# kyoungseoun-chung/pyapes

Measured on AMD Instinct MI355X. Metric: cell-updates*iters/sec, 3-D Poisson CG, higher is better.
Workload: dtype f64; 1 GPU; 3-D Poisson 512x512x512 double, periodic BCs, CG (BASELINE config 3); global_cells=134217728, parallelism=single

## Files before the change

pyapes_amd/csrc/pa_bc.hip:

```cpp
#include "pa_host.h"

#include <math.h>
#include <stdlib.h>
#include <stdio.h>
#include <string.h>

#include <algorithm>
#include <new>

template <typename T>
struct BCArgs {
  int axis, side, type;
  T sval;
  const T* vals;
  T c23, dxf, ndir;
  T c43, c13;
  const T* far0;
  const T* far1;
  const int* done;
};

template <typename T>
__global__ void __launch_bounds__(PA_BLOCK) k_bc_face(DevGeom G, T* __restrict__ x, BCArgs<T> B) {
  if (B.done && *B.done) return;
  const int a = B.axis;
  const int64_t nu = (a == 0) ? G.n1 : G.n0;
  const int64_t nv = (a == 2) ? G.n1 : G.n2;
  const int64_t N = (a == 0) ? G.g0 : (a == 1 ? G.n1 : G.n2);
  const int64_t off = (a == 0) ? G.off0 : 0;
  const int64_t st = (a == 0) ? G.s0 : (a == 1 ? G.s1 : 1);
  for (int64_t q = (int64_t)blockIdx.x * blockDim.x + threadIdx.x; q < nu * nv;
       q += (int64_t)gridDim.x * blockDim.x) {
    const int64_t u = q / nv, v = q - u * nv;
    int64_t base;
    if (a == 0) base = u * G.s1 + v;
    else if (a == 1) base = u * G.s0 + v;
    else base = u * G.s0 + v * G.s1;
    const int64_t f = (B.side == 0) ? 0 : N - 1;
    const int64_t p1 = (B.side == 0) ? pa_wrap(1, N) : pa_wrap(N - 2, N);
    const int64_t p2 = (B.side == 0) ? pa_wrap(2 % N, N) : pa_wrap(N - 3 < 0 ? N - 3 + N : N - 3, N);
    T* xf = x + base + (f - off) * st;
    if (B.type == 1) {
      *xf = B.vals ? B.vals[q] : B.sval;
    } else if (B.type == 2) {
      T vp = x[base + (p1 - off) * st];
      T vpp = x[base + (p2 - off) * st];
      T ct;
      if (B.vals) {
        ct = B.c23 * B.vals[q];
        ct = ct * B.dxf;
        ct = ct * B.ndir;
      } else {
        ct = B.sval;
      }
      T t1 = B.c43 * vp;
      T t2 = B.c13 * vpp;
      t1 = t1 - t2;
      *xf = t1 + ct;
    } else if (B.type == 3) {
      *xf = x[base + (p1 - off) * st];
    } else if (B.type == 4) {
      if (B.side == 0) {
        T vp = x[base + (p1 - off) * st];
        T vf, vff;
        if (B.far0) {
          vf = B.far0[q];
          vff = B.far1[q];
        } else {
          vf = x[base + (N - 1 - off) * st];
          vff = x[base + (pa_wrap(N - 2, N) - off) * st];
        }
        T t1 = vp - vf;
        *xf = t1 + vff;
      } else if (B.far0) {
        T t1 = B.far0[q] - x[base + (N - 1 - off) * st];
        *xf = t1 + x[base + (pa_wrap(N - 2, N) - off) * st];
      } else {
        *xf = x[base + (0 - off) * st];
      }
    }
  }
}

template <typename S>
__device__ __forceinline__ const S& pa_kernarg(size_t off) {
  return *(const S*)((const char*)__builtin_amdgcn_kernarg_segment_ptr() + off);
}
static_assert(sizeof(DevGeom) % 8 == 0, "second kernel parameter starts at sizeof(DevGeom)");

template <typename T>
__global__ void __launch_bounds__(PA_BLOCK) k_shell(DevGeom G, const SolverScalars* __restrict__ sc,
                                                     const T* __restrict__ x, T* __restrict__ shell_old,
                                                     double* __restrict__ partials, int mode) {
  if (mode == 1 && sc->done) return;
  const int64_t sz[3] = {G.n1 * G.n2, G.n0 * G.n2, G.n0 * G.n1};
  int64_t total = 0;
  int64_t start[6];
  for (int f = 0; f < 6; ++f) {
    start[f] = total;
    total += G.act[f >> 1] ? sz[f >> 1] : 0;
  }
  double s[1] = {0.0};
  for (int64_t q = (int64_t)blockIdx.x * blockDim.x + threadIdx.x; q < total;
       q += (int64_t)gridDim.x * blockDim.x) {
    int f = 0;
    for (int w = 1; w < 6; ++w)
      if (G.act[w >> 1] && q >= start[w]) f = w;
    const int a = f >> 1, side = f & 1;
    const int64_t local = q - start[f];
    int64_t i, j, k;
    if (a == 0) {
      int64_t gi = side == 0 ? 0 : G.g0 - 1;
      i = gi - G.off0;
      if (i < 0 || i >= G.n0) continue;
      j = local / G.n2; k = local - j * G.n2;
    } else if (a == 1) {
      i = local / G.n2; k = local - i * G.n2;
      j = side == 0 ? 0 : G.n1 - 1;
      int64_t gi = i + G.off0;
      if (G.act[0] && (gi == 0 || gi == G.g0 - 1)) continue;
    } else {
      i = local / G.n1; j = local - i * G.n1;
      k = side == 0 ? 0 : G.n2 - 1;
      int64_t gi = i + G.off0;
      if (G.act[0] && (gi == 0 || gi == G.g0 - 1)) continue;
      if (G.act[1] && (j == 0 || j == G.n1 - 1)) continue;
    }
    const int64_t o = i * G.s0 + j * G.s1 + k;
    T xn = x[o];
    if (mode == 1) {
      T df = xn - shell_old[q];
      T p = df * df;
      s[0] += (double)p;
    }
    shell_old[q] = xn;
  }
  if (mode == 1) pa_block_reduce_store<1>(s, partials);
}


template <typename T>
struct BCFaceDev {
  int type;
  T sval;
  const T* vals;
  T dxf, ndir;
};
template <typename T>
struct BCAll {
  BCFaceDev<T> f[6];
  T c43, c13, c23;
  const T* far_lo0;
  const T* far_lo1;
  const T* far_hi0;
  int slab_periodic0;
};

template <typename T>
__device__ __forceinline__ T pa_bc_const(const BCAll<T>& B, int f, int64_t q) {
  const BCFaceDev<T>& F = B.f[f];
  if (!F.vals) return F.sval;
  T ct = B.c23 * F.vals[q];
  ct = ct * F.dxf;
  return ct * F.ndir;
}

template <typename T, bool PER = true>
struct BCEval {
  const DevGeom& G;
  const BCAll<T>& B;
  const T* __restrict__ x;

  __device__ __forceinline__ T raw0(int f, int64_t g, int64_t base) const {
    const T* p = x + (g - G.off0) * G.s0;
    if (PER && B.slab_periodic0 && B.f[f].type == 4) {
      if (f == 0) {
        p = (g == G.g0 - 1) ? B.far_lo0 : ((g == G.g0 - 2) ? B.far_lo1 : p);
      } else {
        p = (g == 1) ? B.far_hi0 : p;
      }
    }
    return p[base];
  }

  __device__ __forceinline__ T stage0(int64_t i, int64_t j, int64_t k) const {
    const int64_t gi = i + G.off0;
    const int64_t base = j * G.s1 + k;
    int f = -1;
    if (G.act[0]) {
      if (gi == 0 && B.f[0].type) f = 0;
      else if (gi == G.g0 - 1 && B.f[1].type) f = 1;
    }
    if (f < 0) return x[i * G.s0 + base];
    const int type = B.f[f].type;
    const bool lower = f == 0;
    const int64_t N = G.g0;
    if (type == 1) return B.f[f].vals ? B.f[f].vals[base] : B.f[f].sval;
    if (type == 2) {
      T t1 = B.c43 * raw0(f, lower ? 1 : N - 2, base);
      T t2 = B.c13 * raw0(f, lower ? 2 : N - 3, base);
      t1 = t1 - t2;
      return t1 + pa_bc_const<T>(B, f, base);
    }
    if (type == 3 || !PER) return raw0(f, lower ? 1 : N - 2, base);
    T t1 = raw0(f, 1, base) - raw0(f, N - 1, base);
    return t1 + raw0(f, N - 2, base);
  }

  __device__ __forceinline__ T stage1(int64_t i, int64_t j, int64_t k) const {
    int f = -1;
    if (G.act[1]) {
      if (j == 0 && B.f[2].type) f = 2;
      else if (j == G.n1 - 1 && B.f[3].type) f = 3;
    }
    if (f < 0) return stage0(i, j, k);
    const int type = B.f[f].type;
    const bool lower = f == 2;
    const int64_t N = G.n1, q = i * G.n2 + k;
    if (type == 1) return B.f[f].vals ? B.f[f].vals[q] : B.f[f].sval;
    if (type == 2) {
      T t1 = B.c43 * stage0(i, lower ? 1 : N - 2, k);
      T t2 = B.c13 * stage0(i, lower ? 2 : N - 3, k);
      t1 = t1 - t2;
      return t1 + pa_bc_const<T>(B, f, q);
    }
    if (type == 3 || !PER) return stage0(i, lower ? 1 : N - 2, k);
    T t1 = stage0(i, 1, k) - stage0(i, N - 1, k);
    return t1 + stage0(i, N - 2, k);
  }

  __device__ __forceinline__ T stage2(int64_t i, int64_t j, int64_t k) const {
    int f = -1;
    if (G.act[2]) {
      if (k == 0 && B.f[4].type) f = 4;
      else if (k == G.n2 - 1 && B.f[5].type) f = 5;
    }
    if (f < 0) return stage1(i, j, k);
    const int type = B.f[f].type;
    const bool lower = f == 4;
    const int64_t N = G.n2, q = i * G.n1 + j;
    if (type == 1) return B.f[f].vals ? B.f[f].vals[q] : B.f[f].sval;
    if (type == 2) {
      T t1 = B.c43 * stage1(i, j, lower ? 1 : N - 2);
      T t2 = B.c13 * stage1(i, j, lower ? 2 : N - 3);
      t1 = t1 - t2;
      return t1 + pa_bc_const<T>(B, f, q);
    }
    if (type == 3 || !PER) return stage1(i, j, lower ? 1 : N - 2);
    T t1 = stage1(i, j, 1) - stage1(i, j, N - 1);
    return t1 + stage1(i, j, N - 2);
  }
};

template <typename T, bool PER>
__device__ __forceinline__ T pa_bc_v3(const DevGeom& G, const BCAll<T>& B, const T* __restrict__ x, int64_t i,
                                      int64_t j, int64_t k) {
  BCEval<T, PER> ev{G, B, x};
  return ev.stage2(i, j, k);
}

__device__ __forceinline__ bool pa_shell_node(const DevGeom& G, int64_t q, const int64_t* start, int64_t& i,
                                              int64_t& j, int64_t& k) {
  int f = 0;
  for (int w = 1; w < 6; ++w)
    if (G.act[w >> 1] && q >= start[w]) f = w;
  const int a = f >> 1, side = f & 1;
  const int64_t local = q - start[f];
  const int64_t dn = a == 2 ? G.n1 : G.n2;
  int64_t u, v;
  if (G.ncell <= 0x7fffffffLL) {
    const uint32_t lu = (uint32_t)local, du = (uint32_t)dn, uu = lu / du;
    u = uu; v = lu - uu * du;
  } else {
    u = local / dn; v = local - u * dn;
  }
  if (a == 0) {
    int64_t gi = side == 0 ? 0 : G.g0 - 1;
    i = gi - G.off0;
    if (i < 0 || i >= G.n0) return false;
    j = u; k = v;
  } else if (a == 1) {
    i = u; k = v;
    j = side == 0 ? 0 : G.n1 - 1;
    int64_t gi = i + G.off0;
    if (G.act[0] && (gi == 0 || gi == G.g0 - 1)) return false;
  } else {
    i = u; j = v;
    k = side == 0 ? 0 : G.n2 - 1;
    int64_t gi = i + G.off0;
    if (G.act[0] && (gi == 0 || gi == G.g0 - 1)) return false;
    if (G.act[1] && (j == 0 || j == G.n1 - 1)) return false;
  }
  return true;
}

template <typename T, bool PER>
__global__ void __launch_bounds__(PA_BLOCK) k_bc_compute(DevGeom G, BCAll<T> B_, const int* __restrict__ done,
                                                          const T* x, const T* __restrict__ shell_old,
                                                          T* __restrict__ shell_new, double* __restrict__ partials,
                                                          int with_delta, T* xw) {
  if (done && *done) return;
  const BCAll<T>& B = pa_kernarg<BCAll<T>>(sizeof(DevGeom));
  const int64_t sz[3] = {G.n1 * G.n2, G.n0 * G.n2, G.n0 * G.n1};
  int64_t total = 0, start[6];
  for (int f = 0; f < 6; ++f) { start[f] = total; total += G.act[f >> 1] ? sz[f >> 1] : 0; }
  double s[1] = {0.0};
  for (int64_t q = (int64_t)blockIdx.x * blockDim.x + threadIdx.x; q < total;
       q += (int64_t)gridDim.x * blockDim.x) {
    int64_t i, j, k;
    if (!pa_shell_node(G, q, start, i, j, k)) continue;
    T v = pa_bc_v3<T, PER>(G, B, x, i, j, k);
#ifdef PA_DEBUG_BC
    if (i == 0 && j == 1 && k == G.n2 - 1) {
      BCEval<T, PER> ev{G, B, x};
      printf("DBG node(0,1,%lld) v=%g stage1(0,1,n2-2)=%g stage0=%g types %d %d %d %d %d %d slabp %d far %p %p %p raw1 %g rawN1 %g rawN2 %g\n",
             (long long)k, (double)v, (double)ev.stage1(0, 1, G.n2 - 2), (double)ev.stage0(0, 1, G.n2 - 2),
             B.f[0].type, B.f[1].type, B.f[2].type, B.f[3].type, B.f[4].type, B.f[5].type, B.slab_periodic0,
             (void*)B.far_lo0, (void*)B.far_lo1, (void*)B.far_hi0, (double)ev.raw0(0, 1, 1 * G.s1 + G.n2 - 2),
             (double)ev.raw0(0, G.g0 - 1, 1 * G.s1 + G.n2 - 2), (double)ev.raw0(0, G.g0 - 2, 1 * G.s1 + G.n2 - 2));
    }
#endif
    shell_new[q] = v;
    if (xw) xw[i * G.s0 + j * G.s1 + k] = v;
    if (with_delta) {
      T df = v - shell_old[q];
      T p = df * df;
      s[0] += (double)p;
    }
  }
  if (with_delta) pa_block_reduce_store<1>(s, partials);
}

template <typename T>
__global__ void __launch_bounds__(PA_BLOCK) k_bc_scatter(DevGeom G, const int* __restrict__ done,
                                                          T* __restrict__ x, const T* __restrict__ shell_new) {
  if (done && *done) return;
  const int64_t sz[3] = {G.n1 * G.n2, G.n0 * G.n2, G.n0 * G.n1};
  int64_t total = 0, start[6];
  for (int f = 0; f < 6; ++f) { start[f] = total; total += G.act[f >> 1] ? sz[f >> 1] : 0; }
  for (int64_t q = (int64_t)blockIdx.x * blockDim.x + threadIdx.x; q < total;
       q += (int64_t)gridDim.x * blockDim.x) {
    int64_t i, j, k;
    if (!pa_shell_node(G, q, start, i, j, k)) continue;
    x[i * G.s0 + j * G.s1 + k] = shell_new[q];
  }
}


template <typename T>
struct BCPairArgs {
  BCArgs<T> lo, hi;
  int axis;
  int64_t pos_lo, pos_hi;
};

template <typename T>
__device__ __forceinline__ T pa_bc_face_value(const BCArgs<T>& B, const T* __restrict__ x, int64_t base, int64_t st,
                                              int64_t off, int64_t N, int64_t q, T x0_new) {
  const bool lower = B.side == 0;
  const int64_t p1 = lower ? 1 : N - 2, p2 = lower ? 2 : N - 3;
  if (B.type == 1) return B.vals ? B.vals[q] : B.sval;
  if (B.type == 2) {
    T ct;
    if (B.vals) {
      ct = B.c23 * B.vals[q];
      ct = ct * B.dxf;
      ct = ct * B.ndir;
    } else {
      ct = B.sval;
    }
    T t1 = B.c43 * x[base + (p1 - off) * st];
    T t2 = B.c13 * x[base + (p2 - off) * st];
    t1 = t1 - t2;
    return t1 + ct;
  }
  if (B.type == 3) return x[base + (p1 - off) * st];
  if (lower) {
    T vp = x[base + (1 - off) * st];
    T vf = B.far0 ? B.far0[q] : x[base + (N - 1 - off) * st];
    T vff = B.far0 ? B.far1[q] : x[base + (N - 2 - off) * st];
    T t1 = vp - vf;
    return t1 + vff;
  }
  if (B.far0) {
    T t1 = B.far0[q] - x[base + (N - 1 - off) * st];
    return t1 + x[base + (N - 2 - off) * st];
  }
  return x0_new;
}

template <typename T>
__global__ void __launch_bounds__(PA_BLOCK) k_bc_pair(DevGeom G, T* __restrict__ x, BCPairArgs<T> P,
                                                       const int* __restrict__ done, T* __restrict__ shell_old,
                                                       double* __restrict__ partials, int mode) {
  if (done && *done) return;
  const int a = P.axis;
  const int64_t nu = (a == 0) ? G.n1 : G.n0;
  const int64_t nv = (a == 2) ? G.n1 : G.n2;
  const int64_t N = (a == 0) ? G.g0 : (a == 1 ? G.n1 : G.n2);
  const int64_t off = (a == 0) ? G.off0 : 0;
  const int64_t st = (a == 0) ? G.s0 : (a == 1 ? G.s1 : 1);
  double s[1] = {0.0};
  for (int64_t q = (int64_t)blockIdx.x * blockDim.x + threadIdx.x; q < nu * nv;
       q += (int64_t)gridDim.x * blockDim.x) {
    const int64_t u = q / nv, v = q - u * nv;
    int64_t base;
    bool owned = true;
    if (a == 0) {
      base = u * G.s1 + v;
      if (G.act[1] && (u == 0 || u == G.n1 - 1)) owned = false;
      if (G.act[2] && (v == 0 || v == G.n2 - 1)) owned = false;
    } else if (a == 1) {
      base = u * G.s0 + v;
      if (G.act[2] && (v == 0 || v == G.n2 - 1)) owned = false;
    } else {
      base = u * G.s0 + v * G.s1;
    }
    T x0_new = (T)0;
    if (P.lo.type) {
      T* xf = x + base + (0 - off) * st;
      T val;
      if (mode == 3) {
        val = *xf;
      } else {
        val = pa_bc_face_value<T>(P.lo, x, base, st, off, N, q, (T)0);
        *xf = val;
      }
      x0_new = val;
      if (mode && owned) {
        if (mode == 1) {
          T df = val - shell_old[P.pos_lo + q];
          T p = df * df;
          s[0] += (double)p;
        }
        shell_old[P.pos_lo + q] = val;
      }
    } else if (P.hi.type == 4 && !P.hi.far0) {
      x0_new = x[base + (0 - off) * st];
    }
    if (P.hi.type) {
      T* xf = x + base + (N - 1 - off) * st;
      T val;
      if (mode == 3) {
        val = *xf;
      } else {
        val = pa_bc_face_value<T>(P.hi, x, base, st, off, N, q, x0_new);
        *xf = val;
      }
      if (mode && owned) {
        if (mode == 1) {
          T df = val - shell_old[P.pos_hi + q];
          T p = df * df;
          s[0] += (double)p;
        }
        shell_old[P.pos_hi + q] = val;
      }
    }
  }
  if (mode == 1) pa_block_reduce_store<1>(s, partials);
}

template <typename T>
static int pa_bc_shell_fused(pa_ctx* c, T* x, double* part2, int with_delta, bool guarded, int* nsh, bool standalone);
template <typename T>
static int pa_bc_pair_apply(pa_ctx* c, T* x, double* part2, int mode, bool guarded, int* nsh);
template <typename T>
static void pa_shell_launch(pa_ctx* c, const T* x, T* shell, double* part2, int with_delta);

template <typename T>
int pa_bc_apply_faces(pa_ctx* c, T* x, bool guarded) {
  const DevGeom& G = c->G;
  for (int w = 0; w < c->nbc; ++w) {
    int f = c->bc_order[w];
    const HostBC& b = c->bc[f];
    if (b.type == PA_BC_NONE) continue;
    int a = f >> 1, side = f & 1;
    if (!G.act[a]) continue;
    if (a == 0) {
      if (side == 0 && G.off0 != 0) continue;
      if (side == 1 && G.off0 + G.n0 != G.g0) continue;
    }
    BCArgs<T> B;
    memset(&B, 0, sizeof(B));
    B.axis = a; B.side = side; B.type = b.type;
    B.vals = (const T*)b.vals;
    B.c43 = (T)(4.0 / 3.0);
    B.c13 = (T)(1.0 / 3.0);
    B.c23 = (T)(2.0 / 3.0);
    B.dxf = (T)b.dxf;
    B.ndir = side == 0 ? (T)-1 : (T)1;
    B.done = guarded ? pa_done_flag(c) : nullptr;
    if (b.type == PA_BC_DIRICHLET) B.sval = (T)b.value;
    if (b.type == PA_BC_NEUMANN) {
      T pre = (T)((2.0 / 3.0) * b.value);
      pre = pre * B.dxf;
      pre = pre * B.ndir;
      B.sval = pre;
    }
    if (b.type == PA_BC_PERIODIC && a == 0 && G.n0 != G.g0) {
      B.far0 = (const T*)(side == 0 ? c->bc_far_lo0 : c->bc_far_hi0);
      B.far1 = (const T*)c->bc_far_lo1;
      if (!B.far0) { pa_set_err(c, "periodic axis-0 BC on a slab needs pa_bc_halo_ptrs planes"); return PA_E_STATE; }
    }
    int64_t nu = (a == 0) ? G.n1 : G.n0;
    int64_t nv = (a == 2) ? G.n1 : G.n2;
    hipLaunchKernelGGL(k_bc_face<T>, dim3(pa_grid_blocks(nu * nv)), dim3(PA_BLOCK), 0, c->stream, G, x, B);
  }
  PA_HIP(c, hipGetLastError());
  return PA_OK;
}

template <typename T>
int pa_bc_apply_auto(pa_ctx* c, T* x, bool guarded) {
  if (pa_bc_fusable(c)) return pa_bc_shell_fused<T>(c, x, nullptr, 0, guarded, nullptr, true);
  if (pa_bc_pairable(c)) return pa_bc_pair_apply<T>(c, x, nullptr, 0, guarded, nullptr);
  return pa_bc_apply_faces<T>(c, x, guarded);
}

int pa_bc_apply_any(pa_ctx* c, void* x) {
  return c->dtype == PA_F64 ? pa_bc_apply_auto<double>(c, (double*)x, false) : pa_bc_apply_auto<float>(c, (float*)x, false);
}

extern "C" {

int pa_apply_bc(pa_ctx* c, void* x) {
  if (!c || !c->grid_set) return PA_E_STATE;
  PA_HIP(c, hipSetDevice(c->device));
  return pa_bc_apply_any(c, x);
}

}

int pa_shell_blocks(const pa_ctx* c) {
  const DevGeom& G = c->G;
  int64_t tot = 0;
  if (G.act[0]) tot += 2 * G.n1 * G.n2;
  if (G.act[1]) tot += 2 * G.n0 * G.n2;
  if (G.act[2]) tot += 2 * G.n0 * G.n1;
  return pa_grid_blocks(tot);
}
int64_t pa_shell_elems(const pa_ctx* c) {
  const DevGeom& G = c->G;
  return 2 * (G.n1 * G.n2 + G.n0 * G.n2 + G.n0 * G.n1);
}

bool pa_bc_is_static(const pa_ctx* c) {
  for (int f = 0; f < 6; ++f) {
    int t = c->bc[f].type;
    if (t != PA_BC_NONE && t != PA_BC_DIRICHLET) return false;
  }
  return true;
}


bool pa_bc_fusable(const pa_ctx* c) {
  if (c->bc_path & 1) return false;
  bool one_pass = !c->slab;
  for (int f = 0; f < 6; ++f)
    if (c->bc[f].type == PA_BC_PERIODIC) one_pass = false;
  const int64_t limit = pa_bc_pairable(c) ? (one_pass ? 2000000 : 150000) : 400000;
  if (!(c->bc_path & 4) &&
      2 * (c->G.n1 * c->G.n2 + c->G.n0 * c->G.n2 + c->G.n0 * c->G.n1) > limit)
    return false;
  int last = -1;
  for (int w = 0; w < c->nbc; ++w) {
    if (c->bc[c->bc_order[w]].type == PA_BC_NONE) continue;
    if (c->bc_order[w] <= last) return false;
    last = c->bc_order[w];
  }
  const DevGeom& G = c->G;
  const int64_t N[3] = {G.g0, G.n1, G.n2};
  const int64_t nloc[3] = {G.n0, G.n1, G.n2};
  for (int a = 0; a < 3; ++a)
    if (G.act[a] && (N[a] < 5 || (a == 0 && nloc[0] < 3))) return false;
  for (int a = 0; a < 3; ++a)
    if ((c->bc[2 * a].type == PA_BC_PERIODIC) != (c->bc[2 * a + 1].type == PA_BC_PERIODIC)) return false;
  return true;
}

template <typename T>
static int bc_fill_all(pa_ctx* c, BCAll<T>& B) {
  memset(&B, 0, sizeof(B));
  const DevGeom& G = c->G;
  for (int f = 0; f < 6; ++f) {
    const HostBC& b = c->bc[f];
    BCFaceDev<T>& F = B.f[f];
    F.type = b.type;
    F.vals = (const T*)b.vals;
    F.dxf = (T)b.dxf;
    F.ndir = (f & 1) == 0 ? (T)-1 : (T)1;
    if (b.type == PA_BC_DIRICHLET) F.sval = (T)b.value;
    if (b.type == PA_BC_NEUMANN) {
      T pre = (T)((2.0 / 3.0) * b.value);
      pre = pre * F.dxf;
      pre = pre * F.ndir;
      F.sval = pre;
    }
    if ((f >> 1) == 0 && G.act[0]) {
      if (f == 0 && G.off0 != 0) F.type = PA_BC_NONE;
      if (f == 1 && G.off0 + G.n0 != G.g0) F.type = PA_BC_NONE;
    }
  }
  B.c43 = (T)(4.0 / 3.0);
  B.c13 = (T)(1.0 / 3.0);
  B.c23 = (T)(2.0 / 3.0);
  B.slab_periodic0 = (G.n0 != G.g0 && c->bc[0].type == PA_BC_PERIODIC) ? 1 : 0;
  if (B.slab_periodic0) {
    B.far_lo0 = (const T*)c->bc_far_lo0;
    B.far_lo1 = (const T*)c->bc_far_lo1;
    B.far_hi0 = (const T*)c->bc_far_hi0;
    if ((B.f[0].type == PA_BC_PERIODIC && (!B.far_lo0 || !B.far_lo1)) ||
        (B.f[1].type == PA_BC_PERIODIC && !B.far_hi0)) {
      pa_set_err(c, "periodic axis-0 BC on a slab needs the far planes (pa_slab_set)");
      return PA_E_STATE;
    }
  }
  return PA_OK;
}

template <typename T>
static int pa_bc_shell_fused(pa_ctx* c, T* x, double* part2, int with_delta, bool guarded, int* nsh,
                          bool standalone) {
  BCAll<T> B;
  int rc = bc_fill_all<T>(c, B);
  if (rc) return rc;
  const int nb = pa_shell_blocks(c);
  const size_t half = (size_t)pa_shell_elems(c);
  T *so, *sn;
  if (standalone) {
    if ((rc = pa_scratch(c, &c->scr[SCR_SHELL2], &c->cap[SCR_SHELL2], half * sizeof(T)))) return rc;
    so = sn = (T*)c->scr[SCR_SHELL2];
  } else {
    T* base = (T*)c->scr[SCR_SHELL];
    so = base + (c->shell_cur ? half : 0);
    sn = base + (c->shell_cur ? 0 : half);
  }
  const int* done = guarded ? pa_done_flag(c) : nullptr;
  bool direct = !c->slab;
  for (int f = 0; f < 6; ++f)
    if (c->bc[f].type == PA_BC_PERIODIC) direct = false;
  bool any_per = false;
  for (int f = 0; f < 6; ++f)
    if (c->bc[f].type == PA_BC_PERIODIC) any_per = true;
  if (any_per)
    hipLaunchKernelGGL((k_bc_compute<T, true>), dim3(nb), dim3(PA_BLOCK), 0, c->stream, c->G, B, done, (const T*)x,
                       (const T*)so, sn, part2, with_delta, direct ? x : (T*)nullptr);
  else
    hipLaunchKernelGGL((k_bc_compute<T, false>), dim3(nb), dim3(PA_BLOCK), 0, c->stream, c->G, B, done, (const T*)x,
                       (const T*)so, sn, part2, with_delta, direct ? x : (T*)nullptr);
  if (!direct)
    hipLaunchKernelGGL(k_bc_scatter<T>, dim3(nb), dim3(PA_BLOCK), 0, c->stream, c->G, done, x, (const T*)sn);
  if (!standalone) c->shell_cur ^= 1;
  if (nsh) *nsh = nb;
  PA_HIP(c, hipGetLastError());
  return PA_OK;
}

bool pa_bc_pairable(const pa_ctx* c) {
  if (c->bc_path & 2) return false;
  int last = -1, cnt = 0;
  for (int w = 0; w < c->nbc; ++w) {
    if (c->bc[c->bc_order[w]].type == PA_BC_NONE) continue;
    if (c->bc_order[w] <= last) return false;
    last = c->bc_order[w];
    ++cnt;
  }
  const DevGeom& G = c->G;
  const int64_t N[3] = {G.g0, G.n1, G.n2};
  int need = 0;
  for (int a = 0; a < 3; ++a) {
    if (!G.act[a]) continue;
    need += 2;
    if (N[a] < 5 || (a == 0 && G.n0 < 3)) return false;
    if (c->bc[2 * a].type == PA_BC_NONE || c->bc[2 * a + 1].type == PA_BC_NONE) return false;
    if ((c->bc[2 * a].type == PA_BC_PERIODIC) != (c->bc[2 * a + 1].type == PA_BC_PERIODIC)) return false;
  }
  return cnt == need;
}

template <typename T>
static void bc_face_args(pa_ctx* c, int f, BCArgs<T>& B, bool guarded) {
  const DevGeom& G = c->G;
  const HostBC& b = c->bc[f];
  memset(&B, 0, sizeof(B));
  const int a = f >> 1, side = f & 1;
  B.axis = a; B.side = side; B.type = b.type;
  if (a == 0) {
    if (side == 0 && G.off0 != 0) B.type = 0;
    if (side == 1 && G.off0 + G.n0 != G.g0) B.type = 0;
  }
  B.vals = (const T*)b.vals;
  B.c43 = (T)(4.0 / 3.0);
  B.c13 = (T)(1.0 / 3.0);
  B.c23 = (T)(2.0 / 3.0);
  B.dxf = (T)b.dxf;
  B.ndir = side == 0 ? (T)-1 : (T)1;
  B.done = guarded ? pa_done_flag(c) : nullptr;
  if (b.type == PA_BC_DIRICHLET) B.sval = (T)b.value;
  if (b.type == PA_BC_NEUMANN) {
    T pre = (T)((2.0 / 3.0) * b.value);
    pre = pre * B.dxf;
    pre = pre * B.ndir;
    B.sval = pre;
  }
  if (b.type == PA_BC_PERIODIC && a == 0 && G.n0 != G.g0) {
    B.far0 = (const T*)(side == 0 ? c->bc_far_lo0 : c->bc_far_hi0);
    B.far1 = (const T*)c->bc_far_lo1;
  }
}

template <typename T>
static int pa_bc_pair_apply(pa_ctx* c, T* x, double* part2, int mode, bool guarded, int* nsh) {
  const DevGeom& G = c->G;
  const int64_t sz[3] = {G.n1 * G.n2, G.n0 * G.n2, G.n0 * G.n1};
  int64_t start[6], total = 0;
  for (int f = 0; f < 6; ++f) { start[f] = total; total += G.act[f >> 1] ? sz[f >> 1] : 0; }
  T* shell = (T*)c->scr[SCR_SHELL];
  int rows = 0;
  for (int a = 0; a < 3; ++a) {
    if (!G.act[a]) continue;
    BCPairArgs<T> P;
    bc_face_args<T>(c, 2 * a, P.lo, guarded);
    bc_face_args<T>(c, 2 * a + 1, P.hi, guarded);
    if (mode != 3 && ((P.lo.type == PA_BC_PERIODIC && a == 0 && G.n0 != G.g0 && !P.lo.far0) ||
                      (P.hi.type == PA_BC_PERIODIC && a == 0 && G.n0 != G.g0 && !P.hi.far0))) {
      pa_set_err(c, "periodic axis-0 BC on a slab needs the far planes (pa_slab_set)");
      return PA_E_STATE;
    }
    if (!P.lo.type && !P.hi.type) continue;
    P.axis = a;
    P.pos_lo = start[2 * a];
    P.pos_hi = start[2 * a + 1];
    const int nb = pa_grid_blocks(sz[a]);
    hipLaunchKernelGGL(k_bc_pair<T>, dim3(nb), dim3(PA_BLOCK), 0, c->stream, G, x, P,
                       guarded ? pa_done_flag(c) : (const int*)nullptr, shell, part2 ? part2 + rows : nullptr,
                       mode);
    if (mode == 1) rows += nb;
  }
  if (nsh) *nsh = rows;
  PA_HIP(c, hipGetLastError());
  return PA_OK;
}


int pa_bc_shell_rows(const pa_ctx* c) {
  if (c->bc_fused || !c->bc_pair) return pa_shell_blocks(c);
  const DevGeom& G = c->G;
  const int64_t sz[3] = {G.n1 * G.n2, G.n0 * G.n2, G.n0 * G.n1};
  int rows = 0;
  for (int a = 0; a < 3; ++a) {
    if (!G.act[a]) continue;
    int lo = c->bc[2 * a].type, hi = c->bc[2 * a + 1].type;
    if (a == 0) {
      if (G.off0 != 0) lo = 0;
      if (G.off0 + G.n0 != G.g0) hi = 0;
    }
    if (lo || hi) rows += pa_grid_blocks(sz[a]);
  }
  return rows;
}

template <typename T>
static void pa_shell_launch(pa_ctx* c, const T* x, T* shell, double* part2, int with_delta) {
  hipLaunchKernelGGL(k_shell<T>, dim3(pa_shell_blocks(c)), dim3(PA_BLOCK), 0, c->stream, c->G, c->sc, x, shell, part2,
                     with_delta);
}

void pa_bc_plan(pa_ctx* c) {
  c->bc_static = pa_bc_is_static(c);
  c->bc_fused = pa_bc_fusable(c);
  c->bc_pair = (!c->bc_fused && pa_bc_pairable(c)) ? 1 : 0;
  c->shell_cur = 0;
}

template <typename T>
int pa_bc_fill_start(pa_ctx* c, T* x, bool filled_by_driver) {
  if (c->bc_fused && !filled_by_driver)
    return pa_bc_shell_fused<T>(c, x, nullptr, 0, false, nullptr, false);
  if (c->bc_pair) return pa_bc_pair_apply<T>(c, x, nullptr, filled_by_driver ? 3 : 2, false, nullptr);
  if (!filled_by_driver)
    if (int rc = pa_bc_apply_faces<T>(c, x)) return rc;
  pa_shell_launch<T>(c, (const T*)x, (T*)c->scr[SCR_SHELL], (double*)c->scr[SCR_PART2], 0);
  return PA_OK;
}

template <typename T>
int pa_bc_fill_step(pa_ctx* c, T* x, double* part2, int* nsh) {
  *nsh = 0;
  if (c->bc_static) return PA_OK;
  if (c->bc_fused) return pa_bc_shell_fused<T>(c, x, part2, 1, true, nsh, false);
  if (c->bc_pair) return pa_bc_pair_apply<T>(c, x, part2, 1, true, nsh);
  if (int rc = pa_bc_apply_faces<T>(c, x, true)) return rc;
  *nsh = pa_shell_blocks(c);
  pa_shell_launch<T>(c, (const T*)x, (T*)c->scr[SCR_SHELL], part2, 1);
  return PA_OK;
}

#define PA_BC_INST(T)                                                                            \
  template int pa_bc_apply_faces<T>(pa_ctx*, T*, bool);                                          \
  template int pa_bc_apply_auto<T>(pa_ctx*, T*, bool);                                           \
  template int pa_bc_fill_start<T>(pa_ctx*, T*, bool);                                           \
  template int pa_bc_fill_step<T>(pa_ctx*, T*, double*, int*);
PA_BC_INST(float)
PA_BC_INST(double)
#undef PA_BC_INST
```

pyapes_amd/csrc/pa_cg.hip:

```cpp
#include "pa_solver.h"

template <typename T>
__global__ void __launch_bounds__(PA_BLOCK) k_cg_a(DevGeom G, DevEq<T> E, const SolverScalars* __restrict__ sc,
                                                    Vec<T> rv, Vec<T> dv, T* __restrict__ dnew,
                                                    double* __restrict__ partials) {
  if (sc->done) return;
  DirAcc<T> acc{rv, dv, (T)sc->beta};
  double s[1] = {0.0};
  for (int64_t idx = (int64_t)blockIdx.x * blockDim.x + threadIdx.x; idx < G.ncell;
       idx += (int64_t)gridDim.x * blockDim.x) {
    int64_t i, j, k;
    pa_decode(G, idx, i, j, k);
    T e = (T)0;
    if (pa_in_S(G, i, j, k)) {
      e = acc.at(G, i, j, k);
      T Ad = pa_apply_terms<T>(G, E, acc, i, j, k, e);
      T p = e * Ad;
      s[0] += (double)p;
    }
    dnew[idx] = e;
  }
  pa_block_reduce_store<1>(s, partials);
}

template <typename T>
__global__ void __launch_bounds__(PA_BLOCK) k_cg_b(DevGeom G, DevEq<T> E, const SolverScalars* __restrict__ sc,
                                                    Vec<T> dv, T* __restrict__ x, const T* r, T* r_out,
                                                    T* __restrict__ send_lo, T* __restrict__ send_hi,
                                                    double* __restrict__ partials) {
  if (sc->done) return;
  FieldAcc<T> acc{dv};
  const T alpha = (T)sc->alpha;
  double s[2] = {0.0, 0.0};
  for (int64_t idx = (int64_t)blockIdx.x * blockDim.x + threadIdx.x; idx < G.ncell;
       idx += (int64_t)gridDim.x * blockDim.x) {
    int64_t i, j, k;
    pa_decode(G, idx, i, j, k);
    T rn = (T)0;
    if (pa_in_S(G, i, j, k)) {
      T dc = dv.p[idx];
      T Ad = pa_apply_terms<T>(G, E, acc, i, j, k, dc);
      T xo = x[idx];
      T ad = alpha * dc;
      T xn = xo + ad;
      x[idx] = xn;
      T aAd = alpha * Ad;
      rn = r[idx] - aAd;
      T p = rn * rn;
      s[0] += (double)p;
      if (!pa_on_shell(G, i, j, k)) {
        T df = xn - xo;
        T p2 = df * df;
        s[1] += (double)p2;
      }
    }
    r_out[idx] = rn;
    if (send_lo && i == 0) send_lo[j * G.s1 + k] = rn;
    if (send_hi && i == G.n0 - 1) send_hi[j * G.s1 + k] = rn;
  }
  pa_block_reduce_store<2>(s, partials);
}

template <typename T>
__global__ void __launch_bounds__(PA_BLOCK) k_cg_post_a(SolverScalars* sc, const double* partials, int nblk,
                                                         double* sums, int stage) {
  __shared__ double sm[PA_BLOCK / 64];
  if (sc->done) return;
  if (stage != 1) {
    double v = pa_reduce_partials(partials, nblk, 1, 0, sm);
    if (threadIdx.x == 0) sums[0] = v;
  }
  if (stage != 0 && threadIdx.x == 0) pa_logic_a<T>(sc, sums);
}

template <typename T>
__global__ void __launch_bounds__(PA_BLOCK) k_cg_post_b(SolverScalars* sc, const double* partials, int nblk,
                                                         const double* partials_shell, int nblk_shell,
                                                         double* sums, int stage) {
  __shared__ double sm[PA_BLOCK / 64];
  if (sc->done) return;
  if (stage != 1) {
    double rr = pa_reduce_partials(partials, nblk, 2, 0, sm);
    double dx2 = pa_reduce_partials(partials, nblk, 2, 1, sm);
    double sh = nblk_shell > 0 ? pa_reduce_partials(partials_shell, nblk_shell, 1, 0, sm) : 0.0;
    if (threadIdx.x == 0) {
      sums[1] = rr;
      sums[2] = dx2 + sh;
    }
  }
  if (stage != 0 && threadIdx.x == 0) pa_logic_b<T>(sc, sums);
}

template <typename T>
__global__ void __launch_bounds__(PA_BLOCK) k_ghost_dir(const SolverScalars* __restrict__ sc, int64_t n,
                                                         const T* __restrict__ r_lo, const T* __restrict__ r_hi,
                                                         const T* __restrict__ d_lo, const T* __restrict__ d_hi,
                                                         T* __restrict__ o_lo, T* __restrict__ o_hi) {
  if (sc->done) return;
  const T beta = (T)sc->beta;
  for (int64_t q = (int64_t)blockIdx.x * blockDim.x + threadIdx.x; q < n; q += (int64_t)gridDim.x * blockDim.x) {
    if (r_lo) { T b = beta * d_lo[q]; o_lo[q] = r_lo[q] + b; }
    if (r_hi) { T b = beta * d_hi[q]; o_hi[q] = r_hi[q] + b; }
  }
}

template <typename T>
struct MidArgs {
  const T* d;
  const T* r;
  const T* x;
  const T *r_lo, *r_hi;
  const T *d_lo, *d_hi;
  T *g_lo, *g_hi;
  T *send_lo, *send_hi;
  T *xp_lo1, *xp_hi0, *xp_hi1;
  LapCoef<T> lap;
  T coeff, sign;
  int has_coeff;
  const T* coeff_f;
};

template <typename T>
__device__ __forceinline__ T pa_lap_axis(const DevGeom& G, const LapCoef<T>& L, int a, int64_t g, int64_t N, T xp, T xc,
                                         T xm) {
  T cP = L.inv[a], cC = L.m2inv[a], cM = L.inv[a];
  const T cB = L.c23[a];
  const int rc = pa_row_case(G, a, g, N, G.treat);
  if (rc == 1) { cP = cB; cC = -cB; cM = (T)0; }
  if (rc == 2) { cP = (T)0; cC = -cB; cM = cB; }
  T s = cP * xp;
  T m = cC * xc;
  s = s + m;
  m = cM * xm;
  s = s + m;
  return s;
}

template <typename T>
__global__ void __launch_bounds__(PA_BLOCK) k_slab_mid(DevGeom G, SolverScalars* sc, const double* __restrict__ rows,
                                                        int nrows, double* __restrict__ sums, MidArgs<T> M) {
  __shared__ double sm[8];
  const int done_in = sc->done;
  const double rr_in = sc->rr;
  const T beta = (T)sc->beta;
  double v0 = 0.0;
  for (int b = threadIdx.x; b < nrows; b += PA_BLOCK) v0 += rows[b];
  if (done_in) return;
  for (int off = 32; off > 0; off >>= 1) v0 += __shfl_down(v0, off, 64);
  if ((threadIdx.x & 63) == 0) sm[threadIdx.x >> 6] = v0;
  __syncthreads();
  if (threadIdx.x == 0) {
    double v = 0.0;
    for (int w = 0; w < PA_BLOCK / 64; ++w) v += sm[w];
    const T dAd = (T)v;
    const T a = (T)rr_in / dAd;
    const double al = (isnan(a) || isinf(a)) ? 0.0 : (double)a;
    sm[4] = al;
    if (blockIdx.x == 0) {
      sc->dAd = (double)dAd;
      sc->alpha = al;
      sums[0] = v;
    }
  }
  __syncthreads();
  const T alpha = (T)sm[4];
  const int nb = (int)(gridDim.x / 5), sec = (int)(blockIdx.x / nb), bq = (int)(blockIdx.x - sec * nb);
  if (sec == 0 && !M.r_lo) return;
  if (sec == 1 && !M.r_hi) return;
  T* const xout = sec == 2 ? M.xp_lo1 : (sec == 3 ? M.xp_hi0 : M.xp_hi1);
  if (sec >= 2 && !xout) return;
  const int64_t ip = sec == 0 ? 0 : (sec == 1 ? G.n0 - 1 : (sec == 2 ? 1 : (sec == 3 ? G.n0 - 1 : G.n0 - 2)));
  const int64_t gi = ip + G.off0;
  const bool iS = gi >= G.slo[0] && gi <= G.shi[0];
  const T* const dpl = M.d + ip * G.s0;
  for (int64_t q = (int64_t)bq * blockDim.x + threadIdx.x; q < G.s0; q += (int64_t)nb * blockDim.x) {
    int64_t j, k;
    if (G.s0 <= 0x7fffffffLL) {
      const uint32_t qq = (uint32_t)q, s1 = (uint32_t)G.s1, jj = qq / s1;
      j = jj; k = qq - jj * s1;
    } else {
      j = q / G.s1; k = q - j * G.s1;
    }
    const bool inS = iS && j >= G.slo[1] && j <= G.shi[1] && k >= G.slo[2] && k <= G.shi[2];
    const T dc = dpl[q];
    if (sec >= 2) {
      const T xo = M.x[ip * G.s0 + q];
      T ad = alpha * dc;
      T xn = xo + ad;
      xout[q] = inS ? xn : xo;
      continue;
    }
    const T rg = sec == 0 ? M.r_lo[q] : M.r_hi[q];
    const T dg = sec == 0 ? M.d_lo[q] : M.d_hi[q];
    const T din = sec == 0 ? M.d[G.s0 + q] : M.d[(G.n0 - 2) * G.s0 + q];
    const T dj1 = dpl[pa_wrap(j + 1, G.n1) * G.s1 + k], dj0 = dpl[pa_wrap(j - 1, G.n1) * G.s1 + k];
    const T dk1 = dpl[j * G.s1 + pa_wrap(k + 1, G.n2)], dk0 = dpl[j * G.s1 + pa_wrap(k - 1, G.n2)];
    const T rc = M.r[ip * G.s0 + q];
    T cf = M.coeff;
    if (M.has_coeff && M.coeff_f) cf = M.coeff_f[ip * G.s0 + q];
    T bg = beta * dg;
    const T ghost = rg + bg;
    if (sec == 0) M.g_lo[q] = ghost; else M.g_hi[q] = ghost;
    T ax = (T)0;
    ax = ax + pa_lap_axis<T>(G, M.lap, 0, gi, G.g0, sec == 0 ? din : ghost, dc, sec == 0 ? ghost : din);
    ax = ax + pa_lap_axis<T>(G, M.lap, 1, j, G.n1, dj1, dc, dj0);
    ax = ax + pa_lap_axis<T>(G, M.lap, 2, k, G.n2, dk1, dc, dk0);
    if (M.has_coeff) ax = ax * cf;
    ax = ax * M.sign;
    T Ad = (T)0;
    Ad = Ad + ax;
    T aAd = alpha * Ad;
    T rn = rc - aAd;
    rn = inS ? rn : (T)0;
    if (sec == 0) M.send_lo[q] = rn; else M.send_hi[q] = rn;
  }
}

template <typename T>
static int cg_begin_t(pa_ctx* c, T* x, const T* rhs, double tol, int64_t max_it) {
  const DevGeom& G = c->G;
  const size_t fb = (size_t)G.ncell * sizeof(T);
  const int nblk = pa_grid_blocks(G.ncell);
  int rc;
  c->cg_ps1 = solver_pitch<T>(c, x);
  c->cg_pitch = c->cg_ps1 > 0 ? 1 : 0;
  const size_t fbp = c->cg_pitch ? (size_t)G.n0 * G.n1 * c->cg_ps1 * sizeof(T) : fb;
  if ((rc = pa_scratch(c, &c->scr[SCR_R], &c->cap[SCR_R], fbp))) return rc;
  if ((rc = pa_scratch(c, &c->scr[SCR_D0], &c->cap[SCR_D0], fbp))) return rc;
  if ((rc = pa_scratch(c, &c->scr[SCR_D1], &c->cap[SCR_D1], fbp))) return rc;
  if ((rc = pa_scratch(c, &c->scr[SCR_PART], &c->cap[SCR_PART], (size_t)PA_MAX_PARTIALS * 4 * sizeof(double)))) return rc;
  if ((rc = pa_scratch(c, &c->scr[SCR_PART2], &c->cap[SCR_PART2], (size_t)3 * PA_MAX_GRID * sizeof(double)))) return rc;
  if ((rc = pa_scratch(c, &c->scr[SCR_SHELL], &c->cap[SCR_SHELL], 2 * (size_t)pa_shell_elems(c) * sizeof(T)))) return rc;
  if ((rc = init_scalars(c, tol, max_it))) return rc;
  if ((rc = pa_place_begin(c, x, fb))) return rc;
  if (!c->cg_pitch) PA_HIP(c, hipMemsetAsync(c->scr[SCR_D1], 0, fb, c->stream));
  c->cg_x = x;
  c->cur = 0;
  c->fold_a_n = c->fold_b_n = c->fold_b_nsh = 0;
  c->fold_b_shell = nullptr;
  c->slab_fold = c->slab_fold_live = 0;
  pa_bc_plan(c);
  c->solve = PA_SOLVE_CG;
  DevEq<T> E;
  pa_build_eq<T>(c, c->nterms, c->terms, E);
  if ((rc = pa_bc_fill_start<T>(c, x, c->slab != 0))) return rc;
  T* r = (T*)c->scr[SCR_R];
  T* d = (T*)c->scr[SCR_D0];
  double* part = (double*)c->scr[SCR_PART];
  Vec<T> xv = pa_vec_self<T>(c, x);
  if (c->slab) { xv.glo = (const T*)c->x_glo; xv.ghi = (const T*)c->x_ghi; }
  if (c->cg_pitch) {
    if ((rc = cg_residual_init_pitch<T>(c, E, xv, rhs, (T*)c->scr[SCR_D1], r, d, part))) return rc;
    PA_HIP(c, hipMemsetAsync(c->scr[SCR_D1], 0, fbp, c->stream));
  }
  if (!c->cg_pitch && (rc = cg_residual_init<T>(c, E, xv, rhs, r, d, (T*)c->r_send_lo, (T*)c->r_send_hi, part))) return rc;
  launch_post_init<T>(c, part, nblk, c->slab ? 0 : 2);
  c->pending_init_logic = c->slab ? 1 : 0;
  if (c->slab) {
    const size_t pb = (size_t)G.s0 * sizeof(T);
    if ((rc = pa_scratch(c, &c->scr[SCR_GHOST], &c->cap[SCR_GHOST], 4 * pb))) return rc;
    PA_HIP(c, hipMemsetAsync(c->scr[SCR_GHOST], 0, 4 * pb, c->stream));
    char* g = (char*)c->scr[SCR_GHOST];
    c->d_glo[0] = g; c->d_ghi[0] = g + pb; c->d_glo[1] = g + 2 * pb; c->d_ghi[1] = g + 3 * pb;
  }
  PA_HIP(c, hipGetLastError());
  return PA_OK;
}

template <typename T>
static Vec<T> cg_vec(pa_ctx* c, const T* p, int which ) {
  Vec<T> v = pa_vec_self<T>(c, p);
  if (c->cg_pitch) v.glo = p + (c->G.n0 - 1) * c->G.n1 * c->cg_ps1;
  if (c->slab) {
    if (which == 0) {
      if (c->r_recv_lo) v.glo = (const T*)c->r_recv_lo;
      if (c->r_recv_hi) v.ghi = (const T*)c->r_recv_hi;
    } else {
      if (c->r_recv_lo) v.glo = (const T*)c->d_glo[c->cur];
      if (c->r_recv_hi) v.ghi = (const T*)c->d_ghi[c->cur];
    }
  }
  return v;
}

template <typename T>
static void cg_flush_fold(pa_ctx* c) {
  if (c->fold_a_n > 0) {
    hipLaunchKernelGGL(k_cg_post_a<T>, dim3(1), dim3(PA_BLOCK), 0, c->stream, c->sc,
                       (const double*)c->scr[SCR_PART] + 2 * (size_t)PA_MAX_PARTIALS, c->fold_a_n, pa_sums(c), 2);
    c->fold_a_n = 0;
  }
  if (c->fold_b_n > 0) {
    hipLaunchKernelGGL(k_cg_post_b<T>, dim3(1), dim3(PA_BLOCK), 0, c->stream, c->sc, c->fold_b_part,
                       c->fold_b_n, c->fold_b_shell ? c->fold_b_shell : (const double*)c->scr[SCR_PART2],
                       c->fold_b_nsh, pa_sums(c), 2);
    c->fold_b_n = c->fold_b_nsh = 0;
    c->fold_b_shell = nullptr;
  }
}

template <typename T>
int pa_cg_phase_a_t(pa_ctx* c, int stage_post) {
  PaRange range_("pyapes CG phase A: d' = r + beta d, sum d'.(A d')");
  const DevGeom& G = c->G;
  const int nblk = pa_grid_blocks(G.ncell);
  DevEq<T> E;
  pa_build_eq<T>(c, c->nterms, c->terms, E);
  T* r = (T*)c->scr[SCR_R];
  T* dold = (T*)c->scr[c->cur ? SCR_D1 : SCR_D0];
  T* dnew = (T*)c->scr[c->cur ? SCR_D0 : SCR_D1];
  double* part = (double*)c->scr[SCR_PART];
  const bool foldable = c->fold && c->in_iterate && stage_post == 2 && !c->slab && !c->profile;
  if (foldable) part += 2 * (size_t)PA_MAX_PARTIALS;
  const bool live = c->slab_fold_live != 0;
  if (live) part = c->rows_send;
  if (c->pending_init_logic) {
    launch_post_init<T>(c, nullptr, 0, 1);
    c->pending_init_logic = 0;
  }
  Vec<T> rv = cg_vec<T>(c, r, 0), dv = cg_vec<T>(c, dold, 1);
  if (c->slab && !live && (c->r_recv_lo || c->r_recv_hi)) {
    hipLaunchKernelGGL(k_ghost_dir<T>, dim3(pa_grid_blocks(G.s0)), dim3(PA_BLOCK), 0, c->stream, c->sc, G.s0,
                       (const T*)c->r_recv_lo, (const T*)c->r_recv_hi, (const T*)c->d_glo[c->cur],
                       (const T*)c->d_ghi[c->cur], (T*)c->d_glo[c->cur ^ 1], (T*)c->d_ghi[c->cur ^ 1]);
  }
  if (c->profile) (void)hipEventRecord(c->pev[0], c->stream);
  int rc = pa_cg3d_phase_a<T>(c, E, rv, dv, dnew, part);
  if (rc < 0) return rc;
  int used_blocks = rc;
  if (rc == 0 && live) { pa_set_err(c, "folded slab iteration: the tiled phase A declined after the plan"); return PA_E_STATE; }
  if (rc == 0 && c->cg_pitch) { pa_set_err(c, "pitched CG: the tiled phase A declined"); return PA_E_STATE; }
  if (rc == 0) {
    cg_flush_fold<T>(c);
    hipLaunchKernelGGL(k_cg_a<T>, dim3(nblk), dim3(PA_BLOCK), 0, c->stream, G, E, c->sc, rv, dv, dnew, part);
    used_blocks = nblk;
  }
  if (c->profile) pa_profile_stop(c, 0);
  c->cur ^= 1;
  if (live) {
  } else if (foldable && used_blocks <= PA_MAX_GRID)
    c->fold_a_n = used_blocks;
  else
    hipLaunchKernelGGL(k_cg_post_a<T>, dim3(1), dim3(PA_BLOCK), 0, c->stream, c->sc, part, used_blocks, pa_sums(c),
                       stage_post);
  PA_HIP(c, hipGetLastError());
  return PA_OK;
}

template <typename T>
int pa_cg_phase_b_t(pa_ctx* c, int stage_post) {
  PaRange range_("pyapes CG phase B: x += alpha d', r -= alpha A d', BC fill, sums");
  const DevGeom& G = c->G;
  const int nblk = pa_grid_blocks(G.ncell);
  DevEq<T> E;
  pa_build_eq<T>(c, c->nterms, c->terms, E);
  T* r = (T*)c->scr[SCR_R];
  T* d = (T*)c->scr[c->cur ? SCR_D1 : SCR_D0];
  T* x = (T*)c->cg_x;
  double* part = (double*)c->scr[SCR_PART];
  double* part2 = (double*)c->scr[SCR_PART2];
  Vec<T> dv = cg_vec<T>(c, d, 1);
  const bool live = c->slab_fold_live != 0;
  if (live) part = c->rows_send + c->fold_rows[0] + c->fold_rows[2];
  if (c->profile) (void)hipEventRecord(c->pev[2], c->stream);
  int rc = pa_cg3d_phase_b<T>(c, E, dv, x, r, part);
  if (rc < 0) return rc;
  int used_blocks = rc;
  if (rc == 0 && live) { pa_set_err(c, "folded slab iteration: the tiled phase B declined after the plan"); return PA_E_STATE; }
  if (rc == 0 && c->cg_pitch) { pa_set_err(c, "pitched CG: the tiled phase B declined"); return PA_E_STATE; }
  if (rc == 0) {
    cg_flush_fold<T>(c);
    hipLaunchKernelGGL(k_cg_b<T>, dim3(nblk), dim3(PA_BLOCK), 0, c->stream, G, E, c->sc, dv, x, (const T*)r,
                       c->cg_r_out ? (T*)c->cg_r_out : r, (T*)c->r_send_lo, (T*)c->r_send_hi, part);
    used_blocks = nblk;
  }
  if (c->cg_r_out) pa_place_r_written(c);
  if (c->profile) pa_profile_stop(c, 1);
  c->b_blocks = used_blocks;
  if (c->slab) {
    if (!live) pack_x_planes<T>(c, x);
    PA_HIP(c, hipGetLastError());
    return PA_OK;
  }
  int nsh;
  if ((rc = pa_bc_fill_step<T>(c, x, part2, &nsh))) return rc;
  const bool foldable = c->fold && c->in_iterate && stage_post == 2 && !c->slab && !c->profile &&
                        used_blocks <= PA_MAX_GRID && nsh <= 3 * PA_MAX_GRID;
  if (foldable) {
    c->fold_b_n = used_blocks;
    c->fold_b_nsh = nsh;
    c->fold_b_part = part;
  } else {
    hipLaunchKernelGGL(k_cg_post_b<T>, dim3(1), dim3(PA_BLOCK), 0, c->stream, c->sc, part, used_blocks, part2, nsh,
                       pa_sums(c), stage_post);
  }
  PA_HIP(c, hipGetLastError());
  return PA_OK;
}

template <typename T>
int pa_cg_bc_t(pa_ctx* c) {
  const DevGeom& G = c->G;
  T* x = (T*)c->cg_x;
  double* part = (double*)c->scr[SCR_PART];
  double* part2 = (double*)c->scr[SCR_PART2];
  const bool live = c->slab_fold_live != 0;
  if (live) part2 = c->rows_send + c->fold_rows[0];
  int nsh, rc;
  if ((rc = pa_bc_fill_step<T>(c, x, part2, &nsh))) return rc;
  if (live) {
    if (nsh > c->fold_rows[2]) { pa_set_err(c, "folded slab iteration: %d shell rows, %d planned", nsh, c->fold_rows[2]); return PA_E_STATE; }
    c->fold_b_part = c->rows_recv + c->fold_rows[0] + c->fold_rows[2];
    c->fold_b_n = c->fold_rows[1];
    c->fold_b_shell = c->rows_recv + c->fold_rows[0];
    c->fold_b_nsh = c->fold_rows[2];
  } else {
    hipLaunchKernelGGL(k_cg_post_b<T>, dim3(1), dim3(PA_BLOCK), 0, c->stream, c->sc, part, c->b_blocks, part2, nsh,
                       pa_sums(c), 0);
  }
  PA_HIP(c, hipGetLastError());
  return PA_OK;
}

template <typename T>
static int cg_slab_mid_t(pa_ctx* c) {
  const DevGeom& G = c->G;
  DevEq<T> E;
  pa_build_eq<T>(c, c->nterms, c->terms, E);
  if (E.nterms != 1 || E.t[0].kind != PA_OP_LAPLACIAN || c->coord != PA_COORD_XYZ || !G.act[0]) {
    pa_set_err(c, "folded slab iteration: one Laplacian term on a 3-D xyz mesh expected (the tiled kernels' equation)");
    return PA_E_STATE;
  }
  MidArgs<T> M;
  memset(&M, 0, sizeof(M));
  M.lap = E.lap;
  M.coeff = E.t[0].coeff; M.sign = E.t[0].sign; M.has_coeff = E.t[0].has_coeff; M.coeff_f = E.t[0].coeff_f;
  M.d = (const T*)c->scr[c->cur ? SCR_D1 : SCR_D0];
  M.r = (const T*)c->scr[SCR_R];
  M.x = (const T*)c->cg_x;
  M.r_lo = (const T*)c->r_recv_lo; M.r_hi = (const T*)c->r_recv_hi;
  M.d_lo = (const T*)c->d_glo[c->cur ^ 1]; M.d_hi = (const T*)c->d_ghi[c->cur ^ 1];
  M.g_lo = (T*)c->d_glo[c->cur]; M.g_hi = (T*)c->d_ghi[c->cur];
  M.send_lo = (T*)c->r_send_lo; M.send_hi = (T*)c->r_send_hi;
  if ((M.r_lo && !M.send_lo) || (M.r_hi && !M.send_hi)) { pa_set_err(c, "slab: a neighbour without a send plane"); return PA_E_STATE; }
  M.xp_lo1 = (T*)c->x_pack_lo1; M.xp_hi0 = (T*)c->x_pack_hi0; M.xp_hi1 = (T*)c->x_pack_hi1;
  const bool planes = M.r_lo || M.r_hi || M.xp_lo1 || M.xp_hi0 || M.xp_hi1;
  const int nbm = planes ? std::min(256, pa_grid_blocks(G.s0)) : 1;
  hipLaunchKernelGGL(k_slab_mid<T>, dim3(5 * nbm), dim3(PA_BLOCK), 0, c->stream, G, c->sc,
                     (const double*)c->rows_recv, c->fold_rows[0], pa_sums(c), M);
  PA_HIP(c, hipGetLastError());
  return PA_OK;
}

int pa_cg_slab_mid(pa_ctx* c) {
  return c->dtype == PA_F64 ? cg_slab_mid_t<double>(c) : cg_slab_mid_t<float>(c);
}

int pa_cg_slab_flush(pa_ctx* c) {
  if (c->dtype == PA_F64) cg_flush_fold<double>(c); else cg_flush_fold<float>(c);
  PA_HIP(c, hipGetLastError());
  return PA_OK;
}

template <typename T>
static int cg_run_t(pa_ctx* c, T* x, const T* rhs, double tol, int64_t max_it, pa_report* out) {
  int rc;
  if (try_resident<T>(c, 0, x, rhs, tol, max_it, 1.0, out, &rc)) return rc;
  if ((rc = cg_begin_t<T>(c, x, rhs, tol, max_it))) return rc;
  const int poll = poll_interval(c);
  PA_HIP(c, hipEventRecord(c->ev0, c->stream));
  int64_t enq = 0;
  c->in_iterate = 1;
  PollPipe P;
  bool done = false;
  int64_t batch = 1;
  while (!done && !rc) {
    int64_t nb = std::min<int64_t>(batch, max_it + 1 - enq);
    if (nb <= 0) {
      if ((rc = poll_drain(c, P, &done)) || done) break;
      nb = 1;
    }
    for (int64_t q = 0; q < nb && !rc; ++q) {
      if ((rc = pa_place_tick(c))) break;
      if ((rc = pa_cg_phase_a_t<T>(c, 2))) break;
      copy_x_old<T>(c, x);
      rc = pa_cg_phase_b_t<T>(c, 2);
      ++enq;
    }
    if (rc) break;
    if ((rc = pa_place_batch_end(c))) break;
    cg_flush_fold<T>(c);
    rc = poll_submit(c, P, &done);
    batch = std::min<int64_t>(poll, std::max<int64_t>(1, enq));
  }
  if (!rc) rc = read_scalars(c);
  c->in_iterate = 0;
  if (rc) { c->fold_a_n = c->fold_b_n = c->fold_b_nsh = 0; pa_place_end(c, 0); return rc; }
  rc = timed_report(c, out);
  pa_place_end(c, 1);
  return rc;
}

extern "C" int pa_cg(pa_ctx* c, void* x, const void* rhs, double tol, int64_t max_it, pa_report* out) {
  if (!c || !c->grid_set || !c->eq_set) { if (c) pa_set_err(c, "pa_cg: grid/equation not set"); return PA_E_STATE; }
  if (int rc0 = pa_check_eq_applicable(c)) return rc0;
  if (!out) return PA_E_ARG;
  if (c->slab) { pa_set_err(c, "pa_cg is the single-GPU loop; use the stepwise API on a slab"); return PA_E_STATE; }
  PA_HIP(c, hipSetDevice(c->device));
  const int rc = c->dtype == PA_F64 ? cg_run_t<double>(c, (double*)x, (const double*)rhs, tol, max_it, out)
                                    : cg_run_t<float>(c, (float*)x, (const float*)rhs, tol, max_it, out);
  c->solve = PA_SOLVE_NONE;
  pa_place_end(c, 0);
  return rc;
}

template <typename T>
static int cg_fold_plan_t(pa_ctx* c, int64_t* rows) {
  rows[0] = rows[1] = rows[2] = 0;
  DevEq<T> E;
  pa_build_eq<T>(c, c->nterms, c->terms, E);
  T* r = (T*)c->scr[SCR_R];
  T* d0 = (T*)c->scr[SCR_D0];
  T* d1 = (T*)c->scr[SCR_D1];
  double* part = (double*)c->scr[SCR_PART];
  c->plan_only = 1;
  const int na = pa_cg3d_phase_a<T>(c, E, cg_vec<T>(c, r, 0), cg_vec<T>(c, d0, 1), d1, part);
  const int nb = pa_cg3d_phase_b<T>(c, E, cg_vec<T>(c, d1, 1), (T*)c->cg_x, r, part);
  c->plan_only = 0;
  (void)hipGetLastError();
  const int ns = c->bc_static ? 0 : pa_bc_shell_rows(c);
  if (na <= 0 || nb <= 0 || na > PA_MAX_GRID || nb > PA_MAX_GRID || ns > 3 * PA_MAX_GRID) return PA_OK;
  rows[0] = na; rows[1] = nb; rows[2] = ns;
  return PA_OK;
}

extern "C" {

int pa_cg_begin(pa_ctx* c, void* x, const void* rhs, double tol, int64_t max_it) {
  if (!c || !c->grid_set || !c->eq_set) { if (c) pa_set_err(c, "pa_cg_begin: grid/equation not set"); return PA_E_STATE; }
  if (int rc0 = pa_check_eq_applicable(c)) return rc0;
  PA_HIP(c, hipSetDevice(c->device));
  return c->dtype == PA_F64 ? cg_begin_t<double>(c, (double*)x, (const double*)rhs, tol, max_it)
                            : cg_begin_t<float>(c, (float*)x, (const float*)rhs, tol, max_it);
}

int pa_cg_phase_a(pa_ctx* c) {
  if (int rc = pa_require_solve(c, PA_SOLVE_CG, "pa_cg_phase_a")) return rc;
  const int st = c->slab ? 0 : 2;
  return c->dtype == PA_F64 ? pa_cg_phase_a_t<double>(c, st) : pa_cg_phase_a_t<float>(c, st);
}

int pa_cg_phase_b(pa_ctx* c) {
  if (int rc = pa_require_solve(c, PA_SOLVE_CG, "pa_cg_phase_b")) return rc;
  if (c->slab && !c->slab_fold_live) {
    if (c->dtype == PA_F64)
      hipLaunchKernelGGL(k_cg_post_a<double>, dim3(1), dim3(PA_BLOCK), 0, c->stream, c->sc, (const double*)nullptr, 0, pa_sums(c), 1);
    else
      hipLaunchKernelGGL(k_cg_post_a<float>, dim3(1), dim3(PA_BLOCK), 0, c->stream, c->sc, (const double*)nullptr, 0, pa_sums(c), 1);
  }
  const int st = c->slab ? 0 : 2;
  return c->dtype == PA_F64 ? pa_cg_phase_b_t<double>(c, st) : pa_cg_phase_b_t<float>(c, st);
}

int pa_cg_bc(pa_ctx* c) {
  if (int rc = pa_require_solve(c, PA_SOLVE_CG, "pa_cg_bc")) return rc;
  if (!c->slab) return PA_OK;
  return c->dtype == PA_F64 ? pa_cg_bc_t<double>(c) : pa_cg_bc_t<float>(c);
}

int pa_cg_finish_iter(pa_ctx* c) {
  if (int rc = pa_require_solve(c, PA_SOLVE_CG, "pa_cg_finish_iter")) return rc;
  if (!c->slab || c->slab_fold_live) return PA_OK;
  if (c->dtype == PA_F64)
    hipLaunchKernelGGL(k_cg_post_b<double>, dim3(1), dim3(PA_BLOCK), 0, c->stream, c->sc, (const double*)nullptr, 0,
                       (const double*)nullptr, 0, pa_sums(c), 1);
  else
    hipLaunchKernelGGL(k_cg_post_b<float>, dim3(1), dim3(PA_BLOCK), 0, c->stream, c->sc, (const double*)nullptr, 0,
                       (const double*)nullptr, 0, pa_sums(c), 1);
  PA_HIP(c, hipGetLastError());
  return PA_OK;
}

int pa_cg_fold_plan(pa_ctx* c, int64_t* rows) {
  if (!c || !rows) return PA_E_ARG;
  if (int rc = pa_require_solve(c, PA_SOLVE_CG, "pa_cg_fold_plan")) return rc;
  if (!c->slab) { pa_set_err(c, "pa_cg_fold_plan needs a live slab solve (pa_slab_set, pa_cg_begin)"); return PA_E_STATE; }
  return c->dtype == PA_F64 ? cg_fold_plan_t<double>(c, rows) : cg_fold_plan_t<float>(c, rows);
}

int pa_cg_fold_set(pa_ctx* c, const int64_t* rows) {
  if (!c) return PA_E_ARG;
  if (int rc = pa_require_solve(c, PA_SOLVE_CG, "pa_cg_fold_set")) return rc;
  if (!c->slab) { pa_set_err(c, "pa_cg_fold_set needs a live slab solve"); return PA_E_STATE; }
  c->slab_fold = 0;
  if (!rows || rows[0] <= 0 || rows[1] <= 0 || rows[2] < 0) return PA_OK;
  if (rows[0] > PA_MAX_GRID || rows[1] > PA_MAX_GRID || rows[2] > 3 * PA_MAX_GRID) {
    pa_set_err(c, "pa_cg_fold_set: row counts beyond one resident wave of workgroups");
    return PA_E_ARG;
  }
  int64_t mine[3];
  if (int rc = pa_cg_fold_plan(c, mine)) return rc;
  if (mine[0] <= 0 || mine[0] > rows[0] || mine[1] > rows[1] || mine[2] > rows[2]) {
    pa_set_err(c, "pa_cg_fold_set: agreed rows (%lld %lld %lld) below this rank's (%lld %lld %lld)", (long long)rows[0],
               (long long)rows[1], (long long)rows[2], (long long)mine[0], (long long)mine[1], (long long)mine[2]);
    return PA_E_ARG;
  }
  const size_t tot = (size_t)rows[0] + 2 * (size_t)rows[1] + (size_t)rows[2];
  PA_HIP(c, hipSetDevice(c->device));
  if (tot > c->rows_cap) {
    if (c->rows_buf[0]) (void)hipFree(c->rows_buf[0]);
    if (c->rows_buf[1]) (void)hipFree(c->rows_buf[1]);
    c->rows_buf[0] = c->rows_buf[1] = nullptr;
    c->rows_cap = 0;
    PA_HIP(c, hipMalloc((void**)&c->rows_buf[0], tot * sizeof(double)));
    PA_HIP(c, hipMalloc((void**)&c->rows_buf[1], tot * sizeof(double)));
    c->rows_cap = tot;
  }
  c->rows_send = c->rows_buf[0];
  c->rows_recv = (mine[0] == rows[0] && mine[1] == rows[1] && mine[2] == rows[2]) ? c->rows_buf[0] : c->rows_buf[1];
  PA_HIP(c, hipMemsetAsync(c->rows_buf[0], 0, tot * sizeof(double), c->stream));
  PA_HIP(c, hipMemsetAsync(c->rows_buf[1], 0, tot * sizeof(double), c->stream));
  for (int q = 0; q < 3; ++q) c->fold_rows[q] = (int)rows[q];
  c->slab_fold = 1;
  return PA_OK;
}

int pa_cg_iterate(pa_ctx* c, int64_t n) {
  if (int rc = pa_require_solve(c, PA_SOLVE_CG, "pa_cg_iterate")) return rc;
  if (c->slab) { pa_set_err(c, "pa_cg_iterate is single-rank; drive the phases on a slab"); return PA_E_STATE; }
  c->in_iterate = 1;
  int rc = PA_OK;
  for (int64_t q = 0; q < n && !rc; ++q) {
    if ((rc = pa_place_tick(c))) break;
    rc = c->dtype == PA_F64 ? pa_cg_phase_a_t<double>(c, 2) : pa_cg_phase_a_t<float>(c, 2);
    if (!rc) rc = c->dtype == PA_F64 ? pa_cg_phase_b_t<double>(c, 2) : pa_cg_phase_b_t<float>(c, 2);
  }
  c->in_iterate = 0;
  if (!rc) rc = pa_place_batch_end(c);
  if (c->dtype == PA_F64) cg_flush_fold<double>(c); else cg_flush_fold<float>(c);
  return rc;
}

int pa_cg_end(pa_ctx* c, pa_report* out) {
  if (int rc = pa_require_solve(c, PA_SOLVE_CG, "pa_cg_end")) return rc;
  int rc = out ? pa_report_read(c, out) : PA_OK;
  c->solve = PA_SOLVE_NONE;
  pa_place_end(c, out ? 1 : 0);
  if (rc) return rc;
  return (out && out->status) ? PA_E_NONFINITE : PA_OK;
}

}
```

pyapes_amd/csrc/pa_cg3d.hip:

```cpp
#include "pa_cg3d_kernel.h"
#include "pa_cg2d_kernel.h"

template <typename T>
int pa_cg3d_phase_a(pa_ctx* c, const DevEq<T>& E, Vec<T> r, Vec<T> d, T* dnew, double* partials) {
  const int mode = c->cg_pitch ? 3 : cg3d_mode<T>(c, E, {r.p, d.p, dnew, r.glo, r.ghi, d.glo, d.ghi}, false, false, true);
  if (!mode) return 0;
  const bool rz = c->coord == PA_COORD_RZ;
  Cg3dArgs<T> A;
  memset(&A, 0, sizeof(A));
  fill_common<T>(c, E, A);
  A.ps1 = c->cg_ps1; A.ps0 = c->cg_ps1 * c->G.n1;
  A.r = r; A.d = d; A.dnew = dnew; A.partials = partials;
  A.reverse = 0;
  if (c->fold_b_n > 0) {
    A.pre_part = c->fold_b_part;
    A.pre_n = c->fold_b_n;
    A.pre_shell = c->fold_b_shell ? c->fold_b_shell : (const double*)c->scr[SCR_PART2];
    A.pre_nsh = c->fold_b_nsh;
    A.sc_w = c->sc_alt;
    A.pre_sums = pa_sums(c);
  }
  int n = (mode == 1 || mode == 3 || mode == 4) ? launch_cg2d<T, 0>(c, A, mode == 3) : 0;
  if (n == 0 && rz) return 0;
  if (n == 0) n = launch_any<T, 0>(c, A, mode);
  if (n > 0 && hipGetLastError() != hipSuccess) { pa_set_err(c, "k_cg3d phase A launch failed"); return PA_E_HIP; }
  if (n > 0 && c->fold_b_n > 0) {
    SolverScalars* t = c->sc; c->sc = c->sc_alt; c->sc_alt = t;
    c->fold_b_n = c->fold_b_nsh = 0;
    c->fold_b_shell = nullptr;
  }
  return n;
}

template <typename T>
int pa_cg3d_phase_b(pa_ctx* c, const DevEq<T>& E, Vec<T> d, T* x, T* r, double* partials) {
  T* const r_out = c->cg_r_out ? (T*)c->cg_r_out : r;
  const int mode = c->cg_pitch ? 3 : cg3d_mode<T>(c, E, {d.p, x, r, r_out, d.glo, d.ghi, c->r_send_lo, c->r_send_hi}, false, false, true);
  if (!mode) return 0;
  const bool rz = c->coord == PA_COORD_RZ;
  Cg3dArgs<T> A;
  memset(&A, 0, sizeof(A));
  fill_common<T>(c, E, A);
  A.ps1 = c->cg_ps1; A.ps0 = c->cg_ps1 * c->G.n1;
  A.d = d; A.x = x; A.rw = r; A.rw_out = r_out; A.partials = partials;
  if (!c->slab_fold_live) {
    A.send_lo = (T*)c->r_send_lo; A.send_hi = (T*)c->r_send_hi;
  }
  A.reverse = 1;
  if (c->fold_a_n > 0) {
    A.pre_part = (const double*)c->scr[SCR_PART] + 2 * (size_t)PA_MAX_PARTIALS;
    A.pre_n = c->fold_a_n;
    A.sc_w = c->sc;
    A.pre_sums = pa_sums(c);
  }
  int n = (mode == 1 || mode == 3 || mode == 4) ? launch_cg2d<T, 1>(c, A, mode == 3) : 0;
  if (n == 0 && rz) return 0;
  if (n == 0) n = launch_any<T, 1>(c, A, mode);
  if (n > 0 && hipGetLastError() != hipSuccess) { pa_set_err(c, "k_cg3d phase B launch failed"); return PA_E_HIP; }
  if (n > 0) c->fold_a_n = 0;
  return n;
}

template <typename T>
int pa_tile3d_jacobi(pa_ctx* c, const DevEq<T>& E, Vec<T> x, const T* rhs, T* xnew, double omega, double* partials) {
  const int mode = cg3d_mode<T>(c, E, {x.p, rhs, xnew, x.glo, x.ghi}, false, false, true);
  if (!mode) return 0;
  const bool rz = c->coord == PA_COORD_RZ;
  Cg3dArgs<T> A;
  memset(&A, 0, sizeof(A));
  fill_common<T>(c, E, A);
  A.d = x; A.out = xnew; A.aux = rhs; A.p0 = (T)omega; A.partials = partials;
  if (c->fold_b_n > 0) {
    A.pre_part = c->fold_b_part;
    A.pre_n = c->fold_b_n;
    A.pre_shell = c->fold_b_shell ? c->fold_b_shell : (const double*)c->scr[SCR_PART2];
    A.pre_nsh = c->fold_b_nsh;
    A.sc_w = c->sc_alt;
    A.pre_sums = pa_sums(c);
  }
  int n = 0;
  if (mode == 1 || mode == 4) {
    const bool back2 = c->jac_alt && c->jac_dir && !c->plan_only;
    n = back2 ? launch_cg2d<T, 9>(c, A, false) : launch_cg2d<T, 4>(c, A, false);
    if (n > 0 && !c->plan_only) c->jac_dir ^= 1;
  }
  if (n == 0 && rz) return 0;
  if (n == 0) {
    const bool back = c->jac_alt && c->jac_dir && !c->plan_only;
    n = back ? launch_any<T, 9>(c, A, mode) : launch_any<T, 4>(c, A, mode);
    if (n > 0 && !c->plan_only) c->jac_dir ^= 1;
  }
  if (n > 0 && hipGetLastError() != hipSuccess) { pa_set_err(c, "k_cg3d Jacobi launch failed"); return PA_E_HIP; }
  if (n > 0 && c->fold_b_n > 0) {
    SolverScalars* t = c->sc; c->sc = c->sc_alt; c->sc_alt = t;
    c->fold_b_n = c->fold_b_nsh = 0;
    c->fold_b_shell = nullptr;
  }
  return n;
}

template int pa_tile3d_jacobi<float>(pa_ctx*, const DevEq<float>&, Vec<float>, const float*, float*, double, double*);
template int pa_tile3d_jacobi<double>(pa_ctx*, const DevEq<double>&, Vec<double>, const double*, double*, double, double*);
template int pa_cg3d_phase_a<float>(pa_ctx*, const DevEq<float>&, Vec<float>, Vec<float>, float*, double*);
template int pa_cg3d_phase_a<double>(pa_ctx*, const DevEq<double>&, Vec<double>, Vec<double>, double*, double*);
template int pa_cg3d_phase_b<float>(pa_ctx*, const DevEq<float>&, Vec<float>, float*, float*, double*);
template int pa_cg3d_phase_b<double>(pa_ctx*, const DevEq<double>&, Vec<double>, double*, double*, double*);
```

pyapes_amd/csrc/pa_cg3d_kernel.h:

```cpp
#pragma once
#include "pa_host.h"

#include <stdio.h>
#include <stdlib.h>
#include <string.h>

template <typename T> struct VecOf;
template <> struct VecOf<double> { static constexpr int N = 2; typedef double type __attribute__((ext_vector_type(2))); };
template <> struct VecOf<float>  { static constexpr int N = 4; typedef float type __attribute__((ext_vector_type(4))); };

template <typename T>
struct Cg3dArgs {
  DevGeom G;
  LapCoef<T> lap;
  T coeff, sign;
  int has_coeff;
  const T* coeff_f;
  const SolverScalars* sc;
  Vec<T> r, d;
  T* dnew;
  T* x;
  T* rw;
  T* rw_out;
  T* send_lo;
  T* send_hi;
  double* partials;
  int tiles_j, tiles_k, chunks, reverse;
  const T* aux;
  T* out;
  Vec<T> v;
  T* out2;
  T p0, p1, u;
  T hh[3], h2[3], ih[3];
  int kind;
  int lap_off;
  GradCoef<T> grd;
  int gnd;
  int64_t ps0, ps1;
  const T* rz;
  int64_t rz_n;
  int interior_only;
  int out_all;
  int bcl_type[6];
  T bcl_val[6];
  T bcl_c43, bcl_c13;
  const double* pre_part;
  const double* pre_shell;
  int pre_n, pre_nsh;
  SolverScalars* sc_w;
  double* pre_sums;
  const T* stg_phi0;
  T stg_c0, stg_c1;
  const T* src;
  T src_val;
};

__device__ __forceinline__ int pa_xcd_remap(int b, int nb) {
  const int q = nb >> 3, r = nb & 7, xcd = b & 7, w = b >> 3;
  return (xcd < r ? xcd * (q + 1) : r * (q + 1) + (xcd - r) * q) + w;
}

__device__ __forceinline__ int64_t pa_wrapmod(int64_t v, int64_t n) {
  v %= n;
  return v < 0 ? v + n : v;
}

template <typename T, int RJ, int PHASE, bool CF = false, int KIND = 0, int LAY = 0, bool STG = false>
__global__ void __launch_bounds__(256) k_cg3d(Cg3dArgs<T> A) {
  static_assert(!STG || PHASE == 3, "STG: the explicit Euler step");
  constexpr int PH = PHASE == 9 ? 4 : PHASE;
  constexpr bool NARROW = LAY == 1, PITCH = LAY == 2;
  static_assert(!PITCH || ((PH == 0 || PH == 1 || PH == 5 || PH == 6 || PH == 8) && !CF && KIND == 0),
                "PITCH: the CG / BiCGSTAB phases of a plain Laplacian");
  constexpr int VEC = NARROW ? 1 : VecOf<T>::N;
  typedef T V __attribute__((ext_vector_type(VEC)));
  constexpr int TJ = 4 * RJ, TK = 64 * VEC, TKP = TK + 2 * VEC;
  __shared__ __attribute__((aligned(16))) T tile[2][TJ + 2][TKP];

  (void)sizeof(int[PH >= 0 && PH <= 8 ? 1 : -1]);
  T beta = (T)0, alpha = (T)0;
  T omega = (T)0;
  const DevGeom& G = A.G;
  const int lane = threadIdx.x & 63, wv = threadIdx.x >> 6;
  const int vb = pa_xcd_remap(blockIdx.x, gridDim.x);
  const int tiles = A.tiles_j * A.tiles_k;
  const int chunk = vb / tiles, tl = vb - chunk * tiles;
  const int tjb = tl / A.tiles_k, tkb = tl - tjb * A.tiles_k;
  const int64_t i0 = (int64_t)chunk * G.n0 / A.chunks, i1 = (int64_t)(chunk + 1) * G.n0 / A.chunks;
  const int CI = (int)(i1 - i0);
  const int64_t j0 = (int64_t)tjb * TJ, k0 = (int64_t)tkb * TK;
  constexpr int rev = (PHASE == 1 || PHASE == 9) ? 1 : 0;

  const int64_t kg = k0 + (int64_t)lane * VEC;
  const int64_t kc = pa_wrapmod(kg, G.n2);
  const bool kvalid = kg < G.n2;
  const int64_t fs0 = PITCH ? A.ps0 : G.s0, fs1 = PITCH ? A.ps1 : G.s1;
  const int64_t kcf = PITCH ? (kg < fs1 ? kg : 0) : kc;
  int64_t jrow[RJ];
  unsigned rowS = 0, rowShell = 0, rowValid = 0, rowLo = 0, rowHi = 0;
#pragma unroll
  for (int jj = 0; jj < RJ; ++jj) {
    const int64_t jg = j0 + wv * RJ + jj;
    jrow[jj] = pa_wrapmod(jg, G.n1);
    const bool valid = jg < G.n1;
    if (valid) rowValid |= 1u << jj;
    if (valid && jg >= G.slo[1] && jg <= G.shi[1]) rowS |= 1u << jj;
    if (jg == 0 || jg == G.n1 - 1) rowShell |= 1u << jj;
    const int rc = pa_row_case(G, 1, jg, G.n1, G.treat);
    if (rc == 1) rowLo |= 1u << jj;
    if (rc == 2) rowHi |= 1u << jj;
  }
  unsigned rowPLo = 0, rowPHi = 0, colPLo = 0, colPHi = 0;
  if (PH == 3 || PH == 7 || KIND != 0) {
#pragma unroll
    for (int jj = 0; jj < RJ; ++jj) {
      const int64_t jg = j0 + wv * RJ + jj;
      if (G.bct[2] == 4 && jg == 1) rowPLo |= 1u << jj;
      if (G.bct[3] == 4 && jg == G.n1 - 2) rowPHi |= 1u << jj;
    }
#pragma unroll
    for (int v = 0; v < VEC; ++v) {
      if (G.bct[4] == 4 && kg + v == 1) colPLo |= 1u << v;
      if (G.bct[5] == 4 && kg + v == G.n2 - 2) colPHi |= 1u << v;
    }
  }
  unsigned colS = 0, colShell = 0, colLo = 0, colHi = 0;
#pragma unroll
  for (int v = 0; v < VEC; ++v) {
    const int64_t kk = kg + v;
    if (kvalid && kk >= G.slo[2] && kk <= G.shi[2]) colS |= 1u << v;
    if (kk == 0 || kk == G.n2 - 1) colShell |= 1u << v;
    const int rc = pa_row_case(G, 2, kk, G.n2, G.treat);
    if (rc == 1) colLo |= 1u << v;
    if (rc == 2) colHi |= 1u << v;
  }
#ifdef PA_PLAIN_EXPERIMENT
  rowLo = rowHi = colLo = colHi = 0;
  rowS = rowValid = (1u << RJ) - 1;
  colS = (1u << VEC) - 1;
#endif
  const int64_t hrow = (wv == 0) ? pa_wrapmod(j0 - 1, G.n1) : pa_wrapmod(j0 + TJ, G.n1);
  const bool hvec = (wv == 0 || wv == 3);
  const bool hsc = (wv == 1 && lane < 2 * TJ);
  const int hs_row = lane >> 1, hs_side = lane & 1;
  const int64_t hs_off = pa_wrapmod(j0 + hs_row, G.n1) * fs1 +
                         (hs_side ? pa_wrapmod(k0 + TK, G.n2) : pa_wrapmod(k0 - 1, G.n2));

  auto plane_of = [&](int q) -> int64_t { return rev ? (i1 - 1 - q) : (i0 + q); };
  auto pptr = [&](const Vec<T>& v, int64_t ii) -> const T* {
    return ii < 0 ? v.glo : (ii >= G.n0 ? v.ghi : v.p + ii * fs0);
  };

  struct Raw {
    V d[RJ];
    V r[RJ];
    V q[RJ];
    V hd, hr, hq;
    T sd, sr, sq;
  };
  constexpr bool HAS_R = (PH == 0 || PH == 5 || PH == 6);
  constexpr bool HAS_Q = (PH == 5);
  auto issue_at = [&](const T* dp, const T* rp, const T* qp, Raw& w, bool with_halo) {
#pragma unroll
    for (int jj = 0; jj < RJ; ++jj) {
      const int64_t o = jrow[jj] * fs1 + kcf;
      w.d[jj] = *reinterpret_cast<const V*>(dp + o);
      if (HAS_R) w.r[jj] = *reinterpret_cast<const V*>(rp + o);
      if (HAS_Q) w.q[jj] = *reinterpret_cast<const V*>(qp + o);
    }
    if (with_halo) {
      if (hvec) {
        const int64_t o = hrow * fs1 + kcf;
        w.hd = *reinterpret_cast<const V*>(dp + o);
        if (HAS_R) w.hr = *reinterpret_cast<const V*>(rp + o);
        if (HAS_Q) w.hq = *reinterpret_cast<const V*>(qp + o);
      }
      if (hsc) {
        w.sd = dp[hs_off];
        if (HAS_R) w.sr = rp[hs_off];
        if (HAS_Q) w.sq = qp[hs_off];
      }
    }
  };
  auto issue = [&](int64_t ii, Raw& w, bool with_halo) {
    const T* dp = pptr(A.d, ii);
    issue_at(dp, HAS_R ? pptr(A.r, ii) : dp, HAS_Q ? pptr(A.v, ii) : dp, w, with_halo);
  };
  auto combine = [&](T rr_, T dd_, T qq_) -> T {
    if (PH == 0) {
      T bd = beta * dd_;
      return rr_ + bd;
    } else if (PH == 5) {
      T t = omega * qq_;
      t = dd_ - t;
      t = beta * t;
      return rr_ + t;
    } else if (PH == 6) {
      T av = alpha * dd_;
      return rr_ - av;
    }
    return dd_;
  };
  auto finish_own = [&](const Raw& w, V (&e)[RJ]) {
#pragma unroll
    for (int jj = 0; jj < RJ; ++jj) {
#pragma unroll
      for (int v = 0; v < VEC; ++v)
        e[jj][v] = combine(HAS_R ? w.r[jj][v] : (T)0, w.d[jj][v], HAS_Q ? w.q[jj][v] : (T)0);
    }
  };
  auto finish_halo = [&](const Raw& w, V& hv, T& hs) {
#pragma unroll
    for (int v = 0; v < VEC; ++v) hv[v] = combine(HAS_R ? w.hr[v] : (T)0, w.hd[v], HAS_Q ? w.hq[v] : (T)0);
    hs = combine(HAS_R ? w.sr : (T)0, w.sd, HAS_Q ? w.sq : (T)0);
  };
  auto stage = [&](int buf, const V (&e)[RJ], const V& hv, const T& hs) {
#pragma unroll
    for (int jj = 0; jj < RJ; ++jj)
      *reinterpret_cast<V*>(&tile[buf][wv * RJ + jj + 1][VEC + lane * VEC]) = e[jj];
    if (hvec) *reinterpret_cast<V*>(&tile[buf][wv == 0 ? 0 : TJ + 1][VEC + lane * VEC]) = hv;
    if (hsc) tile[buf][hs_row + 1][hs_side ? VEC + TK : VEC - 1] = hs;
  };

  V ea[RJ], ec[RJ], eb[RJ];
  V hv;
  T hs = (T)0;
  Raw w;
#pragma unroll
  for (int v = 0; v < VEC; ++v) { hv[v] = (T)0; w.hd[v] = (T)0; w.hr[v] = (T)0; w.hq[v] = (T)0; }
  w.sd = (T)0; w.sr = (T)0; w.sq = (T)0;

  const bool act0 = G.act[0] != 0;
  Raw wa = w, wc = w;
  if (act0) issue(plane_of(-1), wa, false);
  issue(plane_of(0), wc, true);
  if (act0) issue(plane_of(1), w, CI > 1);

  if ((PH == 0 || PH == 4) && A.pre_n > 0) {
    __shared__ double pre_sm[16];
    const SolverScalars* si = A.sc;
    const int done_in = si->done;
    const double rr_in = si->rr, beta_in = si->beta, tol_lim = si->tolerance;
    const long long itr_in = si->itr, max_it = si->max_it;
    double v0 = 0.0, v1 = 0.0, v2 = 0.0;
    for (int b = threadIdx.x; b < A.pre_n; b += 256) {
      if (PH == 0) v0 += A.pre_part[2 * (int64_t)b];
      v1 += A.pre_part[2 * (int64_t)b + 1];
    }
    for (int b = threadIdx.x; b < A.pre_nsh; b += 256) v2 += A.pre_shell[b];
    if (done_in) {
      if (blockIdx.x == 0 && threadIdx.x == 0) *A.sc_w = *si;
      return;
    }
    for (int off = 32; off > 0; off >>= 1) {
      v0 += __shfl_down(v0, off, 64);
      v1 += __shfl_down(v1, off, 64);
      v2 += __shfl_down(v2, off, 64);
    }
    if ((threadIdx.x & 63) == 0) {
      const int w = threadIdx.x >> 6;
      pre_sm[3 * w] = v0;
      pre_sm[3 * w + 1] = v1;
      pre_sm[3 * w + 2] = v2;
    }
    __syncthreads();
    if (threadIdx.x == 0) {
      double rr = 0.0, dx2 = 0.0, sh = 0.0;
      for (int w = 0; w < 4; ++w) { rr += pre_sm[3 * w]; dx2 += pre_sm[3 * w + 1]; sh += pre_sm[3 * w + 2]; }
      const T rr_new = (T)rr;
      const T tolv = (T)sqrt(dx2 + sh);
      const bool bad = isnan(tolv) || isinf(tolv);
      const T rr_old = (T)rr_in;
      const double bq = bad ? beta_in : (double)(rr_new / rr_old);
      const long long itr = itr_in + (bad ? 0 : 1);
      const int done = (bad || itr > max_it || !((double)tolv > tol_lim)) ? 1 : 0;
      pre_sm[12] = bq;
      pre_sm[13] = done ? 1.0 : 0.0;
      if (blockIdx.x == 0) {
        SolverScalars* so = A.sc_w;
        *so = *si;
        so->tol = (double)tolv;
        so->done = done;
        if (bad) {
          so->err = 1;
        } else {
          if (PH == 0) {
            so->rr_old = (double)rr_old;
            so->beta = bq;
            so->rr = (double)rr_new;
          }
          so->itr = itr;
        }
        if (PH == 0) A.pre_sums[1] = rr;
        A.pre_sums[2] = dx2 + sh;
      }
    }
    __syncthreads();
    if (pre_sm[13] != 0.0) return;
    beta = (T)pre_sm[12];
  } else if (PH == 1 && A.pre_n > 0) {
    __shared__ double pre_sm[8];
    const int done_in = A.sc->done;
    const double rr_in = A.sc->rr;
    double v0 = 0.0;
    for (int b = threadIdx.x; b < A.pre_n; b += 256) v0 += A.pre_part[b];
    if (done_in) return;
    for (int off = 32; off > 0; off >>= 1) v0 += __shfl_down(v0, off, 64);
    if ((threadIdx.x & 63) == 0) pre_sm[threadIdx.x >> 6] = v0;
    __syncthreads();
    if (threadIdx.x == 0) {
      double v = 0.0;
      for (int w = 0; w < 4; ++w) v += pre_sm[w];
      const T dAd = (T)v;
      const T a = (T)rr_in / dAd;
      const double al = (isnan(a) || isinf(a)) ? 0.0 : (double)a;
      pre_sm[4] = al;
      if (blockIdx.x == 0) {
        A.sc_w->dAd = (double)dAd;
        A.sc_w->alpha = al;
        A.pre_sums[0] = v;
      }
    }
    __syncthreads();
    alpha = (T)pre_sm[4];
  } else if ((PH == 5 || PH == 8) && A.pre_n > 0) {
    __shared__ double pre_sm[8];
    const SolverScalars* si = A.sc;
    const int done_in = si->done, fe = si->finished_early;
    const double tol_lim = si->tolerance, rho_next = si->rho_next, rho_in = si->rho, alpha_in = si->alpha,
                 omega_in = si->omega;
    const long long itr_in = si->itr, max_it = si->max_it;
    double v0 = 0.0;
    for (int b = threadIdx.x; b < A.pre_n; b += 256) v0 += A.pre_part[b];
    if (done_in) {
      if (blockIdx.x == 0 && threadIdx.x == 0) *A.sc_w = *si;
      return;
    }
    for (int off = 32; off > 0; off >>= 1) v0 += __shfl_down(v0, off, 64);
    if ((threadIdx.x & 63) == 0) pre_sm[threadIdx.x >> 6] = v0;
    __syncthreads();
    if (threadIdx.x == 0) {
      double v = 0.0;
      for (int w = 0; w < 4; ++w) v += pre_sm[w];
      const T tolv = (T)sqrt(v);
      const bool bad = !fe && (isnan(tolv) || isinf(tolv));
      int done = (fe || bad) ? 1 : 0;
      T bq = (T)0;
      if (!fe && !bad) {
        if ((double)tolv <= tol_lim) done = 1;
        if (itr_in >= max_it) done = 1;
        bq = (T)rho_next / (T)rho_in;
        bq = bq * (T)alpha_in;
        bq = bq / (T)omega_in;
      }
      pre_sm[4] = (double)bq;
      pre_sm[5] = done ? 1.0 : 0.0;
      if (blockIdx.x == 0) {
        SolverScalars* so = A.sc_w;
        *so = *si;
        so->done = done;
        if (!fe) {
          so->tol = (double)tolv;
          if (bad) {
            so->err = 1;
          } else {
            so->beta = (double)bq;
            so->rho = rho_next;
          }
        }
      }
    }
    __syncthreads();
    if (pre_sm[5] != 0.0) return;
    beta = (T)pre_sm[4];
    omega = (T)omega_in;
  } else if (PH == 6 && A.pre_n > 0) {
    __shared__ double pre_sm[8];
    const int done_in = A.sc->done;
    const double rho_in = A.sc->rho;
    double v0 = 0.0;
    for (int b = threadIdx.x; b < A.pre_n; b += 256) v0 += A.pre_part[b];
    if (done_in) return;
    for (int off = 32; off > 0; off >>= 1) v0 += __shfl_down(v0, off, 64);
    if ((threadIdx.x & 63) == 0) pre_sm[threadIdx.x >> 6] = v0;
    __syncthreads();
    if (threadIdx.x == 0) {
      double v = 0.0;
      for (int w = 0; w < 4; ++w) v += pre_sm[w];
      const T q = (T)rho_in / (T)v;
      const double al = (isnan(q) || isinf(q)) ? 0.0 : (double)q;
      pre_sm[4] = al;
      if (blockIdx.x == 0) {
        A.sc_w->itr += 1;
        A.sc_w->alpha = al;
      }
    }
    __syncthreads();
    alpha = (T)pre_sm[4];
  } else {
    if (PH != 2 && PH != 3 && PH != 7 && A.sc->done) return;
    if (PH == 0) beta = (T)A.sc->beta;
    if (PH == 1) alpha = (T)A.sc->alpha;
    if (PH == 5) { beta = (T)A.sc->beta; omega = (T)A.sc->omega; }
    if (PH == 6) alpha = (T)A.sc->alpha;
  }

  if (act0) {
    finish_own(wa, ea);
  } else {
#pragma unroll
    for (int jj = 0; jj < RJ; ++jj)
#pragma unroll
      for (int v = 0; v < VEC; ++v) ea[jj][v] = (T)0;
  }
  finish_own(wc, ec);
  finish_halo(wc, hv, hs);
  stage(0, ec, hv, hs);
  if (act0) {
    finish_own(w, eb);
    finish_halo(w, hv, hs);
  } else {
#pragma unroll
    for (int jj = 0; jj < RJ; ++jj)
#pragma unroll
      for (int v = 0; v < VEC; ++v) eb[jj][v] = (T)0;
  }
  __syncthreads();

  double s0 = 0.0, s1 = 0.0, s2 = 0.0, s3 = 0.0;
  const T sgn = A.sign, cf = A.coeff;
  const int hasc = A.has_coeff;
  const T cfe = hasc ? cf : (T)1;
  constexpr bool VROW = (PH == 2 || PH == 3 || PH == 4 || PH == 7 || KIND != 0);
  V cPkV, cCkV, cMkV;
  if (VROW) {
#pragma unroll
    for (int v = 0; v < VEC; ++v) {
      T p = A.lap.inv[2], c0 = A.lap.m2inv[2], mq = A.lap.inv[2];
      if (colLo >> v & 1) { p = A.lap.c23[2]; c0 = -A.lap.c23[2]; mq = (T)0; }
      if (colHi >> v & 1) { p = (T)0; c0 = -A.lap.c23[2]; mq = A.lap.c23[2]; }
      cPkV[v] = p; cCkV[v] = c0; cMkV[v] = mq;
    }
  }
  V gPkV, gCkV, gMkV;
  if (PH == 7) {
#pragma unroll
    for (int v = 0; v < VEC; ++v) {
      T p = A.grd.g[2], c0 = (T)0, mq = A.grd.mg[2];
      if (colLo >> v & 1) { p = A.grd.lo_p[2]; c0 = A.grd.lo_c[2]; mq = (T)0; }
      if (colHi >> v & 1) { p = (T)0; c0 = A.grd.hi_c[2]; mq = A.grd.hi_m[2]; }
      if (colPLo >> v & 1) mq = (T)0;
      if (colPHi >> v & 1) p = (T)0;
      gPkV[v] = p; gCkV[v] = c0; gMkV[v] = mq;
    }
  }

  const int64_t pstep = rev ? -fs0 : fs0;
  const T* d_run = A.d.p + plane_of(1) * fs0;
  const T* r_run = HAS_R ? A.r.p + plane_of(1) * fs0 : d_run;
  const T* q_run = HAS_Q ? A.v.p + plane_of(1) * fs0 : d_run;
  const T* const d_end = pptr(A.d, plane_of(CI));
  const T* const r_end = HAS_R ? pptr(A.r, plane_of(CI)) : d_end;
  const T* const q_end = HAS_Q ? pptr(A.v, plane_of(CI)) : d_end;

  for (int m = 0; m < CI; ++m) {
    const int buf = m & 1;
    const int64_t ii = plane_of(m);
    const bool more = m + 1 < CI;
    if (more) stage(buf ^ 1, eb, hv, hs);
    V xv[RJ], rv[RJ];
    if (PH == 1) {
#pragma unroll
      for (int jj = 0; jj < RJ; ++jj) {
        const int64_t o = ii * G.s0 + jrow[jj] * G.s1 + kc;
        if (PITCH) {
          rv[jj] = __builtin_nontemporal_load(reinterpret_cast<const V*>(A.rw + ii * fs0 + jrow[jj] * fs1 + kcf));
          const T* xp = A.x + ii * G.s0 + jrow[jj] * G.s1;
#pragma unroll
          for (int v = 0; v < VEC; ++v) xv[jj][v] = xp[kg + v < G.n2 ? kg + v : G.n2 - 1];
        } else if (NARROW) {
          xv[jj] = *reinterpret_cast<const V*>(A.x + o);
          rv[jj] = *reinterpret_cast<const V*>(A.rw + o);
        } else {
          xv[jj] = __builtin_nontemporal_load(reinterpret_cast<const V*>(A.x + o));
          rv[jj] = __builtin_nontemporal_load(reinterpret_cast<const V*>(A.rw + o));
        }
      }
    }
    V cv[RJ];
    if (CF) {
#pragma unroll
      for (int jj = 0; jj < RJ; ++jj)
        cv[jj] = *reinterpret_cast<const V*>(A.coeff_f + ii * G.s0 + jrow[jj] * G.s1 + kc);
    }
    if (PH == 4 || PH == 5 || PH == 6 || PH == 8 || ((PH == 3 || (PH == 2 && KIND != 0)) && A.aux)) {
#pragma unroll
      for (int jj = 0; jj < RJ; ++jj) {
        if ((PH == 5 || PH == 6 || PH == 8) && !NARROW) {
          xv[jj] = PITCH ? __builtin_nontemporal_load(reinterpret_cast<const V*>(A.aux + ii * fs0 + jrow[jj] * fs1 + kcf))
                         : __builtin_nontemporal_load(reinterpret_cast<const V*>(A.aux + ii * G.s0 + jrow[jj] * G.s1 + kc));
          continue;
        }
        xv[jj] = PITCH ? *reinterpret_cast<const V*>(A.aux + ii * fs0 + jrow[jj] * fs1 + kcf)
                 : (PH == 4 && !NARROW) ? __builtin_nontemporal_load(reinterpret_cast<const V*>(A.aux + ii * G.s0 + jrow[jj] * G.s1 + kc))
                       : *reinterpret_cast<const V*>(A.aux + ii * G.s0 + jrow[jj] * G.s1 + kc);
      }
    }
    if constexpr (STG) {
#pragma unroll
      for (int jj = 0; jj < RJ; ++jj)
        rv[jj] = *reinterpret_cast<const V*>(A.stg_phi0 + ii * G.s0 + jrow[jj] * G.s1 + kc);
    }
    d_run += pstep;
    if (HAS_R) r_run += pstep;
    if (HAS_Q) q_run += pstep;
    if (more) {
      const bool inside = m + 2 < CI;
      issue_at(inside ? d_run : d_end, HAS_R ? (inside ? r_run : r_end) : d_run, HAS_Q ? (inside ? q_run : q_end) : d_run, w, inside);
    }

    const int64_t gi = ii + G.off0;
    const bool iS = gi >= G.slo[0] && gi <= G.shi[0];
    const bool iShell = act0 && (gi == 0 || gi == G.g0 - 1);
    T cPi = A.lap.inv[0], cCi = A.lap.m2inv[0], cMi = A.lap.inv[0];
    {
      const int rc = pa_row_case(G, 0, gi, G.g0, G.treat);
      if (rc == 1) { cPi = A.lap.c23[0]; cCi = -A.lap.c23[0]; cMi = (T)0; }
      if (rc == 2) { cPi = (T)0; cCi = -A.lap.c23[0]; cMi = A.lap.c23[0]; }
      if (!act0) { cPi = (T)0; cCi = (T)0; cMi = (T)0; }
    }
    const bool iPLo = (PH == 3 || PH == 7 || KIND != 0) && G.bct[0] == 4 && gi == 1;
    const bool iPHi = (PH == 3 || PH == 7 || KIND != 0) && G.bct[1] == 4 && gi == G.g0 - 2;
    T gP0 = A.grd.g[0], gC0 = (T)0, gM0 = A.grd.mg[0];
    if (PH == 7) {
      const int rc = pa_row_case(G, 0, gi, G.g0, G.treat);
      if (rc == 1) { gP0 = A.grd.lo_p[0]; gC0 = A.grd.lo_c[0]; gM0 = (T)0; }
      if (rc == 2) { gP0 = (T)0; gC0 = A.grd.hi_c[0]; gM0 = A.grd.hi_m[0]; }
      if (iPLo) gM0 = (T)0;
      if (iPHi) gP0 = (T)0;
    }
    V res[RJ];
    V g0r[RJ], g1r[RJ], g2r[RJ];
#pragma unroll
    for (int jj = 0; jj < RJ; ++jj) {
      const int R = wv * RJ + jj + 1;
      T cPj = A.lap.inv[1], cCj = A.lap.m2inv[1], cMj = A.lap.inv[1];
      if (rowLo >> jj & 1) { cPj = A.lap.c23[1]; cCj = -A.lap.c23[1]; cMj = (T)0; }
      if (rowHi >> jj & 1) { cPj = (T)0; cCj = -A.lap.c23[1]; cMj = A.lap.c23[1]; }
      V up, dn;
      if (jj > 0) up = ec[jj - 1]; else up = *reinterpret_cast<const V*>(&tile[buf][R - 1][VEC + lane * VEC]);
      if (jj < RJ - 1) dn = ec[jj + 1]; else dn = *reinterpret_cast<const V*>(&tile[buf][R + 1][VEC + lane * VEC]);
      const T left = tile[buf][R][VEC + lane * VEC - 1];
      const T right = tile[buf][R][VEC + lane * VEC + VEC];
      if constexpr (VROW) {
        const V xc = ec[jj];
        const V xpi = rev ? ea[jj] : eb[jj];
        const V xmi = rev ? eb[jj] : ea[jj];
        V xpk, xmk;
  #pragma unroll
        for (int v = 0; v < VEC; ++v) {
          xpk[v] = (v < VEC - 1) ? xc[v + 1 < VEC ? v + 1 : v] : right;
          xmk[v] = (v > 0) ? xc[v > 0 ? v - 1 : 0] : left;
        }
        if constexpr (PH == 7) {
          T pj = A.grd.g[1], cj = (T)0, mj = A.grd.mg[1];
          if (rowLo >> jj & 1) { pj = A.grd.lo_p[1]; cj = A.grd.lo_c[1]; mj = (T)0; }
          if (rowHi >> jj & 1) { pj = (T)0; cj = A.grd.hi_c[1]; mj = A.grd.hi_m[1]; }
          if (rowPLo >> jj & 1) mj = (T)0;
          if (rowPHi >> jj & 1) pj = (T)0;
          V s = gP0 * xpi;
          V mm = gC0 * xc;
          s = s + mm;
          mm = gM0 * xmi;
          g0r[jj] = s + mm;
          s = pj * dn;
          mm = cj * xc;
          s = s + mm;
          mm = mj * up;
          g1r[jj] = s + mm;
          s = gPkV * xpk;
          mm = gCkV * xc;
          s = s + mm;
          mm = gMkV * xmk;
          g2r[jj] = s + mm;
          continue;
        }
        V axv;
        {
          V s = cPi * xpi;
          V mm = cCi * xc;
          s = s + mm;
          mm = cMi * xmi;
          s = s + mm;
          if (act0) axv = s; else axv = (V)(T)0;
          s = cPj * dn;
          mm = cCj * xc;
          s = s + mm;
          mm = cMj * up;
          s = s + mm;
          axv = axv + s;
          s = cPkV * xpk;
          mm = cCkV * xc;
          s = s + mm;
          mm = cMkV * xmk;
          s = s + mm;
          axv = axv + s;
          if (hasc) {
            if (CF) axv = axv * cv[jj]; else axv = axv * cf;
          }
          axv = axv * sgn;
        }
        auto div_row = [&](const V& uc) -> V {
          const V xp3[3] = {xpi, dn, xpk}, xm3[3] = {xmi, up, xmk};
          V adv = (V)(T)0;
          if (KIND == 4) {
            V upl, umi;
  #pragma unroll
            for (int v = 0; v < VEC; ++v) {
              upl[v] = uc[v] > (T)0 ? uc[v] : (T)0;
              umi[v] = uc[v] < (T)0 ? uc[v] : (T)0;
            }
  #pragma unroll
            for (int a = 0; a < 3; ++a) {
              if (a == 0 && !act0) continue;
              V bwd = xc - xm3[a];
              V fwd = xp3[a] - xc;
              V t = upl * bwd;
              V m2 = umi * fwd;
              t = t + m2;
              t = t * A.ih[a];
              adv = adv + t;
            }
          } else if (KIND == 3) {
            V cP, cC, cM;
  #pragma unroll
            for (int v = 0; v < VEC; ++v) {
              cP[v] = (T)2 * (uc[v] < (T)0 ? uc[v] : (T)0);
              cC[v] = (T)0 * ((T)2 * uc[v]);
              cM[v] = (T)2 * (uc[v] > (T)0 ? uc[v] : (T)0);
            }
  #pragma unroll
            for (int a = 0; a < 3; ++a) {
              if (a == 0 && !act0) continue;
              V t = cP * xp3[a];
              V m2 = cC * xc;
              t = t + m2;
              m2 = cM * xm3[a];
              t = t + m2;
              adv = adv + t;
            }
          } else {
  #pragma unroll
            for (int a = 0; a < 3; ++a) {
              if (a == 0 && !act0) continue;
              V cP = uc, cC = (T)0 * uc, cM = -uc;
  #pragma unroll
              for (int v = 0; v < VEC; ++v) {
                const bool lo = a == 0 ? iPLo : (a == 1 ? (bool)(rowPLo >> jj & 1) : (bool)(colPLo >> v & 1));
                const bool hi = a == 0 ? iPHi : (a == 1 ? (bool)(rowPHi >> jj & 1) : (bool)(colPHi >> v & 1));
                if (lo) cM[v] = (T)0;
                if (hi) cP[v] = (T)0;
              }
              cP = cP / A.h2[a];
              cC = cC / A.h2[a];
              cM = cM / A.h2[a];
              V t = cP * xp3[a];
              V m2 = cC * xc;
              t = t + m2;
              m2 = cM * xm3[a];
              t = t + m2;
              adv = adv + t;
            }
          }
          return adv;
        };
        if constexpr (PH == 3) {
          const V ax = axv;
          V uc;
          if (A.aux) uc = xv[jj]; else uc = (V)A.u;
          const V adv = div_row(uc);
          V q = A.p0 * ax;
          q = q - adv;
          q = A.p1 * q;
          res[jj] = xc + q;
          continue;
        }
        if constexpr (KIND != 0 && PH != 3) {
          V dv = div_row((PH == 2 && A.aux) ? xv[jj] : (V)A.u);
          dv = dv * A.p0;
          if (A.lap_off) axv = (V)(T)0;
          if (A.p1 != (T)0) axv = dv + axv; else axv = axv + dv;
        }
  #pragma unroll
        for (int v = 0; v < VEC; ++v) {
          T ax = axv[v];
          T cCk = cCkV[v];
          if (PH == 4) {
            T dg = act0 ? cCi : (T)0;
            dg = dg + cCj;
            dg = dg + cCk;
            if (hasc) dg = dg * (CF ? cv[jj][v] : cf);
            dg = dg * sgn;
            T q = xv[jj][v] - ax;
            q = q / dg;
            q = A.p0 * q;
            ax = xc[v] + q;
          }
          res[jj][v] = ax;
        }
      } else {
  #pragma unroll
        for (int v = 0; v < VEC; ++v) {
          const T xc = ec[jj][v];
          const T xpi = rev ? ea[jj][v] : eb[jj][v];
          const T xmi = rev ? eb[jj][v] : ea[jj][v];
          T s = cPi * xpi;
          T mm = cCi * xc;
          s = s + mm;
          mm = cMi * xmi;
          s = s + mm;
          T ax = s;
          s = cPj * dn[v];
          mm = cCj * xc;
          s = s + mm;
          mm = cMj * up[v];
          s = s + mm;
          ax = ax + s;
          T cPk = A.lap.inv[2], cCk = A.lap.m2inv[2], cMk = A.lap.inv[2];
          if (colLo >> v & 1) { cPk = A.lap.c23[2]; cCk = -A.lap.c23[2]; cMk = (T)0; }
          if (colHi >> v & 1) { cPk = (T)0; cCk = -A.lap.c23[2]; cMk = A.lap.c23[2]; }
          const T xpk = (v < VEC - 1) ? ec[jj][v + 1 < VEC ? v + 1 : v] : right;
          const T xmk = (v > 0) ? ec[jj][v > 0 ? v - 1 : 0] : left;
          s = cPk * xpk;
          mm = cCk * xc;
          s = s + mm;
          mm = cMk * xmk;
          s = s + mm;
          ax = ax + s;
          if (CF) ax = ax * cv[jj][v]; else ax = ax * cfe;
          ax = ax * sgn;
          if (PH == 4) {
            T dg = act0 ? cCi : (T)0;
            dg = dg + cCj;
            dg = dg + cCk;
            if (hasc) dg = dg * (CF ? cv[jj][v] : cf);
            dg = dg * sgn;
            T q = xv[jj][v] - ax;
            q = q / dg;
            q = A.p0 * q;
            ax = xc + q;
          }
          res[jj][v] = ax;
        }
      }
    }

#pragma unroll
    for (int jj = 0; jj < RJ; ++jj) {
      if constexpr (PH == 7) {
        if (kvalid && (rowValid >> jj & 1)) {
          const int64_t o = ii * G.s0 + jrow[jj] * G.s1 + kc;
          const int c0 = A.gnd - 3;
          if (act0) *reinterpret_cast<V*>(A.out + (int64_t)c0 * G.ncell + o) = g0r[jj];
          *reinterpret_cast<V*>(A.out + (int64_t)(c0 + 1) * G.ncell + o) = g1r[jj];
          *reinterpret_cast<V*>(A.out + (int64_t)(c0 + 2) * G.ncell + o) = g2r[jj];
        }
        continue;
      }
      V outd;
      V outx;
#pragma unroll
      for (int v = 0; v < VEC; ++v) {
        const bool inS = iS && (rowS >> jj & 1) && (colS >> v & 1);
        const T xc = ec[jj][v];
        if (PH == 5 || PH == 6 || PH == 8) {
          const bool mine = kvalid && (rowValid >> jj & 1);
          const T an = inS ? res[jj][v] : (T)0;
          outd[v] = xc;
          outx[v] = an;
          const T r0c = xv[jj][v];
          if (PH == 5 || PH == 8) {
            T p = r0c * an;
            s0 += inS ? (double)p : 0.0;
          } else {
            T p = xc * xc;
            s0 += mine ? (double)p : 0.0;
            T a = an * xc, b = an * an, cc = r0c * an;
            s1 += inS ? (double)a : 0.0;
            s2 += inS ? (double)b : 0.0;
            s3 += inS ? (double)cc : 0.0;
          }
        } else if (PH == 2) {
          outd[v] = (inS || !A.interior_only) ? res[jj][v] : (T)0;
        } else if (PH == 3) {
          outd[v] = inS ? res[jj][v] : xc;
          if constexpr (STG) {
            T t0 = A.stg_c0 * rv[jj][v];
            T t1 = A.stg_c1 * outd[v];
            outd[v] = t0 + t1;
          }
        } else if (PH == 4) {
          const T xn = inS ? res[jj][v] : xc;
          const bool offshell = inS && !(iShell || (rowShell >> jj & 1) || (colShell >> v & 1));
          T df = xn - xc;
          T p2 = df * df;
          s1 += offshell ? (double)p2 : 0.0;
          outd[v] = xn;
        } else if (PH == 0) {
          const T e = inS ? xc : (T)0;
          outd[v] = e;
          T p = e * res[jj][v];
          s0 += (double)p;
        } else {
          const T xo = xv[jj][v];
          T ad = alpha * xc;
          T xn = xo + ad;
          T aAd = alpha * res[jj][v];
          T rn = rv[jj][v] - aAd;
          xn = inS ? xn : xo;
          rn = inS ? rn : (T)0;
          T p = rn * rn;
          s0 += (double)p;
          const bool offshell = inS && !(iShell || (rowShell >> jj & 1) || (colShell >> v & 1));
          T df = xn - xo;
          T p2 = df * df;
          s1 += offshell ? (double)p2 : 0.0;
          outd[v] = rn;
          outx[v] = xn;
        }
      }
      if (kvalid && (rowValid >> jj & 1)) {
        const int64_t o = ii * G.s0 + jrow[jj] * G.s1 + kc;
        const int64_t ob = PITCH ? ii * fs0 + jrow[jj] * fs1 + kcf : o;
        if (PH == 8) {
          *reinterpret_cast<V*>(A.out2 + ob) = outx;
        } else if (PH == 5 || PH == 6) {
          if (PH == 5 || A.out) *reinterpret_cast<V*>(A.out + ob) = outd;
          *reinterpret_cast<V*>(A.out2 + ob) = outx;
        } else if (PH >= 2) {
          *reinterpret_cast<V*>(A.out + o) = outd;
        } else if (PH == 0) {
          if (PITCH) __builtin_nontemporal_store(outd, reinterpret_cast<V*>(A.dnew + ii * fs0 + jrow[jj] * fs1 + kcf));
          else if (NARROW) *reinterpret_cast<V*>(A.dnew + o) = outd;
          else __builtin_nontemporal_store(outd, reinterpret_cast<V*>(A.dnew + o));
        } else {
          if (PITCH) {
            __builtin_nontemporal_store(outd, reinterpret_cast<V*>(A.rw_out + ii * fs0 + jrow[jj] * fs1 + kcf));
            T* xp = A.x + ii * G.s0 + jrow[jj] * G.s1;
#pragma unroll
            for (int v = 0; v < VEC; ++v)
              if (kg + v < G.n2) xp[kg + v] = outx[v];
          } else if (NARROW) {
            *reinterpret_cast<V*>(A.x + o) = outx;
            *reinterpret_cast<V*>(A.rw_out + o) = outd;
          } else {
            __builtin_nontemporal_store(outx, reinterpret_cast<V*>(A.x + o));
            __builtin_nontemporal_store(outd, reinterpret_cast<V*>(A.rw_out + o));
          }
          if (A.send_lo && ii == 0) *reinterpret_cast<V*>(A.send_lo + jrow[jj] * G.s1 + kc) = outd;
          if (A.send_hi && ii == G.n0 - 1) *reinterpret_cast<V*>(A.send_hi + jrow[jj] * G.s1 + kc) = outd;
        }
      }
    }

#pragma unroll
    for (int jj = 0; jj < RJ; ++jj) {
      ea[jj] = ec[jj];
      ec[jj] = eb[jj];
    }
    if (more) {
      finish_own(w, eb);
      finish_halo(w, hv, hs);
    }
    __syncthreads();
  }

  if (PH == 0) {
    double s[1] = {s0};
    pa_block_reduce_store<1>(s, A.partials);
  } else if (PH == 1 || PH == 4) {
    double s[2] = {s0, s1};
    pa_block_reduce_store<2>(s, A.partials);
  } else if (PH == 5 || PH == 8) {
    double s[1] = {s0};
    pa_block_reduce_store<1>(s, A.partials);
  } else if (PH == 6) {
    double s[4] = {s0, s1, s2, s3};
    pa_block_reduce_store<4>(s, A.partials);
  }
}

template <typename T>
static bool eq_lap_div(const DevEq<T>& E, int& il, int& id, bool field_speed = false) {
  il = id = -1;
  if (E.nterms == 1 && E.t[0].kind == PA_OP_LAPLACIAN) { il = 0; return true; }
  if (E.nterms == 1) {
    const int k = E.t[0].kind;
    const bool speed_ok = !E.t[0].u_f || (field_speed && k != PA_OP_DIV_CENTRAL);
    if ((k == PA_OP_DIV_CENTRAL || k == PA_OP_DIV_UPWIND_COMPAT || k == PA_OP_DIV_UPWIND) && speed_ok &&
        !E.t[0].coeff_f) { id = 0; return true; }
    return false;
  }
  if (E.nterms != 2) return false;
  for (int q = 0; q < 2; ++q) {
    const int k = E.t[q].kind;
    if (k == PA_OP_LAPLACIAN) il = q;
    else if ((k == PA_OP_DIV_CENTRAL || k == PA_OP_DIV_UPWIND_COMPAT || k == PA_OP_DIV_UPWIND) && !E.t[q].u_f) id = q;
  }
  return il >= 0 && id >= 0 && !E.t[il].coeff_f;
}

template <typename T>
static int cg3d_mode(const pa_ctx* c, const DevEq<T>& E, std::initializer_list<const void*> ptrs,
                     bool allow_div = false, bool field_speed = false, bool rz_ok = false) {
  if (!c->fastpath) return 0;
  if (c->coord != PA_COORD_XYZ) {
    if (!rz_ok || c->coord != PA_COORD_RZ || c->ndim != 2 || E.nterms != 1 || E.t[0].kind != PA_OP_LAPLACIAN || E.t[0].coeff_f)
      return 0;
    uintptr_t bits = 0;
    for (const void* q : ptrs) bits |= (uintptr_t)q;
    if ((bits & 15) || c->G.n2 % VecOf<T>::N != 0) return 0;
    return 4;
  }
  if (c->ndim != 3 && c->ndim != 2) return 0;
  int il, id;
  if (!eq_lap_div<T>(E, il, id, field_speed) || (id >= 0 && !allow_div)) return 0;
  if ((c->ndim == 3 && c->G.n0 < 3) || c->G.n1 < 3 || c->G.n2 < 3) return 0;
  uintptr_t bits = il >= 0 ? (uintptr_t)E.t[il].coeff_f : 0;
  if (id >= 0) bits |= (uintptr_t)E.t[id].u_f;
  for (const void* q : ptrs) bits |= (uintptr_t)q;
  if (bits & (sizeof(T) - 1)) return 0;
  constexpr int VEC = VecOf<T>::N;
  if ((bits & 15) || c->G.n2 % VEC != 0 || c->G.n2 < 2 * VEC) return 2;
  return 1;
}

static int cus_of(pa_ctx* c) {
  static int cus = 0;
  if (!cus) {
    hipDeviceProp_t prop;
    if (hipGetDeviceProperties(&prop, c->device) == hipSuccess) cus = prop.multiProcessorCount;
    if (cus <= 0) cus = 256;
  }
  return cus;
}

template <typename T, int RJ, int PHASE, bool CF, int KIND = 0, int LAY = 0, bool STG = false>
static int blocks_per_cu() {
  static int cached = 0;
  if (!cached) {
    int n = 0;
    if (hipOccupancyMaxActiveBlocksPerMultiprocessor(&n, k_cg3d<T, RJ, PHASE, CF, KIND, LAY, STG>, 256, 0) != hipSuccess || n <= 0) n = 2;
    cached = n;
  }
  return cached;
}

template <typename T, int RJ, int PHASE, bool CF = false, int KIND = 0, int LAY = 0, bool STG = false>
static int launch_cg3d(pa_ctx* c, Cg3dArgs<T>& A) {
  constexpr bool NARROW = LAY == 1;
  constexpr int VEC = NARROW ? 1 : VecOf<T>::N;
  constexpr int TJ = 4 * RJ, TK = 64 * VEC;
  const DevGeom& G = c->G;
  int64_t n1e = G.n1, n2e = G.n2;
  if (PHASE == 0 || PHASE == 1 || PHASE == 5 || PHASE == 6 || PHASE == 8) {
    if (G.bct[3] != PA_BC_PERIODIC && n1e > 2) n1e -= 1;
    if (G.bct[5] != PA_BC_PERIODIC && n2e > 2) n2e -= 1;
  }
  A.tiles_j = (int)((n1e + TJ - 1) / TJ);
  A.tiles_k = (int)((n2e + TK - 1) / TK);
  const int tiles = A.tiles_j * A.tiles_k;
  const int capacity = cus_of(c) * blocks_per_cu<T, RJ, PHASE, CF, KIND, LAY, STG>();
  int chunks = capacity / tiles;
  if (chunks < 1) chunks = 1;
  if (chunks > G.n0) chunks = (int)G.n0;
  if (c->chunks > 0 && chunks > c->chunks) chunks = c->chunks;
  A.chunks = chunks;
  const int nblk = tiles * chunks;
  if (nblk > PA_MAX_PARTIALS) return 0;
  static int dbg = -1;
  if (dbg < 0) dbg = getenv("PYAPES_HIP_DEBUG") ? 8 : 0;
  if (dbg > 0) {
    --dbg;
    fprintf(stderr, "[pyapes_hip] k_cg3d phase %c%s%s: tiles %dx%d chunks %d (CI ~%lld) blocks %d, %d blocks/CU x %d CUs\n",
            (char)('A' + PHASE), LAY == 1 ? " (narrow)" : (LAY == 2 ? " (pitched)" : ""), STG ? " (RK stage)" : "", A.tiles_j, A.tiles_k, chunks, (long long)(G.n0 / chunks), nblk,
            blocks_per_cu<T, RJ, PHASE, CF, KIND, LAY, STG>(), cus_of(c));
  }
  if (c->plan_only) return nblk;
  hipLaunchKernelGGL((k_cg3d<T, RJ, PHASE, CF, KIND, LAY, STG>), dim3(nblk), dim3(256), 0, c->stream, A);
  return nblk;
}

template <typename T, int PHASE = 0>
static int pick_rj(pa_ctx* c, bool narrow = false, bool cg_phase = false) {
  const int VEC = narrow ? 1 : VecOf<T>::N;
  const DevGeom& G = c->G;
  if (!G.act[0]) return 4;
  const int64_t n1e = G.n1 - ((cg_phase && G.bct[3] != PA_BC_PERIODIC && G.n1 > 2) ? 1 : 0);
  const int64_t n2e = G.n2 - ((cg_phase && G.bct[5] != PA_BC_PERIODIC && G.n2 > 2) ? 1 : 0);
  const int64_t tk = (n2e + 64 * VEC - 1) / (64 * VEC);
  const int cap = cus_of(c) * 2;
  auto chunk_len = [&](int rj) {
    const int64_t tiles = ((n1e + 4 * rj - 1) / (4 * rj)) * tk;
    const int64_t chunks = cap / tiles > 0 ? cap / tiles : 1;
    return G.n0 / chunks;
  };
  if (PHASE == 3) {
    return chunk_len(4) >= 12 ? 4 : 2;
  }
  if (G.n1 <= 4) return 1;
  if (G.n1 <= 8) return 2;
  return (chunk_len(4) < 24 && chunk_len(2) >= 24) ? 2 : 4;
}

template <typename T, int PHASE, int NARROW, bool STG = false>
static int launch_any_w(pa_ctx* c, Cg3dArgs<T>& A) {
  constexpr bool CF_OK = (PHASE == 0 || PHASE == 1 || PHASE == 2 || PHASE == 4 || PHASE == 9);
  if (A.coeff_f) {
    if (!CF_OK) return 0;
    if constexpr (CF_OK) {
      switch (pick_rj<T>(c, NARROW == 1)) {
        case 1: return launch_cg3d<T, 1, PHASE, true, 0, NARROW>(c, A);
        case 2: return launch_cg3d<T, 2, PHASE, true, 0, NARROW>(c, A);
        default: return launch_cg3d<T, 4, PHASE, true, 0, NARROW>(c, A);
      }
    }
  }
  if constexpr (PHASE == 3) {
    const int rj = pick_rj<T, 3>(c, NARROW == 1);
#define PA_EULER_CASE(K)                                                   \
    case K:                                                                \
      switch (rj) {                                                        \
        case 1: return launch_cg3d<T, 1, 3, false, K, NARROW, STG>(c, A);  \
        case 2: return launch_cg3d<T, 2, 3, false, K, NARROW, STG>(c, A);  \
        default: return launch_cg3d<T, 4, 3, false, K, NARROW, STG>(c, A); \
      }
    switch (A.kind) {
      PA_EULER_CASE(PA_OP_DIV_CENTRAL)
      PA_EULER_CASE(PA_OP_DIV_UPWIND_COMPAT)
      PA_EULER_CASE(PA_OP_DIV_UPWIND)
      default: return 0;
    }
#undef PA_EULER_CASE
  }
  if constexpr (PHASE == 2 || PHASE == 5 || PHASE == 6 || PHASE == 8) {
    if (A.kind != 0) {
      const bool four = pick_rj<T>(c, NARROW == 1) == 4;
#define PA_DIV_CASE(K)                                                                   \
      case K:                                                                            \
        return four ? launch_cg3d<T, 4, PHASE, false, K, NARROW>(c, A)                   \
                    : launch_cg3d<T, 2, PHASE, false, K, NARROW>(c, A);
      switch (A.kind) {
        PA_DIV_CASE(PA_OP_DIV_CENTRAL)
        PA_DIV_CASE(PA_OP_DIV_UPWIND_COMPAT)
        PA_DIV_CASE(PA_OP_DIV_UPWIND)
        default: return 0;
      }
#undef PA_DIV_CASE
    }
  }
  const int rj = pick_rj<T>(c, NARROW == 1, PHASE == 0 || PHASE == 1 || PHASE == 5 || PHASE == 6 || PHASE == 8);
  switch (rj) {
    case 1: return launch_cg3d<T, 1, PHASE, false, 0, NARROW>(c, A);
    case 2: return launch_cg3d<T, 2, PHASE, false, 0, NARROW>(c, A);
    default: return launch_cg3d<T, 4, PHASE, false, 0, NARROW>(c, A);
  }
}

template <typename T, int PHASE>
static int launch_pitched(pa_ctx* c, Cg3dArgs<T>& A) {
  static_assert(PHASE == 0 || PHASE == 1 || PHASE == 5 || PHASE == 6 || PHASE == 8, "PITCH: CG / BiCGSTAB phases");
  if (A.coeff_f || A.kind != 0) return 0;
  switch (pick_rj<T>(c, false, true)) {
    case 1: return launch_cg3d<T, 1, PHASE, false, 0, 2>(c, A);
    case 2: return launch_cg3d<T, 2, PHASE, false, 0, 2>(c, A);
    default: return launch_cg3d<T, 4, PHASE, false, 0, 2>(c, A);
  }
}

template <typename T, int PHASE, bool STG = false>
static int launch_any(pa_ctx* c, Cg3dArgs<T>& A, int mode) {
  if constexpr (PHASE == 0 || PHASE == 1 || PHASE == 5 || PHASE == 6 || PHASE == 8) {
    if (mode == 3) return launch_pitched<T, PHASE>(c, A);
  }
  return mode == 2 ? launch_any_w<T, PHASE, 1, STG>(c, A) : launch_any_w<T, PHASE, 0, STG>(c, A);
}

template <typename T>
static void fill_common(pa_ctx* c, const DevEq<T>& E, Cg3dArgs<T>& A) {
  int il = 0, id = -1;
  (void)eq_lap_div<T>(E, il, id, true);
  A.lap_off = (il < 0 && id >= 0) ? 1 : 0;
  if (il < 0) il = 0;
  A.G = c->G;
  A.lap = E.lap;
  A.coeff = E.t[il].coeff;
  A.coeff_f = E.t[il].coeff_f;
  A.sign = E.t[il].sign;
  A.has_coeff = E.t[il].has_coeff;
  A.sc = c->sc;
  if (id >= 0) {
    for (int a = 0; a < 3; ++a) {
      T h = (T)c->dx[a];
      A.hh[a] = h;
      A.h2[a] = (T)2 * h;
      A.ih[a] = (T)1 / h;
    }
    A.kind = E.t[id].kind;
    A.u = E.t[id].u;
    A.p0 = E.t[id].sign;
    A.p1 = id < il ? (T)1 : (T)0;
  }
}

template <typename T>
static void fill_h(const pa_ctx* c, Cg3dArgs<T>& A) {
  for (int a = 0; a < 3; ++a) {
    T h = (T)c->dx[a];
    A.hh[a] = h;
    A.h2[a] = (T)2 * h;
    A.ih[a] = (T)1 / h;
  }
}
```

pyapes_amd/csrc/pa_core.hip:

```cpp
#include "pa_host.h"

#include <dlfcn.h>
#include <math.h>
#include <stdlib.h>
#include <stdio.h>
#include <string.h>

#include <algorithm>
#include <chrono>
#include <new>

template <typename T>
__global__ void __launch_bounds__(PA_BLOCK) k_rz_tables(int64_t nr, const T* __restrict__ r_nodes, T dr,
                                                         T* __restrict__ tab) {
  auto nn = [](T v) -> T { return (isnan(v) || isinf(v)) ? (T)0 : v; };
  const T h2 = dr * dr;
  const T c23 = (T)(2.0 / 3.0), c13 = (T)(1.0 / 3.0);
  for (int64_t i = (int64_t)blockIdx.x * blockDim.x + threadIdx.x; i < nr; i += (int64_t)gridDim.x * blockDim.x) {
    const T r = r_nodes[i];
    T t = (T)2 * r;
    const T s = nn(dr / t);
    T ap = (T)1 + s;
    T am = (T)1 - s;
    tab[i] = ap / h2;
    tab[nr + i] = am / h2;
    t = c23 * dr;
    T a = nn(t / r);
    a = c23 + a;
    tab[2 * nr + i] = a / h2;
    t = c13 * dr;
    a = nn(t / r);
    tab[3 * nr + i] = c23 - a;
    t = (T)2 * dr;
    tab[4 * nr + i] = nn(t / r);
    tab[5 * nr + i] = r;
  }
}


static thread_local char g_create_err[512] = "";



void pa_set_err(pa_ctx* c, const char* fmt, ...) {
  va_list ap;
  va_start(ap, fmt);
  if (c) vsnprintf(c->err, sizeof(c->err), fmt, ap);
  else vsnprintf(g_create_err, sizeof(g_create_err), fmt, ap);
  va_end(ap);
}

namespace {
struct Roctx {
  int want = -1;
  int state = 0;
  int (*push)(const char*) = nullptr;
  int (*pop)() = nullptr;
};
Roctx g_roctx;
bool roctx_on() {
  Roctx& R = g_roctx;
  if (R.state == 0) {
    R.state = -1;
    const char* e = getenv("PYAPES_HIP_ROCTX");
    if (R.want >= 0 ? R.want != 0 : (e && atoi(e) != 0)) {
      void* h = dlopen("libroctx64.so.4", RTLD_NOW | RTLD_GLOBAL);
      if (!h) h = dlopen("libroctx64.so", RTLD_NOW | RTLD_GLOBAL);
      if (h) {
        R.push = reinterpret_cast<int (*)(const char*)>(dlsym(h, "roctxRangePushA"));
        R.pop = reinterpret_cast<int (*)()>(dlsym(h, "roctxRangePop"));
        if (R.push && R.pop) R.state = 1;
      }
    }
  }
  return R.state == 1;
}
}

void pa_range_push(const char* name) { if (roctx_on()) (void)g_roctx.push(name); }
void pa_range_pop() { if (roctx_on()) (void)g_roctx.pop(); }

int pa_hip_fail(pa_ctx* c, hipError_t e, const char* what) {
  pa_set_err(c, "HIP error in %s: %s", what, hipGetErrorString(e));
  return PA_E_HIP;
}

int pa_grid_blocks(int64_t work) {
  int64_t b = (work + PA_BLOCK - 1) / PA_BLOCK;
  if (b < 1) b = 1;
  if (b > PA_MAX_GRID) b = PA_MAX_GRID;
  return (int)b;
}

int pa_scratch(pa_ctx* c, void** slot, size_t* cap, size_t bytes) {
  if (*cap >= bytes && *slot) return PA_OK;
  const int q = (int)(slot - c->scr);
  if (*slot && (q == SCR_R || q == SCR_D0 || q == SCR_D1)) pa_place_reset(c);
  if (*slot) { (void)hipFree(c->scr_base[q]); c->scr_base[q] = nullptr; *slot = nullptr; *cap = 0; }
  if (bytes == 0) return PA_OK;
  const long stagger = 69888, sbase = 1;
  const size_t off = (size_t)(q + sbase) * (size_t)stagger;
  void* base = nullptr;
  {
    static const bool dbg = getenv("PYAPES_HIP_DEBUG") != nullptr;
    const auto t0 = std::chrono::steady_clock::now();
    PA_HIP(c, hipMalloc(&base, bytes + off + PA_PLACE_ROOM));
    if (dbg && bytes >= ((size_t)32 << 20))
      fprintf(stderr, "[pyapes_hip] scratch slot %d: hipMalloc of %.0f MiB: %.0f us\n", q, bytes / 1048576.0,
              std::chrono::duration<double, std::micro>(std::chrono::steady_clock::now() - t0).count());
  }
  c->scr_base[q] = base;
  *slot = (char*)base + off;
  *cap = bytes;
  return PA_OK;
}

template <typename T>
static void fill_coefs(const pa_ctx* c, DevEq<T>& E) {
  for (int a = 0; a < 3; ++a) {
    T h = (T)c->dx[a];
    T h2 = h * h;
    E.lap.inv[a] = (T)1 / h2;
    E.lap.m2inv[a] = (T)-2 / h2;
    E.lap.c23[a] = (T)(2.0 / 3.0) / h2;
    T th = (T)2 * h;
    T third = (T)(1.0 / 3.0);
    E.grd.h[a] = h;
    E.grd.ih[a] = (T)1 / h;
    E.grd.h2[a] = th;
    E.grd.g[a] = (T)1 / th;
    E.grd.mg[a] = (T)-1 / th;
    T v = (T)1 + third;
    E.grd.lo_p[a] = v / th;
    v = (T)0 - third;
    E.grd.lo_c[a] = v / th;
    v = (T)0 + third;
    E.grd.hi_c[a] = v / th;
    v = (T)-1 - third;
    E.grd.hi_m[a] = v / th;
  }
}

template <typename T>
void pa_build_eq(const pa_ctx* c, int nterms, const pa_term* terms, DevEq<T>& E) {
  memset(&E, 0, sizeof(E));
  E.nterms = nterms;
  for (int q = 0; q < nterms; ++q) {
    E.t[q].kind = terms[q].kind;
    E.t[q].has_coeff = terms[q].has_coeff;
    E.t[q].sign = (T)terms[q].sign;
    E.t[q].coeff = (T)terms[q].coeff;
    E.t[q].coeff_f = (const T*)terms[q].coeff_field;
    E.t[q].u = (T)terms[q].u;
    E.t[q].u_f = (const T*)terms[q].u_field;
  }
  fill_coefs<T>(c, E);
  E.rz = c->coord == PA_COORD_RZ ? (const T*)c->rz_tab : nullptr;
  E.rz_n = c->G.n1;
}
template void pa_build_eq<float>(const pa_ctx*, int, const pa_term*, DevEq<float>&);
template void pa_build_eq<double>(const pa_ctx*, int, const pa_term*, DevEq<double>&);

void pa_refresh_geom(pa_ctx* c) {
  DevGeom& G = c->G;
  for (int a = 0; a < 3; ++a) {
    int64_t N = a == 0 ? G.g0 : (a == 1 ? G.n1 : G.n2);
    if (!G.act[a]) { G.slo[a] = 0; G.shi[a] = 0; continue; }
    G.slo[a] = 1;
    G.shi[a] = N - 2;
    int lo_pos = -1, hi_pos = -1;
    for (int w = 0; w < c->nbc; ++w) {
      if (c->bc_order[w] == 2 * a) lo_pos = w;
      if (c->bc_order[w] == 2 * a + 1) hi_pos = w;
    }
    G.hi_last[a] = hi_pos > lo_pos;
  }
  for (int f = 0; f < 6; ++f) {
    int t = c->bc[f].type;
    G.bct[f] = t;
    G.treat[f] = (t == PA_BC_NEUMANN || t == PA_BC_SYMMETRY);
    if (t == PA_BC_PERIODIC) {
      int a = f >> 1;
      int64_t N = a == 0 ? G.g0 : (a == 1 ? G.n1 : G.n2);
      if ((f & 1) == 0) G.slo[a] = 0; else G.shi[a] = N - 1;
    }
  }
}

template <typename T>
Vec<T> pa_vec_self(const pa_ctx* c, const T* p) {
  Vec<T> v;
  v.p = p;
  v.glo = p + (c->G.n0 - 1) * c->G.s0;
  v.ghi = p;
  return v;
}
template Vec<float> pa_vec_self<float>(const pa_ctx*, const float*);
template Vec<double> pa_vec_self<double>(const pa_ctx*, const double*);

extern "C" {

const char* pa_version(void) { return "pyapes_hip 0.2 (gfx950)"; }

const char* pa_last_error(const pa_ctx* c) { return c ? c->err : g_create_err; }

int pa_ctx_create(int device, void* hip_stream, pa_ctx** out) {
  if (!out) { pa_set_err(nullptr, "pa_ctx_create: out is NULL"); return PA_E_ARG; }
  *out = nullptr;
  int ndev = 0;
  hipError_t e = hipGetDeviceCount(&ndev);
  if (e != hipSuccess || ndev == 0) {
    pa_set_err(nullptr, "pa_ctx_create: no HIP device visible (%s)", hipGetErrorString(e));
    return PA_E_HIP;
  }
  if (device < 0 || device >= ndev) { pa_set_err(nullptr, "pa_ctx_create: bad device %d", device); return PA_E_ARG; }
  e = hipSetDevice(device);
  if (e != hipSuccess) { pa_set_err(nullptr, "hipSetDevice: %s", hipGetErrorString(e)); return PA_E_HIP; }
  pa_ctx* c = new (std::nothrow) pa_ctx();
  if (!c) { pa_set_err(nullptr, "out of host memory"); return PA_E_ARG; }
  c->device = device;
  c->stream = (hipStream_t)hip_stream;
  c->err[0] = 0;
  static const struct { const char* env; const char* opt; } named[] = {
      {"PYAPES_HIP_FASTPATH", "fastpath"}, {"PYAPES_HIP_SF", "sf"}, {"PYAPES_HIP_FOLD", "fold"}, {"PYAPES_HIP_RESIDENT", "resident"},
      {"PYAPES_HIP_PITCH", "pitch"}, {"PYAPES_HIP_BCL", "bcl"}, {"PYAPES_HIP_COMM", "comm"}, {"PYAPES_HIP_SLAB_FOLD", "slab_fold"},
      {"PYAPES_HIP_COMM_OVERLAP", "comm_overlap"}, {"PYAPES_HIP_COMM_TIMEOUT", "comm_timeout"}};
  int orc = PA_OK;
  for (const auto& nv : named)
    if (const char* v = getenv(nv.env)) orc = orc ? orc : pa_ctx_set_option(c, nv.opt, atoi(v));
  if (const char* pl = getenv("PYAPES_HIP_PLACE")) {
    c->place = atoi(pl) != 0;
    if (atoi(pl) == 2) { c->ps.minbytes = 0; c->ps.budget = 1e9; }
  }
  if (const char* all = getenv("PYAPES_HIP_OPTIONS")) {
    char buf[1024];
    strncpy(buf, all, sizeof(buf) - 1);
    buf[sizeof(buf) - 1] = 0;
    for (char* tok = strtok(buf, ","); tok && !orc; tok = strtok(nullptr, ",")) {
      char* eq = strchr(tok, '=');
      if (!eq) { pa_set_err(c, "PYAPES_HIP_OPTIONS: '%s' is not name=value", tok); orc = PA_E_ARG; break; }
      *eq = 0;
      orc = pa_ctx_set_option(c, tok, atoi(eq + 1));
    }
  }
  if (orc) {
    pa_set_err(nullptr, "pa_ctx_create: %s", c->err);
    delete c;
    return orc;
  }
  if (hipMalloc((void**)&c->sc_base, 2 * sizeof(SolverScalars)) != hipSuccess ||
      hipMalloc((void**)&c->sums, PA_NSUM * sizeof(double)) != hipSuccess ||
      hipHostMalloc((void**)&c->h_sc, sizeof(SolverScalars)) != hipSuccess ||
      hipHostMalloc((void**)&c->h_poll[0], sizeof(SolverScalars)) != hipSuccess ||
      hipHostMalloc((void**)&c->h_poll[1], sizeof(SolverScalars)) != hipSuccess ||
      hipEventCreateWithFlags(&c->ev_poll[0], hipEventDisableTiming) != hipSuccess ||
      hipEventCreateWithFlags(&c->ev_poll[1], hipEventDisableTiming) != hipSuccess ||
      hipEventCreate(&c->ev0) != hipSuccess || hipEventCreate(&c->ev1) != hipSuccess) {
    pa_set_err(nullptr, "pa_ctx_create: allocation failed");
    delete c;
    return PA_E_HIP;
  }
  c->sc = c->sc_base;
  c->sc_alt = c->sc_base + 1;
  (void)hipMemsetAsync(c->sc_base, 0, 2 * sizeof(SolverScalars), c->stream);
  (void)hipMemsetAsync(c->sums, 0, PA_NSUM * sizeof(double), c->stream);
  *out = c;
  return PA_OK;
}

int pa_ctx_set_stream(pa_ctx* c, void* hip_stream) {
  if (!c) return PA_E_ARG;
  if (c->solve != PA_SOLVE_NONE && (hipStream_t)hip_stream != c->stream) {
    pa_set_err(c, "pa_ctx_set_stream during a stepwise solve");
    return PA_E_STATE;
  }
  hipStream_t next = (hipStream_t)hip_stream;
  if (next != c->stream) {
    PA_HIP(c, hipSetDevice(c->device));
    if (!c->ev_switch) PA_HIP(c, hipEventCreateWithFlags(&c->ev_switch, hipEventDisableTiming));
    auto order_after = [&](hipStream_t from) {
      if (hipEventRecord(c->ev_switch, from) == hipSuccess && hipStreamWaitEvent(next, c->ev_switch, 0) == hipSuccess) return;
      (void)hipGetLastError();
      (void)hipDeviceSynchronize();
      (void)hipGetLastError();
    };
    order_after(c->stream);
    if (c->xstream) order_after(c->xstream);
  }
  c->stream = next;
  return PA_OK;
}

int pa_ctx_set_option(pa_ctx* c, const char* name, int value) {
  if (!c || !name) return PA_E_ARG;
  if (c->solve != PA_SOLVE_NONE) { pa_set_err(c, "pa_ctx_set_option during a solve"); return PA_E_STATE; }
  if (!strcmp(name, "fastpath")) c->fastpath = value != 0;
  else if (!strcmp(name, "sf")) c->sf = (value == 2 || value == 4) ? value : (value != 0);
  else if (!strcmp(name, "chunks")) c->chunks = value < 0 ? 0 : value;
  else if (!strcmp(name, "sfq")) c->sfq = value < 0 ? 0 : value;
  else if (!strcmp(name, "fold")) c->fold = value != 0;
  else if (!strcmp(name, "resident")) c->resident = value != 0;
  else if (!strcmp(name, "cg2d_mincells")) c->cg2d_mincells = value;
  else if (!strcmp(name, "bcl")) c->bcl = value != 0;
  else if (!strcmp(name, "pitch")) c->pitch = value != 0;
  else if (!strcmp(name, "place")) c->place = value != 0;
  else if (!strcmp(name, "place_minbytes")) c->ps.minbytes = value < 0 ? 0 : (size_t)value;
  else if (!strcmp(name, "place_blocks")) c->ps.blocks = value < 0 ? 0 : (value > PA_PLACE_MAXSPARE ? PA_PLACE_MAXSPARE : value);
  else if (!strcmp(name, "place_budget")) c->ps.budget = 0.01 * (value < 0 ? 0 : value);
  else if (!strcmp(name, "resident_coop")) c->resident_coop = value != 0;
  else if (!strcmp(name, "bc_path")) c->bc_path = value & 7;
  else if (!strcmp(name, "bicg_pfold")) c->bicg_pfold = value != 0;
  else if (!strcmp(name, "bicg_srv")) c->bicg_srv = value != 0;
  else if (!strcmp(name, "jac_alt")) c->jac_alt = value != 0;
  else if (!strcmp(name, "rhs_full")) c->rhs_full = value != 0;
  else if (!strcmp(name, "res_cells")) c->res_cells = value;
  else if (!strcmp(name, "res_nt")) c->res_nt = value;
  else if (!strcmp(name, "res_nt_cells")) c->res_nt_cells = value;
  else if (!strcmp(name, "res_spin")) c->res_spin = value;
  else if (!strcmp(name, "res_rzlean")) c->res_rzlean = value != 0;
  else if (!strcmp(name, "comm")) c->opt_comm = value != 0;
  else if (!strcmp(name, "slab_fold")) c->opt_slab_fold = value != 0;
  else if (!strcmp(name, "comm_overlap")) c->comm_overlap = value < 0 ? -1 : (value != 0);
  else if (!strcmp(name, "comm_timeout")) c->comm_timeout = value > 0 ? value : 60;
  else if (!strcmp(name, "roctx")) { g_roctx.want = value != 0; g_roctx.state = 0; }
  else { pa_set_err(c, "pa_ctx_set_option: unknown option '%s'", name); return PA_E_ARG; }
  return PA_OK;
}

int pa_ctx_get_option(const pa_ctx* c, const char* name, int* value) {
  if (!c || !name || !value) return PA_E_ARG;
  const struct { const char* n; int v; } tab[] = {
      {"fastpath", c->fastpath}, {"sf", c->sf}, {"sfq", c->sfq}, {"chunks", c->chunks}, {"fold", c->fold}, {"resident", c->resident}, {"bcl", c->bcl}, {"pitch", c->pitch},
      {"place", c->place}, {"resident_coop", c->resident_coop}, {"bc_path", c->bc_path}, {"bicg_pfold", c->bicg_pfold}, {"bicg_srv", c->bicg_srv}, {"jac_alt", c->jac_alt},
      {"rhs_full", c->rhs_full}, {"comm", c->opt_comm}, {"slab_fold", c->opt_slab_fold}, {"comm_overlap", c->comm_overlap},
      {"comm_timeout", c->comm_timeout}, {"place_blocks", c->ps.blocks}};
  for (const auto& t : tab)
    if (!strcmp(name, t.n)) { *value = t.v; return PA_OK; }
  return PA_E_ARG;
}

int pa_ctx_destroy(pa_ctx* c) {
  if (!c) return PA_OK;
  (void)hipSetDevice(c->device);
  (void)hipStreamSynchronize(c->stream);
  if (c->comm) (void)pa_comm_destroy(c);
  pa_place_destroy(c);
  for (int q = 0; q < PA_NSCRATCH; ++q)
    if (c->scr_base[q]) (void)hipFree(c->scr_base[q]);
  if (c->sc_base) (void)hipFree(c->sc_base);
  if (c->sums) (void)hipFree(c->sums);
  if (c->rows_buf[0]) (void)hipFree(c->rows_buf[0]);
  if (c->rows_buf[1]) (void)hipFree(c->rows_buf[1]);
  if (c->h_sc) (void)hipHostFree(c->h_sc);
  for (int q = 0; q < 2; ++q) {
    if (c->h_poll[q]) (void)hipHostFree(c->h_poll[q]);
    if (c->ev_poll[q]) (void)hipEventDestroy(c->ev_poll[q]);
  }
  if (c->ev0) (void)hipEventDestroy(c->ev0);
  if (c->ev1) (void)hipEventDestroy(c->ev1);
  if (c->ev_switch) (void)hipEventDestroy(c->ev_switch);
  for (int q = 0; q < 4; ++q)
    if (c->pev[q]) (void)hipEventDestroy(c->pev[q]);
  delete c;
  return PA_OK;
}

int pa_grid_set(pa_ctx* c, int ndim, const int64_t* n, const double* dx, int dtype, int64_t i_off,
                int64_t n0_global) {
  if (!c) return PA_E_ARG;
  if (ndim < 1 || ndim > 3) { pa_set_err(c, "pa_grid_set: ndim must be 1..3"); return PA_E_ARG; }
  if (dtype != PA_F32 && dtype != PA_F64) { pa_set_err(c, "pa_grid_set: bad dtype"); return PA_E_ARG; }
  for (int a = 0; a < ndim; ++a)
    if (n[a] < 3 && !(a == 0 && n0_global >= 3 && n[a] >= 1)) {
      pa_set_err(c, "pa_grid_set: every axis needs >= 3 nodes (linalg.py:43-45)");
      return PA_E_ARG;
    }
  if (ndim < 3 && (i_off != 0 || n0_global != n[0])) {
    pa_set_err(c, "pa_grid_set: slab decomposition is for 3-D meshes only (1-D/2-D: replicas)");
    return PA_E_ARG;
  }
  if (i_off < 0 || i_off + n[0] > n0_global) { pa_set_err(c, "pa_grid_set: slab outside the global grid"); return PA_E_ARG; }
  DevGeom& G = c->G;
  memset(&G, 0, sizeof(G));
  int64_t ext[3] = {1, 1, 1};
  double h[3] = {1.0, 1.0, 1.0};
  const int sh = 3 - ndim;
  for (int a = 0; a < ndim; ++a) { ext[a + sh] = n[a]; h[a + sh] = dx[a]; G.act[a + sh] = 1; }
  G.n0 = ext[0]; G.n1 = ext[1]; G.n2 = ext[2];
  G.s1 = G.n2; G.s0 = G.n1 * G.n2;
  G.ncell = G.n0 * G.n1 * G.n2;
  G.off0 = ndim == 3 ? i_off : 0;
  G.g0 = ndim == 3 ? n0_global : 1;
  for (int a = 0; a < 3; ++a) c->dx[a] = h[a];
  c->ndim = ndim;
  c->dtype = dtype;
  c->esize = dtype == PA_F64 ? 8 : 4;
  c->grid_set = 1;
  c->eq_set = 0;
  c->solve = PA_SOLVE_NONE;
  for (int f = 0; f < 6; ++f) c->bc[f] = HostBC();
  c->nbc = 0;
  c->coord = PA_COORD_XYZ;
  c->rz_tab = nullptr;
  pa_refresh_geom(c);
  pa_place_reset(c);
  return PA_OK;
}

int pa_coord_set(pa_ctx* c, int coord_sys, const void* r_nodes) {
  if (!c || !c->grid_set) { if (c) pa_set_err(c, "pa_coord_set before pa_grid_set"); return PA_E_STATE; }
  if (coord_sys == PA_COORD_XYZ) { c->coord = PA_COORD_XYZ; c->rz_tab = nullptr; return PA_OK; }
  if (coord_sys != PA_COORD_RZ) { pa_set_err(c, "pa_coord_set: unknown coordinate system %d", coord_sys); return PA_E_ARG; }
  if (c->ndim != 2) { pa_set_err(c, "pa_coord_set: rz coordinate system only accepts 2-D grids (_mesh.py:48-49)"); return PA_E_ARG; }
  if (!r_nodes) { pa_set_err(c, "pa_coord_set: rz needs the r coordinates of the nodes"); return PA_E_ARG; }
  PA_HIP(c, hipSetDevice(c->device));
  const int64_t nr = c->G.n1;
  int rc = pa_scratch(c, &c->scr[SCR_RZ], &c->cap[SCR_RZ], (size_t)6 * nr * c->esize);
  if (rc) return rc;
  if (c->dtype == PA_F64)
    hipLaunchKernelGGL(k_rz_tables<double>, dim3(pa_grid_blocks(nr)), dim3(PA_BLOCK), 0, c->stream, nr,
                       (const double*)r_nodes, (double)c->dx[1], (double*)c->scr[SCR_RZ]);
  else
    hipLaunchKernelGGL(k_rz_tables<float>, dim3(pa_grid_blocks(nr)), dim3(PA_BLOCK), 0, c->stream, nr,
                       (const float*)r_nodes, (float)c->dx[1], (float*)c->scr[SCR_RZ]);
  PA_HIP(c, hipGetLastError());
  c->coord = PA_COORD_RZ;
  c->rz_tab = c->scr[SCR_RZ];
  c->solve = PA_SOLVE_NONE;
  return PA_OK;
}

static int pa_refuse_live(pa_ctx* c, const char* what) {
  if (c->solve == PA_SOLVE_NONE) return PA_OK;
  pa_set_err(c, "%s during a stepwise solve (pa_cg_begin ... pa_cg_end); end or abort it first", what);
  return PA_E_STATE;
}

int pa_bc_clear(pa_ctx* c) {
  if (!c || !c->grid_set) return PA_E_STATE;
  if (int rl = pa_refuse_live(c, "pa_bc_clear")) return rl;
  for (int f = 0; f < 6; ++f) c->bc[f] = HostBC();
  c->nbc = 0;
  pa_refresh_geom(c);
  return PA_OK;
}

int pa_bc_set(pa_ctx* c, int face, int order_pos, int type, double value, const void* face_vals, double dxf) {
  if (!c || !c->grid_set) { if (c) pa_set_err(c, "pa_bc_set before pa_grid_set"); return PA_E_STATE; }
  if (int rl = pa_refuse_live(c, "pa_bc_set")) return rl;
  if (face < 0 || face >= 2 * c->ndim) { pa_set_err(c, "pa_bc_set: face %d outside a %d-D mesh", face, c->ndim); return PA_E_ARG; }
  if (order_pos < 0 || order_pos >= 6) { pa_set_err(c, "pa_bc_set: bad order_pos"); return PA_E_ARG; }
  if (type < PA_BC_NONE || type > PA_BC_PERIODIC) { pa_set_err(c, "pa_bc_set: bad type"); return PA_E_ARG; }
  int fi = face + 2 * (3 - c->ndim);
  HostBC& b = c->bc[fi];
  b.type = type; b.value = value; b.vals = face_vals; b.dxf = dxf;
  c->bc_order[order_pos] = fi;
  if (order_pos + 1 > c->nbc) c->nbc = order_pos + 1;
  pa_refresh_geom(c);
  return PA_OK;
}

int pa_eq_set(pa_ctx* c, int nterms, const pa_term* terms) {
  if (!c || !c->grid_set) { if (c) pa_set_err(c, "pa_eq_set before pa_grid_set"); return PA_E_STATE; }
  if (int rl = pa_refuse_live(c, "pa_eq_set")) return rl;
  if (nterms < 1 || nterms > PA_MAX_TERMS) { pa_set_err(c, "pa_eq_set: 1..%d terms", PA_MAX_TERMS); return PA_E_ARG; }
  for (int q = 0; q < nterms; ++q) {
    int k = terms[q].kind;
    if (k == PA_OP_DIV_QUICK) { pa_set_err(c, "pa_eq_set: Div quick is explicit-only (no solver equations)"); return PA_E_ARG; }
    if (k < PA_OP_LAPLACIAN || k > PA_OP_DIV_UPWIND) { pa_set_err(c, "pa_eq_set: bad kind"); return PA_E_ARG; }
    if (k == PA_OP_DIV_CENTRAL)
      for (int f = 0; f < 6; ++f)
        if (c->G.treat[f]) {
          pa_set_err(c, "central Div with neumann/symmetry faces: the reference raises IndexError (fdc.py:583)");
          return PA_E_ARG;
        }
    if (k == PA_OP_DIV_CENTRAL && terms[q].u_field && c->G.n0 != c->G.g0 && c->ndim == 3) {
      pa_set_err(c, "tensor-u central Div is single-GPU only");
      return PA_E_ARG;
    }
  }
  c->nterms = nterms;
  for (int q = 0; q < nterms; ++q) c->terms[q] = terms[q];
  c->eq_set = 1;
  return PA_OK;
}

}

extern "C" {

int pa_slab_set(pa_ctx* c, const pa_slab* s) {
  if (!c || !c->grid_set) { if (c) pa_set_err(c, "pa_slab_set before pa_grid_set"); return PA_E_STATE; }
  if (c->solve != PA_SOLVE_NONE) { pa_set_err(c, "pa_slab_set during a solve"); return PA_E_STATE; }
  if (!s) {
    c->slab = 0;
    c->ext_sums = nullptr;
    c->x_glo = c->x_ghi = nullptr;
    c->r_send_lo = c->r_send_hi = nullptr;
    c->r_recv_lo = c->r_recv_hi = nullptr;
    c->bc_far_lo0 = c->bc_far_lo1 = c->bc_far_hi0 = nullptr;
    c->x_pack_lo1 = c->x_pack_hi0 = c->x_pack_hi1 = nullptr;
    return PA_OK;
  }
  if (c->ndim != 3) { pa_set_err(c, "pa_slab_set: slabs are for 3-D meshes"); return PA_E_ARG; }
  if (!s->sums) { pa_set_err(c, "pa_slab_set: sums buffer is required"); return PA_E_ARG; }
  c->slab = 1;
  c->ext_sums = (double*)s->sums;
  c->r_send_lo = s->r_send_lo; c->r_send_hi = s->r_send_hi;
  c->r_recv_lo = s->r_recv_lo; c->r_recv_hi = s->r_recv_hi;
  c->x_glo = s->x_ghost_lo; c->x_ghi = s->x_ghost_hi;
  c->bc_far_lo0 = s->bc_far_lo0; c->bc_far_lo1 = s->bc_far_lo1; c->bc_far_hi0 = s->bc_far_hi0;
  c->x_pack_lo1 = s->x_pack_lo1; c->x_pack_hi0 = s->x_pack_hi0; c->x_pack_hi1 = s->x_pack_hi1;
  return PA_OK;
}

}
```

pyapes_amd/csrc/pa_host.h:

```cpp
#pragma once
#include <hip/hip_runtime.h>
#include <stdarg.h>
#include <stdint.h>

#include "../../include/pyapes_hip.h"
#include "pa_device.h"

#define PA_MAX_GRID 2048
#define PA_MAX_PARTIALS 131072

struct SolverScalars {
  double rr, rr_old, dAd, alpha, beta, tol, tolerance;
  double rho, omega, rho_next, r0v, ts, tt, r0t;
  long long itr, max_it;
  int done, err, finished_early;
};

struct HostBC {
  int type = PA_BC_NONE;
  double value = 0.0;
  const void* vals = nullptr;
  double dxf = 0.0;
};

enum {
  SCR_R = 0, SCR_D0, SCR_D1, SCR_PART, SCR_PART2, SCR_SHELL, SCR_R0, SCR_V0, SCR_V1, SCR_S, SCR_TT,
  SCR_GHOST, SCR_SHELL2, SCR_RZ, SCR_RES, PA_NSCRATCH
};

#define PA_PLACE_ROOM ((size_t)2 << 20)

#define PA_PLACE_MAXSPARE 8
#define PA_PLACE_NEV 8
#define PA_PLACE_NDUR 32
#define PA_PLACE_NX 4
struct PlaceSearch {
  size_t minbytes = (size_t)128 << 20;
  int blocks = 3;
  double budget = 0.03;
  char* spare[PA_PLACE_MAXSPARE] = {nullptr};
  int spare_epoch[PA_PLACE_MAXSPARE] = {0};
  int nspare = 0;
  size_t bytes = 0, blk = 0;
  int phase = 0;
  int role = 0, cand = 0;
  const void* decided[PA_PLACE_NX] = {nullptr};
  int n_decided = 0;
  int active = 0, st = 0, pause = 0;
  int r_move = 0;
  int epoch = 0;
  const void* x = nullptr;
  int64_t it = 0, known = -1, s = 0, clean_from = 1;
  double base = 0.0;
  double dur[PA_PLACE_NDUR] = {0.0};
  double base_par[2] = {0.0, 0.0};
  unsigned char par[PA_PLACE_NDUR] = {0};
  hipEvent_t ev0[PA_PLACE_NEV] = {nullptr}, ev1[PA_PLACE_NEV] = {nullptr};
  hipEvent_t evs[2] = {nullptr, nullptr};
  int closed = 1, sw_timed = 0;
  int trials = 0, accepted = 0, mallocs = 0;
  double spent_us = 0.0, elapsed_us = 0.0, first_pair = 0.0;
};

enum PaSolve { PA_SOLVE_NONE, PA_SOLVE_CG, PA_SOLVE_BICG, PA_SOLVE_JACOBI };

struct pa_ctx {
  int device = 0;
  hipStream_t stream = nullptr;
  char err[512];
  int grid_set = 0, ndim = 0, dtype = PA_F64, esize = 8;
  double dx[3] = {1, 1, 1};
  DevGeom G;
  HostBC bc[6];
  int bc_order[6] = {0, 0, 0, 0, 0, 0};
  int nbc = 0;
  int eq_set = 0, nterms = 0;
  pa_term terms[PA_MAX_TERMS];
  void* scr[PA_NSCRATCH] = {nullptr};
  void* scr_base[PA_NSCRATCH] = {nullptr};
  size_t cap[PA_NSCRATCH] = {0};
  SolverScalars* sc = nullptr;
  SolverScalars* sc_alt = nullptr;
  SolverScalars* sc_base = nullptr;
  int fold = 1, in_iterate = 0;
  int fold_a_n = 0;
  int fold_b_n = 0, fold_b_nsh = 0;
  const double* fold_b_part = nullptr;
  const double* fold_b_shell = nullptr;
  int slab_fold = 0;
  int slab_fold_live = 0;
  int fold_rows[3] = {0, 0, 0};
  double* rows_send = nullptr;
  double* rows_recv = nullptr;
  double* rows_buf[2] = {nullptr, nullptr};
  size_t rows_cap = 0;
  int plan_only = 0;
  SolverScalars* h_sc = nullptr;
  SolverScalars* h_poll[2] = {nullptr, nullptr};
  hipEvent_t ev_poll[2] = {nullptr, nullptr};
  double* sums = nullptr;
  double* ext_sums = nullptr;
  hipEvent_t ev0 = nullptr, ev1 = nullptr;
  hipEvent_t ev_switch = nullptr;
  PaSolve solve = PA_SOLVE_NONE;
  int cur = 0, pending_init_logic = 0, b_blocks = 0;
  int bc_static = 0, bc_fused = 0, bc_pair = 0;
  int shell_cur = 0;
  void* cg_x = nullptr;
  const void* jac_rhs = nullptr;
  double jac_omega = 1.0;
  void* cg_r_out = nullptr;
  int64_t cg2d_mincells = 1500000;
  int bcl = 1;
  int place = 1;
  PlaceSearch ps;
  int pitch = 1;
  int bc_path = 0;
  int bicg_pfold = 1;
  int bicg_srv = 1;
  int bicg_s_stored = 1;
  int jac_alt = 1;
  int jac_dir = 0;
  int rhs_full = 0;
  int res_cells = 0, res_nt = 0, res_nt_cells = 0, res_spin = -1, res_rzlean = 1;
  int opt_comm = 1;
  int opt_slab_fold = 1;
  int comm_overlap = -1;
  int comm_timeout = 60;
  int cg_pitch = 0;
  int64_t cg_ps1 = 0;
  void* x_old_out = nullptr;
  int slab = 0;
  const void* x_glo = nullptr;
  const void* x_ghi = nullptr;
  void* r_send_lo = nullptr;
  void* r_send_hi = nullptr;
  const void* r_recv_lo = nullptr;
  const void* r_recv_hi = nullptr;
  void* d_glo[2] = {nullptr, nullptr};
  void* d_ghi[2] = {nullptr, nullptr};
  const void* bc_far_lo0 = nullptr;
  const void* bc_far_lo1 = nullptr;
  const void* bc_far_hi0 = nullptr;
  void* v_send_lo = nullptr;
  void* v_send_hi = nullptr;
  const void* v_recv_lo = nullptr;
  const void* v_recv_hi = nullptr;
  void* x_pack_lo1 = nullptr;
  void* x_pack_hi0 = nullptr;
  void* x_pack_hi1 = nullptr;
  int profile = 0;
  hipEvent_t pev[4] = {nullptr, nullptr, nullptr, nullptr};
  double prof_ms[2] = {0.0, 0.0};
  int64_t prof_n[2] = {0, 0};
  int fastpath = 1;
  int sfq = 1;
  int sf = 1;
  int chunks = 0;
  int resident = 1;
  int resident_coop = 1;
  int resident_used = 0;
  void* comm = nullptr;
  void* comm2 = nullptr;
  hipStream_t xstream = nullptr;
  hipEvent_t ev_b = nullptr, ev_x = nullptr;
  int comm_rank = 0, comm_n = 0;
  pa_exchange plan;
  int plan_set = 0;
  int coord = 0;
  const void* rz_tab = nullptr;
};

static inline double* pa_sums(const pa_ctx* c) { return (c->slab && c->ext_sums) ? c->ext_sums : c->sums; }

static inline const int* pa_done_flag(const pa_ctx* c) { return &c->sc->done; }

void pa_set_err(pa_ctx* c, const char* fmt, ...);
void pa_range_push(const char* name);
void pa_range_pop();
struct PaRange {
  explicit PaRange(const char* name) { pa_range_push(name); }
  ~PaRange() { pa_range_pop(); }
};
int pa_hip_fail(pa_ctx* c, hipError_t e, const char* what);
int pa_grid_blocks(int64_t work);
int pa_scratch(pa_ctx* c, void** slot, size_t* cap, size_t bytes);
void pa_refresh_geom(pa_ctx* c);
int pa_bc_apply_any(pa_ctx* c, void* x);
int pa_check_eq_applicable(pa_ctx* c);
int pa_require_solve(pa_ctx* c, PaSolve kind, const char* what);
int pa_cg_slab_mid(pa_ctx* c);
int pa_cg_slab_flush(pa_ctx* c);
int pa_bc_shell_rows(const pa_ctx* c);
void pa_profile_stop(pa_ctx* c, int which);
int pa_place_begin(pa_ctx* c, const void* x, size_t array_bytes);
int pa_place_tick(pa_ctx* c);
int pa_place_batch_end(pa_ctx* c);
void pa_place_r_written(pa_ctx* c);
int pa_place_prepare_block(pa_ctx* c, void* block);
void pa_place_end(pa_ctx* c, int may_free);
void pa_place_reset(pa_ctx* c);
void pa_place_destroy(pa_ctx* c);

int pa_shell_blocks(const pa_ctx* c);
int64_t pa_shell_elems(const pa_ctx* c);
bool pa_bc_is_static(const pa_ctx* c);
bool pa_bc_fusable(const pa_ctx* c);
bool pa_bc_pairable(const pa_ctx* c);
template <typename T>
int pa_bc_apply_faces(pa_ctx* c, T* x, bool guarded = false);
template <typename T>
int pa_bc_apply_auto(pa_ctx* c, T* x, bool guarded);
void pa_bc_plan(pa_ctx* c);
template <typename T>
int pa_bc_fill_start(pa_ctx* c, T* x, bool filled_by_driver);
template <typename T>
int pa_bc_fill_step(pa_ctx* c, T* x, double* part2, int* nsh);

#define PA_HIP(c, call)                                              \
  do {                                                               \
    hipError_t e__ = (call);                                         \
    if (e__ != hipSuccess) return pa_hip_fail((c), e__, #call);      \
  } while (0)

template <typename T>
void pa_build_eq(const pa_ctx* c, int nterms, const pa_term* terms, DevEq<T>& E);
template <typename T>
Vec<T> pa_vec_self(const pa_ctx* c, const T* p);

template <typename T>
int pa_cg3d_phase_a(pa_ctx* c, const DevEq<T>& E, Vec<T> r, Vec<T> d, T* dnew, double* partials);
template <typename T>
int pa_cg3d_phase_b(pa_ctx* c, const DevEq<T>& E, Vec<T> d, T* x, T* r, double* partials);

template <typename T>
int pa_resident_launch(pa_ctx* c, int solver, T* x, const T* rhs, double tol, int64_t max_it, double omega);

template <typename T>
int pa_tile3d_aop(pa_ctx* c, const DevEq<T>& E, Vec<T> x, T* y, int interior_only);
template <typename T>
int pa_tile3d_grad(pa_ctx* c, Vec<T> x, T* y, int nd);
template <typename T>
int pa_sfq_euler(pa_ctx* c, Vec<T> phi, T* out, double u, const void* u_field, double nu, double dt, const T* phi0 = nullptr,
                 double c0 = 0.0, double c1 = 0.0, const pa_source* src = nullptr);
template <typename T>
int pa_tile3d_euler(pa_ctx* c, Vec<T> phi, T* out, int kind, double u, const void* u_field, double nu, double dt,
                    int bcl = 0,
                    const T* phi0 = nullptr, double c0 = 0.0, double c1 = 0.0,
                    const pa_source* src = nullptr);
template <typename T>
int pa_tile3d_jacobi(pa_ctx* c, const DevEq<T>& E, Vec<T> x, const T* rhs, T* xnew, double omega, double* partials);
template <typename T>
int pa_tile3d_bicg_pv(pa_ctx* c, const DevEq<T>& E, Vec<T> r, Vec<T> p, Vec<T> v, const T* r0, T* pnew, T* vnew,
                      double* partials);
template <typename T>
int pa_tile3d_bicg_v(pa_ctx* c, const DevEq<T>& E, Vec<T> p, const T* r0, T* vnew, double* partials);
template <typename T>
int pa_tile3d_bicg_st(pa_ctx* c, const DevEq<T>& E, Vec<T> r, Vec<T> v, const T* r0, T* s_out, T* t_out,
                      double* partials);
```

Before: 88.07 billion cell-updates*iters/s.

## Fold periodic z-face boundary fill into CG phase B kernel

Adds a ZF variant of the tiled CG phase B kernel. It applies the periodic z-face boundary update (the two end k-columns) inline, and its own tail lanes handle the last z vectors and write the wrapped ghost value. The separate BC pair kernel then covers only the remaining rows near the x/y faces, which shrinks the z-axis BC pass and its extra global reads and writes of the x field. The cost is a more complex kernel with extra lane broadcasts and masked stores, a waves_per_eu hint of 2, and an extra partial reduction buffer.

```diff
diff --git a/pyapes_amd/csrc/pa_bc.hip b/pyapes_amd/csrc/pa_bc.hip
--- a/pyapes_amd/csrc/pa_bc.hip
+++ b/pyapes_amd/csrc/pa_bc.hip
@@ -352,6 +352,7 @@
   BCArgs<T> lo, hi;
   int axis;
   int64_t pos_lo, pos_hi;
+  int zlo[2], zhi[2];
 };
 
 template <typename T>
@@ -389,7 +390,7 @@
   return x0_new;
 }
 
-template <typename T>
+template <typename T, bool ZROWS = false>
 __global__ void __launch_bounds__(PA_BLOCK) k_bc_pair(DevGeom G, T* __restrict__ x, BCPairArgs<T> P,
                                                        const int* __restrict__ done, T* __restrict__ shell_old,
                                                        double* __restrict__ partials, int mode) {
@@ -401,9 +402,26 @@
   const int64_t off = (a == 0) ? G.off0 : 0;
   const int64_t st = (a == 0) ? G.s0 : (a == 1 ? G.s1 : 1);
   double s[1] = {0.0};
-  for (int64_t q = (int64_t)blockIdx.x * blockDim.x + threadIdx.x; q < nu * nv;
-       q += (int64_t)gridDim.x * blockDim.x) {
-    const int64_t u = q / nv, v = q - u * nv;
+  const int64_t nI = ZROWS ? P.zlo[0] + P.zhi[0] : 0, nJ = ZROWS ? P.zlo[1] + P.zhi[1] : 0;
+  const int64_t work = ZROWS ? nI * nv + (nu - nI) * nJ : nu * nv;
+  for (int64_t w = (int64_t)blockIdx.x * blockDim.x + threadIdx.x; w < work;
+       w += (int64_t)gridDim.x * blockDim.x) {
+    int64_t u, v;
+    if (ZROWS) {
+      if (w < nI * nv) {
+        const int64_t ui = w / nv;
+        v = w - ui * nv;
+        u = ui < P.zlo[0] ? ui : nu - nI + ui;
+      } else {
+        const int64_t w2 = w - nI * nv, ui = w2 / nJ, vj = w2 - ui * nJ;
+        u = P.zlo[0] + ui;
+        v = vj < P.zlo[1] ? vj : nv - nJ + vj;
+      }
+    } else {
+      u = w / nv;
+      v = w - u * nv;
+    }
+    const int64_t q = u * nv + v;
     int64_t base;
     bool owned = true;
     if (a == 0) {
@@ -463,7 +481,7 @@
 template <typename T>
 static int pa_bc_shell_fused(pa_ctx* c, T* x, double* part2, int with_delta, bool guarded, int* nsh, bool standalone);
 template <typename T>
-static int pa_bc_pair_apply(pa_ctx* c, T* x, double* part2, int mode, bool guarded, int* nsh);
+static int pa_bc_pair_apply(pa_ctx* c, T* x, double* part2, int mode, bool guarded, int* nsh, bool zrows = false);
 template <typename T>
 static void pa_shell_launch(pa_ctx* c, const T* x, T* shell, double* part2, int with_delta);
 
@@ -709,8 +727,13 @@
   }
 }
 
-template <typename T>
-static int pa_bc_pair_apply(pa_ctx* c, T* x, double* part2, int mode, bool guarded, int* nsh) {
+static int64_t pa_bc_zrows(const pa_ctx* c) {
+  const int64_t nI = c->zf_lo[0] + c->zf_hi[0], nJ = c->zf_lo[1] + c->zf_hi[1];
+  return nI * c->G.n1 + (c->G.n0 - nI) * nJ;
+}
+
+template <typename T>
+static int pa_bc_pair_apply(pa_ctx* c, T* x, double* part2, int mode, bool guarded, int* nsh, bool zrows) {
   const DevGeom& G = c->G;
   const int64_t sz[3] = {G.n1 * G.n2, G.n0 * G.n2, G.n0 * G.n1};
   int64_t start[6], total = 0;
@@ -731,10 +754,15 @@
     P.axis = a;
     P.pos_lo = start[2 * a];
     P.pos_hi = start[2 * a + 1];
-    const int nb = pa_grid_blocks(sz[a]);
-    hipLaunchKernelGGL(k_bc_pair<T>, dim3(nb), dim3(PA_BLOCK), 0, c->stream, G, x, P,
-                       guarded ? pa_done_flag(c) : (const int*)nullptr, shell, part2 ? part2 + rows : nullptr,
-                       mode);
+    for (int q = 0; q < 2; ++q) { P.zlo[q] = c->zf_lo[q]; P.zhi[q] = c->zf_hi[q]; }
+    const bool zr = zrows && a == 2;
+    const int nb = pa_grid_blocks(zr ? pa_bc_zrows(c) : sz[a]);
+    if (zr)
+      hipLaunchKernelGGL((k_bc_pair<T, true>), dim3(nb), dim3(PA_BLOCK), 0, c->stream, G, x, P,
+                         guarded ? pa_done_flag(c) : (const int*)nullptr, shell, part2 ? part2 + rows : nullptr, mode);
+    else
+      hipLaunchKernelGGL((k_bc_pair<T, false>), dim3(nb), dim3(PA_BLOCK), 0, c->stream, G, x, P,
+                         guarded ? pa_done_flag(c) : (const int*)nullptr, shell, part2 ? part2 + rows : nullptr, mode);
     if (mode == 1) rows += nb;
   }
   if (nsh) *nsh = rows;
@@ -770,6 +798,7 @@
   c->bc_static = pa_bc_is_static(c);
   c->bc_fused = pa_bc_fusable(c);
   c->bc_pair = (!c->bc_fused && pa_bc_pairable(c)) ? 1 : 0;
+  c->bc_zfold = 0;
   c->shell_cur = 0;
 }
 
@@ -789,7 +818,7 @@
   *nsh = 0;
   if (c->bc_static) return PA_OK;
   if (c->bc_fused) return pa_bc_shell_fused<T>(c, x, part2, 1, true, nsh, false);
-  if (c->bc_pair) return pa_bc_pair_apply<T>(c, x, part2, 1, true, nsh);
+  if (c->bc_pair) return pa_bc_pair_apply<T>(c, x, part2, 1, true, nsh, c->bc_zfold != 0);
   if (int rc = pa_bc_apply_faces<T>(c, x, true)) return rc;
   *nsh = pa_shell_blocks(c);
   pa_shell_launch<T>(c, (const T*)x, (T*)c->scr[SCR_SHELL], part2, 1);
diff --git a/pyapes_amd/csrc/pa_cg.hip b/pyapes_amd/csrc/pa_cg.hip
--- a/pyapes_amd/csrc/pa_cg.hip
+++ b/pyapes_amd/csrc/pa_cg.hip
@@ -217,6 +217,28 @@
 }
 
 template <typename T>
+static void cg_zfold_plan(pa_ctx* c, const DevEq<T>& E, const T* x) {
+  c->bc_zfold = 0;
+  if ((c->bc_path & 8) || c->slab || !c->bc_pair || c->bc_fused || c->bc_static) return;
+  if (c->bc[4].type != PA_BC_PERIODIC || c->bc[5].type != PA_BC_PERIODIC) return;
+  if (!pa_cg3d_zfold_ok<T>(c, E, x)) return;
+  const int64_t n[2] = {c->G.n0, c->G.n1};
+  for (int a = 0; a < 2; ++a) {
+    auto depth = [&](int f, int other) {
+      const int t = c->bc[f].type;
+      if (t == PA_BC_NEUMANN) return 3;
+      if (t == PA_BC_SYMMETRY || t == PA_BC_PERIODIC || c->bc[other].type == PA_BC_PERIODIC) return 2;
+      return 1;
+    };
+    int lo = depth(2 * a, 2 * a + 1), hi = depth(2 * a + 1, 2 * a);
+    if (lo + hi >= n[a]) { lo = (int)n[a]; hi = 0; }
+    c->zf_lo[a] = lo;
+    c->zf_hi[a] = hi;
+  }
+  c->bc_zfold = 1;
+}
+
+template <typename T>
 static int cg_begin_t(pa_ctx* c, T* x, const T* rhs, double tol, int64_t max_it) {
   const DevGeom& G = c->G;
   const size_t fb = (size_t)G.ncell * sizeof(T);
@@ -229,7 +251,7 @@
   if ((rc = pa_scratch(c, &c->scr[SCR_D0], &c->cap[SCR_D0], fbp))) return rc;
   if ((rc = pa_scratch(c, &c->scr[SCR_D1], &c->cap[SCR_D1], fbp))) return rc;
   if ((rc = pa_scratch(c, &c->scr[SCR_PART], &c->cap[SCR_PART], (size_t)PA_MAX_PARTIALS * 4 * sizeof(double)))) return rc;
-  if ((rc = pa_scratch(c, &c->scr[SCR_PART2], &c->cap[SCR_PART2], (size_t)3 * PA_MAX_GRID * sizeof(double)))) return rc;
+  if ((rc = pa_scratch(c, &c->scr[SCR_PART2], &c->cap[SCR_PART2], ((size_t)3 * PA_MAX_GRID + PA_MAX_PARTIALS) * sizeof(double)))) return rc;
   if ((rc = pa_scratch(c, &c->scr[SCR_SHELL], &c->cap[SCR_SHELL], 2 * (size_t)pa_shell_elems(c) * sizeof(T)))) return rc;
   if ((rc = init_scalars(c, tol, max_it))) return rc;
   if ((rc = pa_place_begin(c, x, fb))) return rc;
@@ -243,6 +265,7 @@
   c->solve = PA_SOLVE_CG;
   DevEq<T> E;
   pa_build_eq<T>(c, c->nterms, c->terms, E);
+  cg_zfold_plan<T>(c, E, x);
   if ((rc = pa_bc_fill_start<T>(c, x, c->slab != 0))) return rc;
   T* r = (T*)c->scr[SCR_R];
   T* d = (T*)c->scr[SCR_D0];
@@ -368,6 +391,7 @@
   int used_blocks = rc;
   if (rc == 0 && live) { pa_set_err(c, "folded slab iteration: the tiled phase B declined after the plan"); return PA_E_STATE; }
   if (rc == 0 && c->cg_pitch) { pa_set_err(c, "pitched CG: the tiled phase B declined"); return PA_E_STATE; }
+  if (rc == 0 && c->bc_zfold) { pa_set_err(c, "CG with the z-face fill inside phase B: the tiled phase B declined"); return PA_E_STATE; }
   if (rc == 0) {
     cg_flush_fold<T>(c);
     hipLaunchKernelGGL(k_cg_b<T>, dim3(nblk), dim3(PA_BLOCK), 0, c->stream, G, E, c->sc, dv, x, (const T*)r,
@@ -383,7 +407,9 @@
     return PA_OK;
   }
   int nsh;
-  if ((rc = pa_bc_fill_step<T>(c, x, part2, &nsh))) return rc;
+  const int nzf = c->bc_zfold ? used_blocks : 0;
+  if ((rc = pa_bc_fill_step<T>(c, x, part2 + nzf, &nsh))) return rc;
+  nsh += nzf;
   const bool foldable = c->fold && c->in_iterate && stage_post == 2 && !c->slab && !c->profile &&
                         used_blocks <= PA_MAX_GRID && nsh <= 3 * PA_MAX_GRID;
   if (foldable) {
diff --git a/pyapes_amd/csrc/pa_cg3d.hip b/pyapes_amd/csrc/pa_cg3d.hip
--- a/pyapes_amd/csrc/pa_cg3d.hip
+++ b/pyapes_amd/csrc/pa_cg3d.hip
@@ -53,6 +53,16 @@
     A.sc_w = c->sc;
     A.pre_sums = pa_sums(c);
   }
+  if (c->bc_zfold) {
+    if (mode != 1 || c->ndim != 3 || c->slab) return 0;
+    for (int a = 0; a < 2; ++a) { A.zf_lo[a] = c->zf_lo[a]; A.zf_hi[a] = c->zf_hi[a]; }
+    A.zf_nl = (int)std::min<int64_t>(8, c->G.n2 / VecOf<T>::N - 1);
+    A.zf_part = (double*)c->scr[SCR_PART2];
+    const int nz = launch_zfold<T>(c, A);
+    if (nz > 0 && hipGetLastError() != hipSuccess) { pa_set_err(c, "k_cg3d phase B (z faces folded) launch failed"); return PA_E_HIP; }
+    if (nz > 0) c->fold_a_n = 0;
+    return nz;
+  }
   int n = (mode == 1 || mode == 3 || mode == 4) ? launch_cg2d<T, 1>(c, A, mode == 3) : 0;
   if (n == 0 && rz) return 0;
   if (n == 0) n = launch_any<T, 1>(c, A, mode);
@@ -60,6 +70,17 @@
   if (n > 0) c->fold_a_n = 0;
   return n;
 }
+
+template <typename T>
+bool pa_cg3d_zfold_ok(pa_ctx* c, const DevEq<T>& E, const T* x) {
+  if (c->slab || c->ndim != 3 || !c->G.act[0] || c->cg_pitch || c->coord != PA_COORD_XYZ) return false;
+  if (E.nterms != 1 || E.t[0].kind != PA_OP_LAPLACIAN || E.t[0].coeff_f) return false;
+  if (cg3d_mode<T>(c, E, {x, c->scr[SCR_R], c->scr[SCR_D0], c->scr[SCR_D1]}) != 1) return false;
+  const int rj = pick_rj<T>(c, false, true);
+  return rj == 2 || rj == 4;
+}
+template bool pa_cg3d_zfold_ok<float>(pa_ctx*, const DevEq<float>&, const float*);
+template bool pa_cg3d_zfold_ok<double>(pa_ctx*, const DevEq<double>&, const double*);
 
 template <typename T>
 int pa_tile3d_jacobi(pa_ctx* c, const DevEq<T>& E, Vec<T> x, const T* rhs, T* xnew, double omega, double* partials) {
diff --git a/pyapes_amd/csrc/pa_cg3d_kernel.h b/pyapes_amd/csrc/pa_cg3d_kernel.h
--- a/pyapes_amd/csrc/pa_cg3d_kernel.h
+++ b/pyapes_amd/csrc/pa_cg3d_kernel.h
@@ -53,6 +53,9 @@
   T stg_c0, stg_c1;
   const T* src;
   T src_val;
+  int zf_lo[2], zf_hi[2];
+  int zf_nl;
+  double* zf_part;
 };
 
 __device__ __forceinline__ int pa_xcd_remap(int b, int nb) {
@@ -60,14 +63,22 @@
   return (xcd < r ? xcd * (q + 1) : r * (q + 1) + (xcd - r) * q) + w;
 }
 
+__device__ __forceinline__ float pa_lane_bcast(float v, int l) {
+  return __int_as_float(__builtin_amdgcn_readlane(__float_as_int(v), l));
+}
+__device__ __forceinline__ double pa_lane_bcast(double v, int l) {
+  return __hiloint2double(__builtin_amdgcn_readlane(__double2hiint(v), l), __builtin_amdgcn_readlane(__double2loint(v), l));
+}
+
 __device__ __forceinline__ int64_t pa_wrapmod(int64_t v, int64_t n) {
   v %= n;
   return v < 0 ? v + n : v;
 }
 
-template <typename T, int RJ, int PHASE, bool CF = false, int KIND = 0, int LAY = 0, bool STG = false>
-__global__ void __launch_bounds__(256) k_cg3d(Cg3dArgs<T> A) {
+template <typename T, int RJ, int PHASE, bool CF = false, int KIND = 0, int LAY = 0, bool STG = false, bool ZF = false>
+__global__ void __launch_bounds__(256) __attribute__((amdgpu_waves_per_eu(ZF ? 2 : 1))) k_cg3d(Cg3dArgs<T> A) {
   static_assert(!STG || PHASE == 3, "STG: the explicit Euler step");
+  static_assert(!ZF || (PHASE == 1 && LAY == 0 && !CF), "ZF: CG phase B in the vector layout, scalar coefficient");
   constexpr int PH = PHASE == 9 ? 4 : PHASE;
   constexpr bool NARROW = LAY == 1, PITCH = LAY == 2;
   static_assert(!PITCH || ((PH == 0 || PH == 1 || PH == 5 || PH == 6 || PH == 8) && !CF && KIND == 0),
@@ -110,6 +121,20 @@
     if (rc == 1) rowLo |= 1u << jj;
     if (rc == 2) rowHi |= 1u << jj;
   }
+  const int znl = ZF ? A.zf_nl : 0, zt = lane & 7;
+  const bool ztile = ZF && tkb == 0, ztail = ZF && kvalid && kg >= G.n2 - (int64_t)znl * VEC;
+  const bool zmine = ztile && lane < 8 * RJ && zt < znl;
+  const bool zface = zmine && zt == znl - 1;
+  int64_t zoff = 0;
+  unsigned rowZ = 0;
+  if constexpr (ZF) {
+#pragma unroll
+    for (int jj = 0; jj < RJ; ++jj) {
+      const int64_t jg = j0 + wv * RJ + jj;
+      if (jg >= A.zf_lo[1] && jg < G.n1 - A.zf_hi[1]) rowZ |= 1u << jj;
+      if ((lane >> 3) == jj) zoff = jrow[jj] * G.s1 + (G.n2 - (int64_t)(znl - zt) * VEC);
+    }
+  }
   unsigned rowPLo = 0, rowPHi = 0, colPLo = 0, colPHi = 0;
   if (PH == 3 || PH == 7 || KIND != 0) {
 #pragma unroll
@@ -133,6 +158,10 @@
     const int rc = pa_row_case(G, 2, kk, G.n2, G.treat);
     if (rc == 1) colLo |= 1u << v;
     if (rc == 2) colHi |= 1u << v;
+  }
+  if constexpr (ZF) {
+    colLo = colHi = 0;
+    colS = kvalid ? (1u << VEC) - 1 : 0u;
   }
 #ifdef PA_PLAIN_EXPERIMENT
   rowLo = rowHi = colLo = colHi = 0;
@@ -469,10 +498,19 @@
     const bool more = m + 1 < CI;
     if (more) stage(buf ^ 1, eb, hv, hs);
     V xv[RJ], rv[RJ];
+    V xl, dl;
+    T x1s[RJ];
+    const unsigned foldZ = (ZF && ii >= A.zf_lo[0] && ii < G.n0 - A.zf_hi[0]) ? rowZ : 0u;
     if (PH == 1) {
 #pragma unroll
       for (int jj = 0; jj < RJ; ++jj) {
         const int64_t o = ii * G.s0 + jrow[jj] * G.s1 + kc;
+        if constexpr (ZF) {
+          if (ztail && (foldZ >> jj & 1)) xv[jj] = (V)(T)0;
+          else xv[jj] = __builtin_nontemporal_load(reinterpret_cast<const V*>(A.x + o));
+          rv[jj] = __builtin_nontemporal_load(reinterpret_cast<const V*>(A.rw + o));
+          continue;
+        }
         if (PITCH) {
           rv[jj] = __builtin_nontemporal_load(reinterpret_cast<const V*>(A.rw + ii * fs0 + jrow[jj] * fs1 + kcf));
           const T* xp = A.x + ii * G.s0 + jrow[jj] * G.s1;
@@ -485,6 +523,12 @@
           xv[jj] = __builtin_nontemporal_load(reinterpret_cast<const V*>(A.x + o));
           rv[jj] = __builtin_nontemporal_load(reinterpret_cast<const V*>(A.rw + o));
         }
+      }
+    }
+    if constexpr (ZF) {
+      if (zmine && (foldZ >> (lane >> 3) & 1)) {
+        xl = __builtin_nontemporal_load(reinterpret_cast<const V*>(A.x + ii * G.s0 + zoff));
+        dl = *reinterpret_cast<const V*>(d_run - pstep + zoff);
       }
     }
     V cv[RJ];
@@ -821,7 +865,8 @@
           rn = inS ? rn : (T)0;
           T p = rn * rn;
           s0 += (double)p;
-          const bool offshell = inS && !(iShell || (rowShell >> jj & 1) || (colShell >> v & 1));
+          bool offshell = inS && !(iShell || (rowShell >> jj & 1) || (colShell >> v & 1));
+          if constexpr (ZF) offshell = offshell && !(ztail && (foldZ >> jj & 1));
           T df = xn - xo;
           T p2 = df * df;
           s1 += offshell ? (double)p2 : 0.0;
@@ -829,6 +874,7 @@
           outx[v] = xn;
         }
       }
+      if constexpr (ZF) x1s[jj] = pa_lane_bcast(outx[1], 0);
       if (kvalid && (rowValid >> jj & 1)) {
         const int64_t o = ii * G.s0 + jrow[jj] * G.s1 + kc;
         const int64_t ob = PITCH ? ii * fs0 + jrow[jj] * fs1 + kcf : o;
@@ -854,12 +900,49 @@
             *reinterpret_cast<V*>(A.x + o) = outx;
             *reinterpret_cast<V*>(A.rw_out + o) = outd;
           } else {
-            __builtin_nontemporal_store(outx, reinterpret_cast<V*>(A.x + o));
+            if (ZF && (foldZ >> jj & 1) && (ztail || (ztile && lane == 0))) {
+              if (!ztail) {
+#pragma unroll
+                for (int v = 1; v < VEC; ++v) __builtin_nontemporal_store(outx[v], A.x + o + v);
+              }
+            } else {
+              __builtin_nontemporal_store(outx, reinterpret_cast<V*>(A.x + o));
+            }
             __builtin_nontemporal_store(outd, reinterpret_cast<V*>(A.rw_out + o));
           }
           if (A.send_lo && ii == 0) *reinterpret_cast<V*>(A.send_lo + jrow[jj] * G.s1 + kc) = outd;
           if (A.send_hi && ii == G.n0 - 1) *reinterpret_cast<V*>(A.send_hi + jrow[jj] * G.s1 + kc) = outd;
         }
+      }
+    }
+
+    if constexpr (ZF) {
+      if (zmine && (foldZ >> (lane >> 3) & 1)) {
+        T x1 = x1s[0];
+#pragma unroll
+        for (int jj = 1; jj < RJ; ++jj)
+          if ((lane >> 3) == jj) x1 = x1s[jj];
+        V xnl;
+#pragma unroll
+        for (int v = 0; v < VEC; ++v) {
+          T ad = alpha * dl[v];
+          xnl[v] = xl[v] + ad;
+          T df = xnl[v] - xl[v];
+          T p2 = df * df;
+          s1 += (v < VEC - 1 || !zface) ? (double)p2 : 0.0;
+        }
+        T* xr = A.x + ii * G.s0 + zoff;
+        if (zface) {
+          T t = x1 - xnl[VEC - 1];
+          const T x0 = t + xnl[VEC - 2];
+          T df = x0 - xl[VEC - 1];
+          T p2 = df * df;
+          s2 += (double)p2;
+          s2 += (double)p2;
+          xnl[VEC - 1] = x0;
+          __builtin_nontemporal_store(x0, xr - (G.n2 - VEC));
+        }
+        __builtin_nontemporal_store(xnl, reinterpret_cast<V*>(xr));
       }
     }
 
@@ -881,6 +964,10 @@
   } else if (PH == 1 || PH == 4) {
     double s[2] = {s0, s1};
     pa_block_reduce_store<2>(s, A.partials);
+    if constexpr (ZF) {
+      double sz[1] = {s2};
+      pa_block_reduce_store<1>(sz, A.zf_part);
+    }
   } else if (PH == 5 || PH == 8) {
     double s[1] = {s0};
     pa_block_reduce_store<1>(s, A.partials);
@@ -945,18 +1032,18 @@
   return cus;
 }
 
-template <typename T, int RJ, int PHASE, bool CF, int KIND = 0, int LAY = 0, bool STG = false>
+template <typename T, int RJ, int PHASE, bool CF, int KIND = 0, int LAY = 0, bool STG = false, bool ZF = false>
 static int blocks_per_cu() {
   static int cached = 0;
   if (!cached) {
     int n = 0;
-    if (hipOccupancyMaxActiveBlocksPerMultiprocessor(&n, k_cg3d<T, RJ, PHASE, CF, KIND, LAY, STG>, 256, 0) != hipSuccess || n <= 0) n = 2;
+    if (hipOccupancyMaxActiveBlocksPerMultiprocessor(&n, k_cg3d<T, RJ, PHASE, CF, KIND, LAY, STG, ZF>, 256, 0) != hipSuccess || n <= 0) n = 2;
     cached = n;
   }
   return cached;
 }
 
-template <typename T, int RJ, int PHASE, bool CF = false, int KIND = 0, int LAY = 0, bool STG = false>
+template <typename T, int RJ, int PHASE, bool CF = false, int KIND = 0, int LAY = 0, bool STG = false, bool ZF = false>
 static int launch_cg3d(pa_ctx* c, Cg3dArgs<T>& A) {
   constexpr bool NARROW = LAY == 1;
   constexpr int VEC = NARROW ? 1 : VecOf<T>::N;
@@ -970,7 +1057,7 @@
   A.tiles_j = (int)((n1e + TJ - 1) / TJ);
   A.tiles_k = (int)((n2e + TK - 1) / TK);
   const int tiles = A.tiles_j * A.tiles_k;
-  const int capacity = cus_of(c) * blocks_per_cu<T, RJ, PHASE, CF, KIND, LAY, STG>();
+  const int capacity = cus_of(c) * blocks_per_cu<T, RJ, PHASE, CF, KIND, LAY, STG, ZF>();
   int chunks = capacity / tiles;
   if (chunks < 1) chunks = 1;
   if (chunks > G.n0) chunks = (int)G.n0;
@@ -983,11 +1070,11 @@
   if (dbg > 0) {
     --dbg;
     fprintf(stderr, "[pyapes_hip] k_cg3d phase %c%s%s: tiles %dx%d chunks %d (CI ~%lld) blocks %d, %d blocks/CU x %d CUs\n",
-            (char)('A' + PHASE), LAY == 1 ? " (narrow)" : (LAY == 2 ? " (pitched)" : ""), STG ? " (RK stage)" : "", A.tiles_j, A.tiles_k, chunks, (long long)(G.n0 / chunks), nblk,
-            blocks_per_cu<T, RJ, PHASE, CF, KIND, LAY, STG>(), cus_of(c));
+            (char)('A' + PHASE), LAY == 1 ? " (narrow)" : (LAY == 2 ? " (pitched)" : ""), STG ? " (RK stage)" : (ZF ? " (z faces folded)" : ""), A.tiles_j, A.tiles_k, chunks, (long long)(G.n0 / chunks), nblk,
+            blocks_per_cu<T, RJ, PHASE, CF, KIND, LAY, STG, ZF>(), cus_of(c));
   }
   if (c->plan_only) return nblk;
-  hipLaunchKernelGGL((k_cg3d<T, RJ, PHASE, CF, KIND, LAY, STG>), dim3(nblk), dim3(256), 0, c->stream, A);
+  hipLaunchKernelGGL((k_cg3d<T, RJ, PHASE, CF, KIND, LAY, STG, ZF>), dim3(nblk), dim3(256), 0, c->stream, A);
   return nblk;
 }
 
@@ -1064,6 +1151,16 @@
     case 1: return launch_cg3d<T, 1, PHASE, false, 0, NARROW>(c, A);
     case 2: return launch_cg3d<T, 2, PHASE, false, 0, NARROW>(c, A);
     default: return launch_cg3d<T, 4, PHASE, false, 0, NARROW>(c, A);
+  }
+}
+
+template <typename T>
+static int launch_zfold(pa_ctx* c, Cg3dArgs<T>& A) {
+  if (A.coeff_f || A.kind != 0) return 0;
+  switch (pick_rj<T>(c, false, true)) {
+    case 2: return launch_cg3d<T, 2, 1, false, 0, 0, false, true>(c, A);
+    case 4: return launch_cg3d<T, 4, 1, false, 0, 0, false, true>(c, A);
+    default: return 0;
   }
 }
 
diff --git a/pyapes_amd/csrc/pa_core.hip b/pyapes_amd/csrc/pa_core.hip
--- a/pyapes_amd/csrc/pa_core.hip
+++ b/pyapes_amd/csrc/pa_core.hip
@@ -308,7 +308,7 @@
   else if (!strcmp(name, "place_blocks")) c->ps.blocks = value < 0 ? 0 : (value > PA_PLACE_MAXSPARE ? PA_PLACE_MAXSPARE : value);
   else if (!strcmp(name, "place_budget")) c->ps.budget = 0.01 * (value < 0 ? 0 : value);
   else if (!strcmp(name, "resident_coop")) c->resident_coop = value != 0;
-  else if (!strcmp(name, "bc_path")) c->bc_path = value & 7;
+  else if (!strcmp(name, "bc_path")) c->bc_path = value & 15;
   else if (!strcmp(name, "bicg_pfold")) c->bicg_pfold = value != 0;
   else if (!strcmp(name, "bicg_srv")) c->bicg_srv = value != 0;
   else if (!strcmp(name, "jac_alt")) c->jac_alt = value != 0;
@@ -333,7 +333,8 @@
       {"fastpath", c->fastpath}, {"sf", c->sf}, {"sfq", c->sfq}, {"chunks", c->chunks}, {"fold", c->fold}, {"resident", c->resident}, {"bcl", c->bcl}, {"pitch", c->pitch},
       {"place", c->place}, {"resident_coop", c->resident_coop}, {"bc_path", c->bc_path}, {"bicg_pfold", c->bicg_pfold}, {"bicg_srv", c->bicg_srv}, {"jac_alt", c->jac_alt},
       {"rhs_full", c->rhs_full}, {"comm", c->opt_comm}, {"slab_fold", c->opt_slab_fold}, {"comm_overlap", c->comm_overlap},
-      {"comm_timeout", c->comm_timeout}, {"place_blocks", c->ps.blocks}};
+      {"comm_timeout", c->comm_timeout}, {"place_blocks", c->ps.blocks},
+      {"bc_zfold", c->bc_zfold}};
   for (const auto& t : tab)
     if (!strcmp(name, t.n)) { *value = t.v; return PA_OK; }
   return PA_E_ARG;
diff --git a/pyapes_amd/csrc/pa_host.h b/pyapes_amd/csrc/pa_host.h
--- a/pyapes_amd/csrc/pa_host.h
+++ b/pyapes_amd/csrc/pa_host.h
@@ -105,6 +105,8 @@
   PaSolve solve = PA_SOLVE_NONE;
   int cur = 0, pending_init_logic = 0, b_blocks = 0;
   int bc_static = 0, bc_fused = 0, bc_pair = 0;
+  int bc_zfold = 0;
+  int zf_lo[2] = {0, 0}, zf_hi[2] = {0, 0};
   int shell_cur = 0;
   void* cg_x = nullptr;
   const void* jac_rhs = nullptr;
@@ -232,6 +234,8 @@
 int pa_cg3d_phase_a(pa_ctx* c, const DevEq<T>& E, Vec<T> r, Vec<T> d, T* dnew, double* partials);
 template <typename T>
 int pa_cg3d_phase_b(pa_ctx* c, const DevEq<T>& E, Vec<T> d, T* x, T* r, double* partials);
+template <typename T>
+bool pa_cg3d_zfold_ok(pa_ctx* c, const DevEq<T>& E, const T* x);
 
 template <typename T>
 int pa_resident_launch(pa_ctx* c, int solver, T* x, const T* rhs, double tol, int64_t max_it, double omega);
```

After: 88.02 billion cell-updates*iters/s. No clear change (-0.1%).
